# rasmus-kirk/halo

Measured on AMD Instinct MI355X. Metric: MSM points/sec (Pippenger, Pallas, 2^20 points, resident SRS), higher is better.
Workload: dtype u32 limbs (255-bit Montgomery field, integer)

## Files before the change

halo_amd/csrc/curve.hpp:

```cpp
#pragma once
#include "fields.hpp"

HALO_ARITH_BEGIN

struct PallasCurve {
    using Base = FqCfg;
    using Scalar = FpCfg;
    using K = PallasCurveCfg;
};
struct VestaCurve {
    using Base = FpCfg;
    using Scalar = FqCfg;
    using K = VestaCurveCfg;
};

template <class F>
struct Affine {
    Fe<F> x, y;
};

template <class F>
struct XYZZ {
    Fe<F> X, Y, ZZ, ZZZ;
};
// ... 44 lines not shown
    const Fe<F> V = fe_sqr(U);
    const Fe<F> W = fe_mul(U, V);
    const Fe<F> S = fe_mul(p.X, V);
    const Fe<F> X2 = fe_sqr(p.X);
    const Fe<F> M = fe_norm(fe_add_nc(X2, fe_add_nc(X2, X2)));
    XYZZ<F> r;
    r.X = fe_reduce_8p(fe_sub_k<4>(fe_sqr(M), fe_add_nc(S, S)));
    r.Y = fe_sub(fe_mul(M, fe_sub_k<2>(S, r.X)), fe_mul(W, p.Y));
    r.ZZ = fe_mul(V, p.ZZ);
    r.ZZZ = fe_mul(W, p.ZZZ);
    return r;
}

template <class F>
HALO_DEV XYZZ<F> xyzz_mdbl(const Affine<F>& a) {
    const Fe<F> U = fe_norm(fe_add_nc(a.y, a.y));
    const Fe<F> V = fe_sqr(U);
    const Fe<F> W = fe_mul(U, V);
    const Fe<F> S = fe_mul(a.x, V);
    const Fe<F> X2 = fe_sqr(a.x);
    const Fe<F> M = fe_norm(fe_add_nc(X2, fe_add_nc(X2, X2)));
    XYZZ<F> r;
    r.X = fe_reduce_8p(fe_sub_k<4>(fe_sqr(M), fe_add_nc(S, S)));
    r.Y = fe_sub(fe_mul(M, fe_sub_k<2>(S, r.X)), fe_mul(W, a.y));
    r.ZZ = V;
    r.ZZZ = W;
    return r;
}

template <class F>
HALO_DEV XYZZ<F> xyzz_madd(const XYZZ<F>& p, const Affine<F>& q) {
    if (aff_is_id(q)) return p;
    if (xyzz_is_id(p)) return xyzz_from_aff(q);
    const Fe<F> U2 = fe_mul(q.x, p.ZZ);
    const Fe<F> S2 = fe_mul(q.y, p.ZZZ);
    const Fe<F> P = fe_sub_k<2>(U2, p.X);
    const Fe<F> R = fe_sub_k<2>(S2, p.Y);
    const Fe<F> PP = fe_sqr(P);
    const Fe<F> ZZ3 = fe_mul(p.ZZ, PP);
    if (fe_is_zero(ZZ3)) {
        if (fe_is_zero_4p(R)) return xyzz_mdbl(q);
        return xyzz_id<F>();
    }
    const Fe<F> PPP = fe_mul(P, PP);
    const Fe<F> Q = fe_mul(p.X, PP);
    XYZZ<F> r;
    r.X = fe_reduce_8p(fe_sub_k<6>(fe_sqr(R), fe_add_nc(PPP, fe_add_nc(Q, Q))));
    r.Y = fe_sub(fe_mul(R, fe_sub_k<2>(Q, r.X)), fe_mul(p.Y, PPP));
    r.ZZ = ZZ3;
    r.ZZZ = fe_mul(p.ZZZ, PPP);
    return r;
}

template <class F>
HALO_DEV XYZZ<F> xyzz_madd_acc(const XYZZ<F>& p, const Affine<F>& q, uint32_t negmask) {
    if (aff_is_id(q)) return p;
    if (xyzz_is_id(p)) {
        XYZZ<F> r = xyzz_from_aff(q);
        if (negmask) r.Y = fe_neg(q.y);
        return r;
    }
    const Fe<F> U2 = fe_mul(q.x, p.ZZ);
    const Fe<F> S2 = fe_mul(q.y, p.ZZZ);
    const Fe<F> P = fe_sub_k<8>(U2, p.X);
    const Fe<F> R = fe_sub_k_sgn<4>(S2, p.Y, negmask);
    const Fe<F> PP = fe_sqr(P);
    const Fe<F> R2 = fe_sqr(R);
    const Fe<F> ZZ3 = fe_mul(p.ZZ, PP);
    const Fe<F> PPP = fe_mul(P, PP);
    const Fe<F> Q = fe_mul(p.X, PP);
    XYZZ<F> r;
    r.X = fe_sub_k<6>(R2, fe_add_nc(PPP, fe_add_nc(Q, Q)));
    const Fe<F> T = fe_sub_k<8>(Q, r.X);
    r.Y = fe_mul2(R, T, PPP, fe_sub_k<2>(fe_zero<F>(), p.Y));
    r.ZZ = ZZ3;
    r.ZZZ = fe_mul(p.ZZZ, PPP);
    if (fe_is_zero(ZZ3)) {
        if (fe_is_zero(fe_reduce_8p(R))) {
            Affine<F> qs = q;
            if (negmask) qs.y = fe_neg(q.y);
            return xyzz_mdbl(qs);
        }
        return xyzz_id<F>();
    }
    return r;
}

template <class F>
HALO_DEV XYZZ<F> xyzz_madd_run(const XYZZ<F>& p, uint32_t& sneg, bool& fresh, const Affine<F>& q, uint32_t negmask,
                               bool check_q) {
    if (check_q && aff_is_id(q)) return p;
    if (fresh) {
        fresh = false;
        sneg = negmask;
        asm volatile("" : "+v"(sneg));
        XYZZ<F> r;
        r.X = q.x;
        r.Y = q.y;
        r.ZZ = fe_one<F>();
        r.ZZZ = fe_one<F>();
        return r;
    }
    const Fe<F> U2 = fe_mul(q.x, p.ZZ);
    const Fe<F> S2 = fe_mul(q.y, p.ZZZ);
    const Fe<F> P = fe_sub_k<4>(U2, p.X);
    const Fe<F> R = fe_sub_k_sgn<4>(S2, p.Y, negmask ^ sneg);
    const Fe<F> PP = fe_sqr(P);
    const Fe<F> R2 = fe_sqr(R);
    const Fe<F> ZZ3 = fe_mul(p.ZZ, PP);
    const Fe<F> PPP = fe_mul(P, PP);
    const Fe<F> V = fe_mul(U2, PP);
    const Fe<F> Q = fe_sub_nc(V, PPP);
    XYZZ<F> r;
    r.X = fe_sub_nc(fe_sub_nc(R2, Q), V);
    const Fe<F> T = fe_sub_k<6>(r.X, Q);
    r.Y = fe_mul2(R, T, p.Y, PPP);
    r.ZZ = ZZ3;
    r.ZZZ = fe_mul(p.ZZZ, PPP);
    if (P.v[0] < 10u && fe_is_zero(ZZ3)) {
        const bool dbl = fe_is_zero(fe_reduce_8p(R));
        sneg = 0;
        if (dbl) {
            Affine<F> qs = q;
            if (negmask) qs.y = fe_neg(q.y);
            return xyzz_mdbl(qs);
        }
        fresh = true;
        return xyzz_id<F>();
    }
    sneg = ~sneg;
    return r;
}

template <class F>
HALO_DEV XYZZ<F> xyzz_madd_run_aff(const XYZZ<F>& p, uint32_t& sneg, bool& fresh, const Affine<F>& q, uint32_t negmask,
                                   bool check_q) {
    if (check_q && aff_is_id(q)) return p;
    if (fresh) {
        fresh = false;
        sneg = negmask;
        asm volatile("" : "+v"(sneg));
        XYZZ<F> r;
        r.X = q.x;
        r.Y = q.y;
        r.ZZ = fe_one<F>();
        r.ZZZ = fe_one<F>();
        return r;
    }
    const Fe<F> P = fe_sub_k<2>(q.x, p.X);
    const Fe<F> R = fe_sub_k_sgn<4>(q.y, p.Y, negmask ^ sneg);
    const Fe<F> PP = fe_sqr(P);
    const Fe<F> R2 = fe_sqr(R);
    const Fe<F> PPP = fe_mul(P, PP);
    const Fe<F> V = fe_mul(q.x, PP);
    const Fe<F> Q = fe_sub_nc(V, PPP);
    XYZZ<F> r;
    r.X = fe_sub_nc(fe_sub_nc(R2, Q), V);
    const Fe<F> T = fe_sub_k<6>(r.X, Q);
    r.Y = fe_mul2(R, T, p.Y, PPP);
    r.ZZ = PP;
    r.ZZZ = PPP;
    if (P.v[0] < 4u && fe_is_zero(PP)) {
        const bool dbl = fe_is_zero(fe_reduce_8p(R));
        sneg = 0;
        if (dbl) {
            Affine<F> qs = q;
            if (negmask) qs.y = fe_neg(q.y);
            return xyzz_mdbl(qs);
        }
        fresh = true;
        return xyzz_id<F>();
    }
    sneg = ~sneg;
    return r;
}

template <class F>
HALO_DEV XYZZ<F> xyzz_run_out(const XYZZ<F>& p, uint32_t sneg) {
    XYZZ<F> r = p;
    r.X = fe_sub_k<4>(p.X, fe_zero<F>());
    int32_t c = 0;
#pragma unroll
    for (int i = 0; i < NLIMB; i++) {
        const int32_t x = (int32_t)((p.Y.v[i] ^ sneg) - sneg) + (int32_t)(F::P2[i] & sneg) + c;
        r.Y.v[i] = (i == NLIMB - 1) ? (uint32_t)x : ((uint32_t)x & LIMB_MASK);
        c = x >> LIMB_BITS;
    }
    return r;
}

template <class F>
HALO_DEV XYZZ<F> xyzz_settle(const XYZZ<F>& p) {
    XYZZ<F> r = p;
    r.X = fe_reduce_8p(p.X);
    return r;
}

template <class F>
HALO_DEV XYZZ<F> xyzz_add(const XYZZ<F>& p, const XYZZ<F>& q) {
    if (xyzz_is_id(q)) return p;
    if (xyzz_is_id(p)) return q;
    const Fe<F> U1 = fe_mul(p.X, q.ZZ);
    const Fe<F> U2 = fe_mul(q.X, p.ZZ);
    const Fe<F> S1 = fe_mul(p.Y, q.ZZZ);
    const Fe<F> S2 = fe_mul(q.Y, p.ZZZ);
    const Fe<F> P = fe_sub_k<2>(U2, U1);
    const Fe<F> R = fe_sub_k<2>(S2, S1);
    const Fe<F> PP = fe_sqr(P);
    const Fe<F> ZZ3 = fe_mul(fe_mul(p.ZZ, q.ZZ), PP);
    if (fe_is_zero(ZZ3)) {
        if (fe_is_zero_4p(R)) return xyzz_dbl(p);
        return xyzz_id<F>();
    }
    const Fe<F> PPP = fe_mul(P, PP);
    const Fe<F> Q = fe_mul(U1, PP);
    XYZZ<F> r;
    r.X = fe_reduce_8p(fe_sub_k<6>(fe_sqr(R), fe_add_nc(PPP, fe_add_nc(Q, Q))));
    r.Y = fe_sub(fe_mul(R, fe_sub_k<2>(Q, r.X)), fe_mul(S1, PPP));
    r.ZZ = ZZ3;
    r.ZZZ = fe_mul(fe_mul(p.ZZZ, q.ZZZ), PPP);
    return r;
}

template <class F>
HALO_DEV XYZZ<F> xyzz_add_acc(const XYZZ<F>& p, const XYZZ<F>& q) {
    if (xyzz_is_id(q)) return p;
    if (xyzz_is_id(p)) return q;
    const Fe<F> U1 = fe_mul(p.X, q.ZZ);
    const Fe<F> U2 = fe_mul(q.X, p.ZZ);
    const Fe<F> S1 = fe_mul(p.Y, q.ZZZ);
    const Fe<F> S2 = fe_mul(q.Y, p.ZZZ);
    const Fe<F> P = fe_sub_k<2>(U2, U1);
    const Fe<F> R = fe_sub_k<2>(S2, S1);
    const Fe<F> PP = fe_sqr(P);
    const Fe<F> R2 = fe_sqr(R);
    const Fe<F> ZZ3 = fe_mul(fe_mul(p.ZZ, q.ZZ), PP);
    const Fe<F> PPP = fe_mul(P, PP);
    const Fe<F> Q = fe_mul(U1, PP);
    XYZZ<F> r;
    r.X = fe_sub_k<6>(R2, fe_add_nc(PPP, fe_add_nc(Q, Q)));
    const Fe<F> T = fe_sub_k<8>(Q, r.X);
    r.Y = fe_mul2(R, T, PPP, fe_sub_k<2>(fe_zero<F>(), S1));
    r.ZZ = ZZ3;
    r.ZZZ = fe_mul(fe_mul(p.ZZZ, q.ZZZ), PPP);
    if (P.v[0] < 4u && fe_is_zero(ZZ3)) {
        if (fe_is_zero_4p(R)) return xyzz_dbl(xyzz_settle(p));
        return xyzz_id<F>();
    }
    return r;
}

template <class F>
HALO_DEV XYZZ<F> xyzz_neg(const XYZZ<F>& p) {
    XYZZ<F> r = p;
    r.Y = fe_neg(p.Y);
    return r;
}

template <class F>
HALO_DEV Affine<F> xyzz_to_aff(const XYZZ<F>& p) {
    Affine<F> r;
    if (xyzz_is_id(p)) {
        r.x = fe_zero<F>();
        r.y = fe_zero<F>();
        return r;
    }
    const Fe<F> t = fe_inv(fe_mul(p.ZZ, p.ZZZ));
    r.x = fe_mul(p.X, fe_mul(t, p.ZZZ));
    r.y = fe_mul(p.Y, fe_mul(t, p.ZZ));
    return r;
}

template <class F>
HALO_DEV Affine<F> aff_load(const uint4* p) {
    Affine<F> a;
    a.x = fe_load<F>(p);
    a.y = fe_load<F>(p + 2);
    return a;
}
template <class F>
HALO_DEV void aff_store(uint4* p, const Affine<F>& a) {
    fe_store(p, a.x);
    fe_store(p + 2, a.y);
}
template <class F>
HALO_DEV XYZZ<F> xyzz_load(const uint4* p) {
    XYZZ<F> a;
    a.X = fe_load<F>(p);
    a.Y = fe_load<F>(p + 2);
    a.ZZ = fe_load<F>(p + 4);
    a.ZZZ = fe_load<F>(p + 6);
    return a;
}
template <class F>
HALO_DEV void xyzz_store(uint4* p, const XYZZ<F>& a) {
    fe_store(p, a.X);
    fe_store(p + 2, a.Y);
    fe_store(p + 4, a.ZZ);
    fe_store(p + 6, a.ZZZ);
}

constexpr int PARTIAL_U4 = 9;
template <class F>
HALO_DEV void partial_store(uint4* p, const XYZZ<F>& a) {
    const Fe<F>* c[4] = {&a.X, &a.Y, &a.ZZ, &a.ZZZ};
    uint32_t w[4 * NLIMB];
#pragma unroll
    for (int k = 0; k < 4; k++)
#pragma unroll
        for (int i = 0; i < NLIMB; i++) w[k * NLIMB + i] = c[k]->v[i];
#pragma unroll
    for (int q = 0; q < PARTIAL_U4; q++) p[q] = make_uint4(w[4 * q], w[4 * q + 1], w[4 * q + 2], w[4 * q + 3]);
}
template <class F>
HALO_DEV XYZZ<F> partial_load(const uint4* p) {
    uint32_t w[4 * NLIMB];
#pragma unroll
    for (int q = 0; q < PARTIAL_U4; q++) {
        const uint4 v = p[q];
        w[4 * q] = v.x;
        w[4 * q + 1] = v.y;
        w[4 * q + 2] = v.z;
        w[4 * q + 3] = v.w;
    }
    XYZZ<F> a;
    Fe<F>* c[4] = {&a.X, &a.Y, &a.ZZ, &a.ZZZ};
#pragma unroll
    for (int k = 0; k < 4; k++)
#pragma unroll
        for (int i = 0; i < NLIMB; i++) c[k]->v[i] = w[k * NLIMB + i];
    a.X = fe_reduce_8p(a.X);
    return a;
}

template <class F>
HALO_DEV Affine<F> aff_from_wrapped(const uint4* p) {
    Affine<F> a;
    a.x = fe_from_ark<F>(p);
    a.y = fe_from_ark<F>(p + 2);
    return a;
}
template <class F>
HALO_DEV void aff_to_wrapped(uint4* p, const Affine<F>& a) {
    fe_to_ark(p, a.x);
    fe_to_ark(p + 2, a.y);
}

template <class F>
struct Jac {
    Fe<F> X, Y, Z;
};

template <class F>
HALO_DEV Jac<F> jac_from_xyzz(const XYZZ<F>& p) {
    Jac<F> r;
    if (xyzz_is_id(p)) {
        r.X = fe_one<F>();
        r.Y = fe_one<F>();
        r.Z = fe_zero<F>();
        return r;
    }
    r.X = fe_mul(p.X, fe_sqr(p.ZZ));
    r.Y = fe_mul(p.Y, fe_sqr(p.ZZZ));
    r.Z = p.ZZZ;
    return r;
}

template <class F>
HALO_DEV XYZZ<F> jac_to_xyzz(const Jac<F>& j) {
    XYZZ<F> r;
    r.X = j.X;
    r.Y = j.Y;
    r.ZZ = fe_sqr(j.Z);
    r.ZZZ = fe_mul(r.ZZ, j.Z);
    return r;
}

template <class F>
HALO_DEV Jac<F> jac_dbl(const Jac<F>& p) {
    const Fe<F> A = fe_sqr(p.X);
    const Fe<F> B = fe_sqr(p.Y);
    const Fe<F> C = fe_sqr(B);
    const Fe<F> D = fe_dbl(fe_sub(fe_sub(fe_sqr(fe_add(p.X, B)), A), C));
    const Fe<F> E = fe_add(A, fe_dbl(A));
    const Fe<F> Fv = fe_sqr(E);
    Jac<F> r;
    r.X = fe_sub(Fv, fe_dbl(D));
    const Fe<F> C8 = fe_dbl(fe_dbl(fe_dbl(C)));
    r.Y = fe_sub(fe_mul(E, fe_sub(D, r.X)), C8);
    r.Z = fe_dbl(fe_mul(p.Y, p.Z));
    return r;
}

template <class F>
HALO_DEV XYZZ<F> xyzz_scalar_mul(const Affine<F>& P, const uint32_t (&k)[8]) {
    XYZZ<F> acc = xyzz_id<F>();
    for (int i = 255; i >= 0; i--) {
        acc = xyzz_dbl(acc);
        if ((k[i >> 5] >> (i & 31)) & 1u) acc = xyzz_madd(acc, P);
    }
    return acc;
}

HALO_ARITH_END
```

halo_amd/csrc/digits.hpp:

```cpp
#pragma once
#include "digits_core.hpp"
#include "fields.hpp"

namespace halo {

template <class S, int WMAX = 0, int C = 0, class Fn>
HALO_DEV void scalar_signed_digits(const uint4* scalar, int c, int W, Fn&& f) {
    uint32_t w8[8];
    fe_ark_to_canonical_words<S>(scalar, w8);
    uint32_t t8[8];
    int64_t br = 0, lt = 0;
#pragma unroll
    for (int q = 0; q < 8; q++) {
        const int64_t d = (int64_t)(uint32_t)(S::MODULUS64[q >> 1] >> (32 * (q & 1))) - (int64_t)w8[q] + br;
        t8[q] = (uint32_t)d;
        br = d >> 32;
        lt = ((int64_t)t8[q] - (int64_t)w8[q] + lt) >> 32;
    }
    const bool neg = lt != 0;
#pragma unroll
    for (int q = 0; q < 8; q++) w8[q] = neg ? t8[q] : w8[q];
    signed_digit_entries<C, WMAX>(w8, neg ? 0x80000000u : 0u, c, W, f);
}

}
```

halo_amd/csrc/digits_core.hpp:

```cpp
#pragma once
#include <cstdint>

#if defined(__HIPCC__)
#define HALO_DIGITS_FN __host__ __device__ inline __attribute__((always_inline))
#else
#define HALO_DIGITS_FN inline
#endif
#if defined(__clang__)
#define HALO_DIGITS_UNROLL _Pragma("unroll")
#else
#define HALO_DIGITS_UNROLL
#endif

namespace halo {

constexpr uint32_t DIGIT_NONE = 0xffffffffu;

HALO_DIGITS_FN uint32_t digits_funnel(uint32_t hi, uint32_t lo, uint32_t s) {
    return (uint32_t)((((uint64_t)hi << 32) | lo) >> s);
}

HALO_DIGITS_FN uint32_t digits_entry(uint32_t raw, uint32_t& carry, uint32_t half, uint32_t full, uint32_t flip) {
    const uint32_t v = raw + carry;
    carry = (uint32_t)(v > half);
    const uint32_t m = 0u - carry;
    const uint32_t mag = (v ^ m) + ((full + 1u) & m);
    return (mag - 1u) | ((carry << 31) ^ flip);
}

template <int C>
constexpr int digits_windows() { return C > 0 ? (255 + C - 1) / C : 0; }

template <int C, int WMAX = 0, class Fn>
HALO_DIGITS_FN void signed_digit_entries(const uint32_t (&w8)[8], uint32_t flip, int c, int W, Fn&& f) {
    static_assert(C >= 0 && C < 32, "window width");
    uint32_t carry = 0;
    if constexpr (C > 0) {
        constexpr uint32_t full = 1u << C, half = full >> 1;
        static_assert(WMAX == 0 || WMAX >= digits_windows<C>(), "W <= WMAX");
        HALO_DIGITS_UNROLL
        for (int w = 0; w < digits_windows<C>(); w++) {
            const int bit = w * C, q = bit >> 5, s = bit & 31;
            const uint32_t hi = (q + 1 < 8 && s + C > 32) ? w8[q + 1] : 0u;
            const uint32_t raw = digits_funnel(hi, w8[q], (uint32_t)s) & (full - 1u);
            f(w, digits_entry(raw, carry, half, full, flip));
        }
    } else {
        const uint32_t full = 1u << c, half = full >> 1;
        uint32_t x[8];
        HALO_DIGITS_UNROLL
        for (int q = 0; q < 8; q++) x[q] = w8[q];
        auto window = [&](int w) {
            const uint32_t raw = x[0] & (full - 1u);
            HALO_DIGITS_UNROLL
            for (int q = 0; q < 7; q++) x[q] = digits_funnel(x[q + 1], x[q], (uint32_t)c);
            x[7] >>= c;
            f(w, digits_entry(raw, carry, half, full, flip));
        };
        if constexpr (WMAX > 0) {
            HALO_DIGITS_UNROLL
            for (int w = 0; w < WMAX; w++)
                if (w < W) window(w);
        } else {
            for (int w = 0; w < W; w++) window(w);
        }
    }
}

}
```

halo_amd/csrc/field_asm.hpp:

```cpp
#pragma once
#include <stdint.h>

namespace halo {

__device__ __forceinline__ void fe_mul_asm(const uint32_t (&a)[9], const uint32_t (&b)[9], const uint32_t (&np)[5], uint32_t (&r)[9]) {
    uint64_t cc;
    asm(
        "v_mad_u64_u32 v[0:1], %9, %10, %19, 0\n"
        "v_and_b32 %0, 0x1fffffff, v0\n"
        "v_ashrrev_i64 v[0:1], 29, v[0:1]\n"
        "v_mad_u64_u32 v[0:1], %9, %10, %20, v[0:1]\n"
        "v_mad_u64_u32 v[0:1], %9, %11, %19, v[0:1]\n"
        "v_mad_i64_i32 v[0:1], %9, %0, %28, v[0:1]\n"
        "v_and_b32 %1, 0x1fffffff, v0\n"
        "v_ashrrev_i64 v[0:1], 29, v[0:1]\n"
        "v_mad_u64_u32 v[0:1], %9, %10, %21, v[0:1]\n"
        "v_mad_u64_u32 v[0:1], %9, %11, %20, v[0:1]\n"
        "v_mad_u64_u32 v[0:1], %9, %12, %19, v[0:1]\n"
        "v_mad_i64_i32 v[0:1], %9, %1, %28, v[0:1]\n"
        "v_mad_i64_i32 v[0:1], %9, %0, %29, v[0:1]\n"
        "v_and_b32 %2, 0x1fffffff, v0\n"
        "v_ashrrev_i64 v[0:1], 29, v[0:1]\n"
        "v_mad_u64_u32 v[0:1], %9, %10, %22, v[0:1]\n"
        "v_mad_u64_u32 v[0:1], %9, %11, %21, v[0:1]\n"
        "v_mad_u64_u32 v[0:1], %9, %12, %20, v[0:1]\n"
        "v_mad_u64_u32 v[0:1], %9, %13, %19, v[0:1]\n"
        "v_mad_i64_i32 v[0:1], %9, %2, %28, v[0:1]\n"
        "v_mad_i64_i32 v[0:1], %9, %1, %29, v[0:1]\n"
        "v_mad_i64_i32 v[0:1], %9, %0, %30, v[0:1]\n"
        "v_and_b32 %3, 0x1fffffff, v0\n"
        "v_ashrrev_i64 v[0:1], 29, v[0:1]\n"
        "v_mad_u64_u32 v[0:1], %9, %10, %23, v[0:1]\n"
        "v_mad_u64_u32 v[0:1], %9, %11, %22, v[0:1]\n"
        "v_mad_u64_u32 v[0:1], %9, %12, %21, v[0:1]\n"
        "v_mad_u64_u32 v[0:1], %9, %13, %20, v[0:1]\n"
        "v_mad_u64_u32 v[0:1], %9, %14, %19, v[0:1]\n"
        "v_mad_i64_i32 v[0:1], %9, %3, %28, v[0:1]\n"
        "v_mad_i64_i32 v[0:1], %9, %2, %29, v[0:1]\n"
        "v_mad_i64_i32 v[0:1], %9, %1, %30, v[0:1]\n"
        "v_mad_i64_i32 v[0:1], %9, %0, %31, v[0:1]\n"
        "v_and_b32 %4, 0x1fffffff, v0\n"
        "v_ashrrev_i64 v[0:1], 29, v[0:1]\n"
        "v_mad_u64_u32 v[0:1], %9, %10, %24, v[0:1]\n"
        "v_mad_u64_u32 v[0:1], %9, %11, %23, v[0:1]\n"
        "v_mad_u64_u32 v[0:1], %9, %12, %22, v[0:1]\n"
        "v_mad_u64_u32 v[0:1], %9, %13, %21, v[0:1]\n"
        "v_mad_u64_u32 v[0:1], %9, %14, %20, v[0:1]\n"
        "v_mad_u64_u32 v[0:1], %9, %15, %19, v[0:1]\n"
        "v_mad_i64_i32 v[0:1], %9, %4, %28, v[0:1]\n"
        "v_mad_i64_i32 v[0:1], %9, %3, %29, v[0:1]\n"
        "v_mad_i64_i32 v[0:1], %9, %2, %30, v[0:1]\n"
        "v_mad_i64_i32 v[0:1], %9, %1, %31, v[0:1]\n"
        "v_and_b32 %5, 0x1fffffff, v0\n"
        "v_ashrrev_i64 v[0:1], 29, v[0:1]\n"
        "v_mad_u64_u32 v[0:1], %9, %10, %25, v[0:1]\n"
        "v_mad_u64_u32 v[0:1], %9, %11, %24, v[0:1]\n"
        "v_mad_u64_u32 v[0:1], %9, %12, %23, v[0:1]\n"
        "v_mad_u64_u32 v[0:1], %9, %13, %22, v[0:1]\n"
        "v_mad_u64_u32 v[0:1], %9, %14, %21, v[0:1]\n"
        "v_mad_u64_u32 v[0:1], %9, %15, %20, v[0:1]\n"
        "v_mad_u64_u32 v[0:1], %9, %16, %19, v[0:1]\n"
        "v_mad_i64_i32 v[0:1], %9, %5, %28, v[0:1]\n"
        "v_mad_i64_i32 v[0:1], %9, %4, %29, v[0:1]\n"
        "v_mad_i64_i32 v[0:1], %9, %3, %30, v[0:1]\n"
        "v_mad_i64_i32 v[0:1], %9, %2, %31, v[0:1]\n"
        "v_and_b32 %6, 0x1fffffff, v0\n"
        "v_ashrrev_i64 v[0:1], 29, v[0:1]\n"
        "v_mad_u64_u32 v[0:1], %9, %10, %26, v[0:1]\n"
        "v_mad_u64_u32 v[0:1], %9, %11, %25, v[0:1]\n"
        "v_mad_u64_u32 v[0:1], %9, %12, %24, v[0:1]\n"
        "v_mad_u64_u32 v[0:1], %9, %13, %23, v[0:1]\n"
        "v_mad_u64_u32 v[0:1], %9, %14, %22, v[0:1]\n"
        "v_mad_u64_u32 v[0:1], %9, %15, %21, v[0:1]\n"
        "v_mad_u64_u32 v[0:1], %9, %16, %20, v[0:1]\n"
        "v_mad_u64_u32 v[0:1], %9, %17, %19, v[0:1]\n"
        "v_mad_i64_i32 v[0:1], %9, %6, %28, v[0:1]\n"
        "v_mad_i64_i32 v[0:1], %9, %5, %29, v[0:1]\n"
        "v_mad_i64_i32 v[0:1], %9, %4, %30, v[0:1]\n"
        "v_mad_i64_i32 v[0:1], %9, %3, %31, v[0:1]\n"
        "v_and_b32 %7, 0x1fffffff, v0\n"
        "v_ashrrev_i64 v[0:1], 29, v[0:1]\n"
        "v_mad_u64_u32 v[0:1], %9, %10, %27, v[0:1]\n"
        "v_mad_u64_u32 v[0:1], %9, %11, %26, v[0:1]\n"
        "v_mad_u64_u32 v[0:1], %9, %12, %25, v[0:1]\n"
        "v_mad_u64_u32 v[0:1], %9, %13, %24, v[0:1]\n"
        "v_mad_u64_u32 v[0:1], %9, %14, %23, v[0:1]\n"
        "v_mad_u64_u32 v[0:1], %9, %15, %22, v[0:1]\n"
        "v_mad_u64_u32 v[0:1], %9, %16, %21, v[0:1]\n"
        "v_mad_u64_u32 v[0:1], %9, %17, %20, v[0:1]\n"
        "v_mad_u64_u32 v[0:1], %9, %18, %19, v[0:1]\n"
        "v_mad_i64_i32 v[0:1], %9, %7, %28, v[0:1]\n"
        "v_mad_i64_i32 v[0:1], %9, %6, %29, v[0:1]\n"
        "v_mad_i64_i32 v[0:1], %9, %5, %30, v[0:1]\n"
        "v_mad_i64_i32 v[0:1], %9, %4, %31, v[0:1]\n"
        "v_mad_i64_i32 v[0:1], %9, %0, %32, v[0:1]\n"
        "v_or_b32 %8, 0xe0000000, v0\n"
        "v_ashrrev_i64 v[0:1], 29, v[0:1]\n"
        "v_lshl_add_u64 v[0:1], v[0:1], 0, 1\n"
        "v_mad_u64_u32 v[0:1], %9, %11, %27, v[0:1]\n"
        "v_mad_u64_u32 v[0:1], %9, %12, %26, v[0:1]\n"
        "v_mad_u64_u32 v[0:1], %9, %13, %25, v[0:1]\n"
        "v_mad_u64_u32 v[0:1], %9, %14, %24, v[0:1]\n"
        "v_mad_u64_u32 v[0:1], %9, %15, %23, v[0:1]\n"
        "v_mad_u64_u32 v[0:1], %9, %16, %22, v[0:1]\n"
        "v_mad_u64_u32 v[0:1], %9, %17, %21, v[0:1]\n"
        "v_mad_u64_u32 v[0:1], %9, %18, %20, v[0:1]\n"
        "v_mad_i64_i32 v[0:1], %9, %8, %28, v[0:1]\n"
        "v_mad_i64_i32 v[0:1], %9, %7, %29, v[0:1]\n"
        "v_mad_i64_i32 v[0:1], %9, %6, %30, v[0:1]\n"
        "v_mad_i64_i32 v[0:1], %9, %5, %31, v[0:1]\n"
        "v_mad_i64_i32 v[0:1], %9, %1, %32, v[0:1]\n"
        "v_and_b32 %0, 0x1fffffff, v0\n"
        "v_ashrrev_i64 v[0:1], 29, v[0:1]\n"
        "v_mad_u64_u32 v[0:1], %9, %12, %27, v[0:1]\n"
        "v_mad_u64_u32 v[0:1], %9, %13, %26, v[0:1]\n"
        "v_mad_u64_u32 v[0:1], %9, %14, %25, v[0:1]\n"
        "v_mad_u64_u32 v[0:1], %9, %15, %24, v[0:1]\n"
        "v_mad_u64_u32 v[0:1], %9, %16, %23, v[0:1]\n"
        "v_mad_u64_u32 v[0:1], %9, %17, %22, v[0:1]\n"
        "v_mad_u64_u32 v[0:1], %9, %18, %21, v[0:1]\n"
        "v_mad_i64_i32 v[0:1], %9, %8, %29, v[0:1]\n"
        "v_mad_i64_i32 v[0:1], %9, %7, %30, v[0:1]\n"
        "v_mad_i64_i32 v[0:1], %9, %6, %31, v[0:1]\n"
        "v_mad_i64_i32 v[0:1], %9, %2, %32, v[0:1]\n"
        "v_and_b32 %1, 0x1fffffff, v0\n"
        "v_ashrrev_i64 v[0:1], 29, v[0:1]\n"
        "v_mad_u64_u32 v[0:1], %9, %13, %27, v[0:1]\n"
        "v_mad_u64_u32 v[0:1], %9, %14, %26, v[0:1]\n"
        "v_mad_u64_u32 v[0:1], %9, %15, %25, v[0:1]\n"
        "v_mad_u64_u32 v[0:1], %9, %16, %24, v[0:1]\n"
        "v_mad_u64_u32 v[0:1], %9, %17, %23, v[0:1]\n"
        "v_mad_u64_u32 v[0:1], %9, %18, %22, v[0:1]\n"
        "v_mad_i64_i32 v[0:1], %9, %8, %30, v[0:1]\n"
        "v_mad_i64_i32 v[0:1], %9, %7, %31, v[0:1]\n"
        "v_mad_i64_i32 v[0:1], %9, %3, %32, v[0:1]\n"
        "v_and_b32 %2, 0x1fffffff, v0\n"
        "v_ashrrev_i64 v[0:1], 29, v[0:1]\n"
        "v_mad_u64_u32 v[0:1], %9, %14, %27, v[0:1]\n"
        "v_mad_u64_u32 v[0:1], %9, %15, %26, v[0:1]\n"
        "v_mad_u64_u32 v[0:1], %9, %16, %25, v[0:1]\n"
        "v_mad_u64_u32 v[0:1], %9, %17, %24, v[0:1]\n"
        "v_mad_u64_u32 v[0:1], %9, %18, %23, v[0:1]\n"
        "v_mad_i64_i32 v[0:1], %9, %8, %31, v[0:1]\n"
        "v_mad_i64_i32 v[0:1], %9, %4, %32, v[0:1]\n"
        "v_and_b32 %3, 0x1fffffff, v0\n"
        "v_ashrrev_i64 v[0:1], 29, v[0:1]\n"
        "v_mad_u64_u32 v[0:1], %9, %15, %27, v[0:1]\n"
        "v_mad_u64_u32 v[0:1], %9, %16, %26, v[0:1]\n"
        "v_mad_u64_u32 v[0:1], %9, %17, %25, v[0:1]\n"
        "v_mad_u64_u32 v[0:1], %9, %18, %24, v[0:1]\n"
        "v_mad_i64_i32 v[0:1], %9, %5, %32, v[0:1]\n"
        "v_and_b32 %4, 0x1fffffff, v0\n"
        "v_ashrrev_i64 v[0:1], 29, v[0:1]\n"
        "v_mad_u64_u32 v[0:1], %9, %16, %27, v[0:1]\n"
        "v_mad_u64_u32 v[0:1], %9, %17, %26, v[0:1]\n"
        "v_mad_u64_u32 v[0:1], %9, %18, %25, v[0:1]\n"
        "v_mad_i64_i32 v[0:1], %9, %6, %32, v[0:1]\n"
        "v_and_b32 %5, 0x1fffffff, v0\n"
        "v_ashrrev_i64 v[0:1], 29, v[0:1]\n"
        "v_mad_u64_u32 v[0:1], %9, %17, %27, v[0:1]\n"
        "v_mad_u64_u32 v[0:1], %9, %18, %26, v[0:1]\n"
        "v_mad_i64_i32 v[0:1], %9, %7, %32, v[0:1]\n"
        "v_and_b32 %6, 0x1fffffff, v0\n"
        "v_ashrrev_i64 v[0:1], 29, v[0:1]\n"
        "v_mad_u64_u32 v[0:1], %9, %18, %27, v[0:1]\n"
        "v_mad_i64_i32 v[0:1], %9, %8, %32, v[0:1]\n"
        "v_and_b32 %7, 0x1fffffff, v0\n"
        "v_alignbit_b32 %8, v1, v0, 29\n"
        : "=&v"(r[0]), "=&v"(r[1]), "=&v"(r[2]), "=&v"(r[3]), "=&v"(r[4]), "=&v"(r[5]), "=&v"(r[6]), "=&v"(r[7]), "=&v"(r[8]), "=&s"(cc)
        : "v"(a[0]), "v"(a[1]), "v"(a[2]), "v"(a[3]), "v"(a[4]), "v"(a[5]), "v"(a[6]), "v"(a[7]), "v"(a[8]), "v"(b[0]), "v"(b[1]), "v"(b[2]), "v"(b[3]), "v"(b[4]), "v"(b[5]), "v"(b[6]), "v"(b[7]), "v"(b[8]), "s"(np[0]), "s"(np[1]), "s"(np[2]), "s"(np[3]), "s"(np[4])
        : "v0", "v1");
}

__device__ __forceinline__ void fe_sqr_asm(const uint32_t (&a)[9], const uint32_t (&a2)[9], const uint32_t (&np)[5], uint32_t (&r)[9]) {
    uint64_t cc;
    asm(
        "v_mad_u64_u32 v[0:1], %9, %10, %10, 0\n"
        "v_and_b32 %0, 0x1fffffff, v0\n"
        "v_ashrrev_i64 v[0:1], 29, v[0:1]\n"
        "v_mad_u64_u32 v[0:1], %9, %19, %11, v[0:1]\n"
        "v_mad_i64_i32 v[0:1], %9, %0, %28, v[0:1]\n"
        "v_and_b32 %1, 0x1fffffff, v0\n"
        "v_ashrrev_i64 v[0:1], 29, v[0:1]\n"
        "v_mad_u64_u32 v[0:1], %9, %19, %12, v[0:1]\n"
        "v_mad_u64_u32 v[0:1], %9, %11, %11, v[0:1]\n"
        "v_mad_i64_i32 v[0:1], %9, %1, %28, v[0:1]\n"
        "v_mad_i64_i32 v[0:1], %9, %0, %29, v[0:1]\n"
        "v_and_b32 %2, 0x1fffffff, v0\n"
        "v_ashrrev_i64 v[0:1], 29, v[0:1]\n"
        "v_mad_u64_u32 v[0:1], %9, %19, %13, v[0:1]\n"
        "v_mad_u64_u32 v[0:1], %9, %20, %12, v[0:1]\n"
        "v_mad_i64_i32 v[0:1], %9, %2, %28, v[0:1]\n"
        "v_mad_i64_i32 v[0:1], %9, %1, %29, v[0:1]\n"
        "v_mad_i64_i32 v[0:1], %9, %0, %30, v[0:1]\n"
        "v_and_b32 %3, 0x1fffffff, v0\n"
        "v_ashrrev_i64 v[0:1], 29, v[0:1]\n"
        "v_mad_u64_u32 v[0:1], %9, %19, %14, v[0:1]\n"
        "v_mad_u64_u32 v[0:1], %9, %20, %13, v[0:1]\n"
        "v_mad_u64_u32 v[0:1], %9, %12, %12, v[0:1]\n"
        "v_mad_i64_i32 v[0:1], %9, %3, %28, v[0:1]\n"
        "v_mad_i64_i32 v[0:1], %9, %2, %29, v[0:1]\n"
        "v_mad_i64_i32 v[0:1], %9, %1, %30, v[0:1]\n"
        "v_mad_i64_i32 v[0:1], %9, %0, %31, v[0:1]\n"
        "v_and_b32 %4, 0x1fffffff, v0\n"
        "v_ashrrev_i64 v[0:1], 29, v[0:1]\n"
        "v_mad_u64_u32 v[0:1], %9, %19, %15, v[0:1]\n"
        "v_mad_u64_u32 v[0:1], %9, %20, %14, v[0:1]\n"
        "v_mad_u64_u32 v[0:1], %9, %21, %13, v[0:1]\n"
        "v_mad_i64_i32 v[0:1], %9, %4, %28, v[0:1]\n"
        "v_mad_i64_i32 v[0:1], %9, %3, %29, v[0:1]\n"
        "v_mad_i64_i32 v[0:1], %9, %2, %30, v[0:1]\n"
        "v_mad_i64_i32 v[0:1], %9, %1, %31, v[0:1]\n"
        "v_and_b32 %5, 0x1fffffff, v0\n"
        "v_ashrrev_i64 v[0:1], 29, v[0:1]\n"
        "v_mad_u64_u32 v[0:1], %9, %19, %16, v[0:1]\n"
        "v_mad_u64_u32 v[0:1], %9, %20, %15, v[0:1]\n"
        "v_mad_u64_u32 v[0:1], %9, %21, %14, v[0:1]\n"
        "v_mad_u64_u32 v[0:1], %9, %13, %13, v[0:1]\n"
        "v_mad_i64_i32 v[0:1], %9, %5, %28, v[0:1]\n"
        "v_mad_i64_i32 v[0:1], %9, %4, %29, v[0:1]\n"
        "v_mad_i64_i32 v[0:1], %9, %3, %30, v[0:1]\n"
        "v_mad_i64_i32 v[0:1], %9, %2, %31, v[0:1]\n"
        "v_and_b32 %6, 0x1fffffff, v0\n"
        "v_ashrrev_i64 v[0:1], 29, v[0:1]\n"
        "v_mad_u64_u32 v[0:1], %9, %19, %17, v[0:1]\n"
        "v_mad_u64_u32 v[0:1], %9, %20, %16, v[0:1]\n"
        "v_mad_u64_u32 v[0:1], %9, %21, %15, v[0:1]\n"
        "v_mad_u64_u32 v[0:1], %9, %22, %14, v[0:1]\n"
        "v_mad_i64_i32 v[0:1], %9, %6, %28, v[0:1]\n"
        "v_mad_i64_i32 v[0:1], %9, %5, %29, v[0:1]\n"
        "v_mad_i64_i32 v[0:1], %9, %4, %30, v[0:1]\n"
        "v_mad_i64_i32 v[0:1], %9, %3, %31, v[0:1]\n"
        "v_and_b32 %7, 0x1fffffff, v0\n"
        "v_ashrrev_i64 v[0:1], 29, v[0:1]\n"
        "v_mad_u64_u32 v[0:1], %9, %19, %18, v[0:1]\n"
        "v_mad_u64_u32 v[0:1], %9, %20, %17, v[0:1]\n"
        "v_mad_u64_u32 v[0:1], %9, %21, %16, v[0:1]\n"
        "v_mad_u64_u32 v[0:1], %9, %22, %15, v[0:1]\n"
        "v_mad_u64_u32 v[0:1], %9, %14, %14, v[0:1]\n"
        "v_mad_i64_i32 v[0:1], %9, %7, %28, v[0:1]\n"
        "v_mad_i64_i32 v[0:1], %9, %6, %29, v[0:1]\n"
        "v_mad_i64_i32 v[0:1], %9, %5, %30, v[0:1]\n"
        "v_mad_i64_i32 v[0:1], %9, %4, %31, v[0:1]\n"
        "v_mad_i64_i32 v[0:1], %9, %0, %32, v[0:1]\n"
        "v_or_b32 %8, 0xe0000000, v0\n"
        "v_ashrrev_i64 v[0:1], 29, v[0:1]\n"
        "v_lshl_add_u64 v[0:1], v[0:1], 0, 1\n"
        "v_mad_u64_u32 v[0:1], %9, %20, %18, v[0:1]\n"
        "v_mad_u64_u32 v[0:1], %9, %21, %17, v[0:1]\n"
        "v_mad_u64_u32 v[0:1], %9, %22, %16, v[0:1]\n"
        "v_mad_u64_u32 v[0:1], %9, %23, %15, v[0:1]\n"
        "v_mad_i64_i32 v[0:1], %9, %8, %28, v[0:1]\n"
        "v_mad_i64_i32 v[0:1], %9, %7, %29, v[0:1]\n"
        "v_mad_i64_i32 v[0:1], %9, %6, %30, v[0:1]\n"
        "v_mad_i64_i32 v[0:1], %9, %5, %31, v[0:1]\n"
        "v_mad_i64_i32 v[0:1], %9, %1, %32, v[0:1]\n"
        "v_and_b32 %0, 0x1fffffff, v0\n"
        "v_ashrrev_i64 v[0:1], 29, v[0:1]\n"
        "v_mad_u64_u32 v[0:1], %9, %21, %18, v[0:1]\n"
        "v_mad_u64_u32 v[0:1], %9, %22, %17, v[0:1]\n"
        "v_mad_u64_u32 v[0:1], %9, %23, %16, v[0:1]\n"
        "v_mad_u64_u32 v[0:1], %9, %15, %15, v[0:1]\n"
        "v_mad_i64_i32 v[0:1], %9, %8, %29, v[0:1]\n"
        "v_mad_i64_i32 v[0:1], %9, %7, %30, v[0:1]\n"
        "v_mad_i64_i32 v[0:1], %9, %6, %31, v[0:1]\n"
        "v_mad_i64_i32 v[0:1], %9, %2, %32, v[0:1]\n"
        "v_and_b32 %1, 0x1fffffff, v0\n"
        "v_ashrrev_i64 v[0:1], 29, v[0:1]\n"
        "v_mad_u64_u32 v[0:1], %9, %22, %18, v[0:1]\n"
        "v_mad_u64_u32 v[0:1], %9, %23, %17, v[0:1]\n"
        "v_mad_u64_u32 v[0:1], %9, %24, %16, v[0:1]\n"
        "v_mad_i64_i32 v[0:1], %9, %8, %30, v[0:1]\n"
        "v_mad_i64_i32 v[0:1], %9, %7, %31, v[0:1]\n"
        "v_mad_i64_i32 v[0:1], %9, %3, %32, v[0:1]\n"
        "v_and_b32 %2, 0x1fffffff, v0\n"
        "v_ashrrev_i64 v[0:1], 29, v[0:1]\n"
        "v_mad_u64_u32 v[0:1], %9, %23, %18, v[0:1]\n"
        "v_mad_u64_u32 v[0:1], %9, %24, %17, v[0:1]\n"
        "v_mad_u64_u32 v[0:1], %9, %16, %16, v[0:1]\n"
        "v_mad_i64_i32 v[0:1], %9, %8, %31, v[0:1]\n"
        "v_mad_i64_i32 v[0:1], %9, %4, %32, v[0:1]\n"
        "v_and_b32 %3, 0x1fffffff, v0\n"
        "v_ashrrev_i64 v[0:1], 29, v[0:1]\n"
        "v_mad_u64_u32 v[0:1], %9, %24, %18, v[0:1]\n"
        "v_mad_u64_u32 v[0:1], %9, %25, %17, v[0:1]\n"
        "v_mad_i64_i32 v[0:1], %9, %5, %32, v[0:1]\n"
        "v_and_b32 %4, 0x1fffffff, v0\n"
        "v_ashrrev_i64 v[0:1], 29, v[0:1]\n"
        "v_mad_u64_u32 v[0:1], %9, %25, %18, v[0:1]\n"
        "v_mad_u64_u32 v[0:1], %9, %17, %17, v[0:1]\n"
        "v_mad_i64_i32 v[0:1], %9, %6, %32, v[0:1]\n"
        "v_and_b32 %5, 0x1fffffff, v0\n"
        "v_ashrrev_i64 v[0:1], 29, v[0:1]\n"
        "v_mad_u64_u32 v[0:1], %9, %26, %18, v[0:1]\n"
        "v_mad_i64_i32 v[0:1], %9, %7, %32, v[0:1]\n"
        "v_and_b32 %6, 0x1fffffff, v0\n"
        "v_ashrrev_i64 v[0:1], 29, v[0:1]\n"
        "v_mad_u64_u32 v[0:1], %9, %18, %18, v[0:1]\n"
        "v_mad_i64_i32 v[0:1], %9, %8, %32, v[0:1]\n"
        "v_and_b32 %7, 0x1fffffff, v0\n"
        "v_alignbit_b32 %8, v1, v0, 29\n"
        : "=&v"(r[0]), "=&v"(r[1]), "=&v"(r[2]), "=&v"(r[3]), "=&v"(r[4]), "=&v"(r[5]), "=&v"(r[6]), "=&v"(r[7]), "=&v"(r[8]), "=&s"(cc)
        : "v"(a[0]), "v"(a[1]), "v"(a[2]), "v"(a[3]), "v"(a[4]), "v"(a[5]), "v"(a[6]), "v"(a[7]), "v"(a[8]), "v"(a2[0]), "v"(a2[1]), "v"(a2[2]), "v"(a2[3]), "v"(a2[4]), "v"(a2[5]), "v"(a2[6]), "v"(a2[7]), "v"(a2[8]), "s"(np[0]), "s"(np[1]), "s"(np[2]), "s"(np[3]), "s"(np[4])
        : "v0", "v1");
}

__device__ __forceinline__ void fe_mul2_asm(const uint32_t (&a)[9], const uint32_t (&b)[9], const uint32_t (&c)[9], const uint32_t (&d)[9], const uint32_t (&np)[5], uint32_t (&r)[9]) {
    uint64_t cc;
    asm(
        "v_mad_u64_u32 v[0:1], %9, %10, %19, 0\n"
        "v_mad_u64_u32 v[2:3], %9, %28, %37, 0\n"
        "v_lshl_add_u64 v[0:1], v[2:3], 0, v[0:1]\n"
        "v_and_b32 %0, 0x1fffffff, v0\n"
        "v_ashrrev_i64 v[0:1], 29, v[0:1]\n"
        "v_mad_u64_u32 v[0:1], %9, %10, %20, v[0:1]\n"
        "v_mad_u64_u32 v[0:1], %9, %11, %19, v[0:1]\n"
        "v_mad_u64_u32 v[2:3], %9, %28, %38, 0\n"
        "v_mad_u64_u32 v[2:3], %9, %29, %37, v[2:3]\n"
        "v_lshl_add_u64 v[0:1], v[2:3], 0, v[0:1]\n"
        "v_mad_i64_i32 v[0:1], %9, %0, %46, v[0:1]\n"
        "v_and_b32 %1, 0x1fffffff, v0\n"
        "v_ashrrev_i64 v[0:1], 29, v[0:1]\n"
        "v_mad_u64_u32 v[0:1], %9, %10, %21, v[0:1]\n"
        "v_mad_u64_u32 v[0:1], %9, %11, %20, v[0:1]\n"
        "v_mad_u64_u32 v[0:1], %9, %12, %19, v[0:1]\n"
        "v_mad_u64_u32 v[2:3], %9, %28, %39, 0\n"
        "v_mad_u64_u32 v[2:3], %9, %29, %38, v[2:3]\n"
        "v_mad_u64_u32 v[2:3], %9, %30, %37, v[2:3]\n"
        "v_lshl_add_u64 v[0:1], v[2:3], 0, v[0:1]\n"
        "v_mad_i64_i32 v[0:1], %9, %1, %46, v[0:1]\n"
        "v_mad_i64_i32 v[0:1], %9, %0, %47, v[0:1]\n"
        "v_and_b32 %2, 0x1fffffff, v0\n"
        "v_ashrrev_i64 v[0:1], 29, v[0:1]\n"
        "v_mad_u64_u32 v[0:1], %9, %10, %22, v[0:1]\n"
        "v_mad_u64_u32 v[0:1], %9, %11, %21, v[0:1]\n"
        "v_mad_u64_u32 v[0:1], %9, %12, %20, v[0:1]\n"
        "v_mad_u64_u32 v[0:1], %9, %13, %19, v[0:1]\n"
        "v_mad_u64_u32 v[2:3], %9, %28, %40, 0\n"
        "v_mad_u64_u32 v[2:3], %9, %29, %39, v[2:3]\n"
        "v_mad_u64_u32 v[2:3], %9, %30, %38, v[2:3]\n"
        "v_mad_u64_u32 v[2:3], %9, %31, %37, v[2:3]\n"
        "v_lshl_add_u64 v[0:1], v[2:3], 0, v[0:1]\n"
        "v_mad_i64_i32 v[0:1], %9, %2, %46, v[0:1]\n"
        "v_mad_i64_i32 v[0:1], %9, %1, %47, v[0:1]\n"
        "v_mad_i64_i32 v[0:1], %9, %0, %48, v[0:1]\n"
        "v_and_b32 %3, 0x1fffffff, v0\n"
        "v_ashrrev_i64 v[0:1], 29, v[0:1]\n"
        "v_mad_u64_u32 v[0:1], %9, %10, %23, v[0:1]\n"
        "v_mad_u64_u32 v[0:1], %9, %11, %22, v[0:1]\n"
        "v_mad_u64_u32 v[0:1], %9, %12, %21, v[0:1]\n"
        "v_mad_u64_u32 v[0:1], %9, %13, %20, v[0:1]\n"
        "v_mad_u64_u32 v[0:1], %9, %14, %19, v[0:1]\n"
        "v_mad_u64_u32 v[2:3], %9, %28, %41, 0\n"
        "v_mad_u64_u32 v[2:3], %9, %29, %40, v[2:3]\n"
        "v_mad_u64_u32 v[2:3], %9, %30, %39, v[2:3]\n"
        "v_mad_u64_u32 v[2:3], %9, %31, %38, v[2:3]\n"
        "v_mad_u64_u32 v[2:3], %9, %32, %37, v[2:3]\n"
        "v_lshl_add_u64 v[0:1], v[2:3], 0, v[0:1]\n"
        "v_mad_i64_i32 v[0:1], %9, %3, %46, v[0:1]\n"
        "v_mad_i64_i32 v[0:1], %9, %2, %47, v[0:1]\n"
        "v_mad_i64_i32 v[0:1], %9, %1, %48, v[0:1]\n"
        "v_mad_i64_i32 v[0:1], %9, %0, %49, v[0:1]\n"
        "v_and_b32 %4, 0x1fffffff, v0\n"
        "v_ashrrev_i64 v[0:1], 29, v[0:1]\n"
        "v_mad_u64_u32 v[0:1], %9, %10, %24, v[0:1]\n"
        "v_mad_u64_u32 v[0:1], %9, %11, %23, v[0:1]\n"
        "v_mad_u64_u32 v[0:1], %9, %12, %22, v[0:1]\n"
        "v_mad_u64_u32 v[0:1], %9, %13, %21, v[0:1]\n"
        "v_mad_u64_u32 v[0:1], %9, %14, %20, v[0:1]\n"
        "v_mad_u64_u32 v[0:1], %9, %15, %19, v[0:1]\n"
        "v_mad_u64_u32 v[2:3], %9, %28, %42, 0\n"
        "v_mad_u64_u32 v[2:3], %9, %29, %41, v[2:3]\n"
        "v_mad_u64_u32 v[2:3], %9, %30, %40, v[2:3]\n"
        "v_mad_u64_u32 v[2:3], %9, %31, %39, v[2:3]\n"
        "v_mad_u64_u32 v[2:3], %9, %32, %38, v[2:3]\n"
        "v_mad_u64_u32 v[2:3], %9, %33, %37, v[2:3]\n"
        "v_lshl_add_u64 v[0:1], v[2:3], 0, v[0:1]\n"
        "v_mad_i64_i32 v[0:1], %9, %4, %46, v[0:1]\n"
        "v_mad_i64_i32 v[0:1], %9, %3, %47, v[0:1]\n"
        "v_mad_i64_i32 v[0:1], %9, %2, %48, v[0:1]\n"
        "v_mad_i64_i32 v[0:1], %9, %1, %49, v[0:1]\n"
        "v_and_b32 %5, 0x1fffffff, v0\n"
        "v_ashrrev_i64 v[0:1], 29, v[0:1]\n"
        "v_mad_u64_u32 v[0:1], %9, %10, %25, v[0:1]\n"
        "v_mad_u64_u32 v[0:1], %9, %11, %24, v[0:1]\n"
        "v_mad_u64_u32 v[0:1], %9, %12, %23, v[0:1]\n"
        "v_mad_u64_u32 v[0:1], %9, %13, %22, v[0:1]\n"
        "v_mad_u64_u32 v[0:1], %9, %14, %21, v[0:1]\n"
        "v_mad_u64_u32 v[0:1], %9, %15, %20, v[0:1]\n"
        "v_mad_u64_u32 v[0:1], %9, %16, %19, v[0:1]\n"
        "v_mad_u64_u32 v[2:3], %9, %28, %43, 0\n"
        "v_mad_u64_u32 v[2:3], %9, %29, %42, v[2:3]\n"
        "v_mad_u64_u32 v[2:3], %9, %30, %41, v[2:3]\n"
        "v_mad_u64_u32 v[2:3], %9, %31, %40, v[2:3]\n"
        "v_mad_u64_u32 v[2:3], %9, %32, %39, v[2:3]\n"
        "v_mad_u64_u32 v[2:3], %9, %33, %38, v[2:3]\n"
        "v_mad_u64_u32 v[2:3], %9, %34, %37, v[2:3]\n"
        "v_lshl_add_u64 v[0:1], v[2:3], 0, v[0:1]\n"
        "v_mad_i64_i32 v[0:1], %9, %5, %46, v[0:1]\n"
        "v_mad_i64_i32 v[0:1], %9, %4, %47, v[0:1]\n"
        "v_mad_i64_i32 v[0:1], %9, %3, %48, v[0:1]\n"
        "v_mad_i64_i32 v[0:1], %9, %2, %49, v[0:1]\n"
        "v_and_b32 %6, 0x1fffffff, v0\n"
        "v_ashrrev_i64 v[0:1], 29, v[0:1]\n"
        "v_mad_u64_u32 v[0:1], %9, %10, %26, v[0:1]\n"
        "v_mad_u64_u32 v[0:1], %9, %11, %25, v[0:1]\n"
        "v_mad_u64_u32 v[0:1], %9, %12, %24, v[0:1]\n"
        "v_mad_u64_u32 v[0:1], %9, %13, %23, v[0:1]\n"
        "v_mad_u64_u32 v[0:1], %9, %14, %22, v[0:1]\n"
        "v_mad_u64_u32 v[0:1], %9, %15, %21, v[0:1]\n"
        "v_mad_u64_u32 v[0:1], %9, %16, %20, v[0:1]\n"
        "v_mad_u64_u32 v[0:1], %9, %17, %19, v[0:1]\n"
        "v_mad_u64_u32 v[2:3], %9, %28, %44, 0\n"
        "v_mad_u64_u32 v[2:3], %9, %29, %43, v[2:3]\n"
        "v_mad_u64_u32 v[2:3], %9, %30, %42, v[2:3]\n"
        "v_mad_u64_u32 v[2:3], %9, %31, %41, v[2:3]\n"
        "v_mad_u64_u32 v[2:3], %9, %32, %40, v[2:3]\n"
        "v_mad_u64_u32 v[2:3], %9, %33, %39, v[2:3]\n"
        "v_mad_u64_u32 v[2:3], %9, %34, %38, v[2:3]\n"
        "v_mad_u64_u32 v[2:3], %9, %35, %37, v[2:3]\n"
        "v_lshl_add_u64 v[0:1], v[2:3], 0, v[0:1]\n"
        "v_mad_i64_i32 v[0:1], %9, %6, %46, v[0:1]\n"
        "v_mad_i64_i32 v[0:1], %9, %5, %47, v[0:1]\n"
        "v_mad_i64_i32 v[0:1], %9, %4, %48, v[0:1]\n"
        "v_mad_i64_i32 v[0:1], %9, %3, %49, v[0:1]\n"
        "v_and_b32 %7, 0x1fffffff, v0\n"
        "v_ashrrev_i64 v[0:1], 29, v[0:1]\n"
        "v_mad_u64_u32 v[0:1], %9, %10, %27, v[0:1]\n"
        "v_mad_u64_u32 v[0:1], %9, %11, %26, v[0:1]\n"
        "v_mad_u64_u32 v[0:1], %9, %12, %25, v[0:1]\n"
        "v_mad_u64_u32 v[0:1], %9, %13, %24, v[0:1]\n"
        "v_mad_u64_u32 v[0:1], %9, %14, %23, v[0:1]\n"
        "v_mad_u64_u32 v[0:1], %9, %15, %22, v[0:1]\n"
        "v_mad_u64_u32 v[0:1], %9, %16, %21, v[0:1]\n"
        "v_mad_u64_u32 v[0:1], %9, %17, %20, v[0:1]\n"
        "v_mad_u64_u32 v[0:1], %9, %18, %19, v[0:1]\n"
        "v_mad_u64_u32 v[2:3], %9, %28, %45, 0\n"
        "v_mad_u64_u32 v[2:3], %9, %29, %44, v[2:3]\n"
        "v_mad_u64_u32 v[2:3], %9, %30, %43, v[2:3]\n"
        "v_mad_u64_u32 v[2:3], %9, %31, %42, v[2:3]\n"
        "v_mad_u64_u32 v[2:3], %9, %32, %41, v[2:3]\n"
        "v_mad_u64_u32 v[2:3], %9, %33, %40, v[2:3]\n"
        "v_mad_u64_u32 v[2:3], %9, %34, %39, v[2:3]\n"
        "v_mad_u64_u32 v[2:3], %9, %35, %38, v[2:3]\n"
        "v_mad_u64_u32 v[2:3], %9, %36, %37, v[2:3]\n"
        "v_lshl_add_u64 v[0:1], v[2:3], 0, v[0:1]\n"
        "v_mad_i64_i32 v[0:1], %9, %7, %46, v[0:1]\n"
        "v_mad_i64_i32 v[0:1], %9, %6, %47, v[0:1]\n"
        "v_mad_i64_i32 v[0:1], %9, %5, %48, v[0:1]\n"
        "v_mad_i64_i32 v[0:1], %9, %4, %49, v[0:1]\n"
        "v_mad_i64_i32 v[0:1], %9, %0, %50, v[0:1]\n"
        "v_or_b32 %8, 0xe0000000, v0\n"
        "v_ashrrev_i64 v[0:1], 29, v[0:1]\n"
        "v_lshl_add_u64 v[0:1], v[0:1], 0, 1\n"
        "v_mad_u64_u32 v[0:1], %9, %11, %27, v[0:1]\n"
        "v_mad_u64_u32 v[0:1], %9, %12, %26, v[0:1]\n"
        "v_mad_u64_u32 v[0:1], %9, %13, %25, v[0:1]\n"
        "v_mad_u64_u32 v[0:1], %9, %14, %24, v[0:1]\n"
        "v_mad_u64_u32 v[0:1], %9, %15, %23, v[0:1]\n"
        "v_mad_u64_u32 v[0:1], %9, %16, %22, v[0:1]\n"
        "v_mad_u64_u32 v[0:1], %9, %17, %21, v[0:1]\n"
        "v_mad_u64_u32 v[0:1], %9, %18, %20, v[0:1]\n"
        "v_mad_u64_u32 v[2:3], %9, %29, %45, 0\n"
        "v_mad_u64_u32 v[2:3], %9, %30, %44, v[2:3]\n"
        "v_mad_u64_u32 v[2:3], %9, %31, %43, v[2:3]\n"
        "v_mad_u64_u32 v[2:3], %9, %32, %42, v[2:3]\n"
        "v_mad_u64_u32 v[2:3], %9, %33, %41, v[2:3]\n"
        "v_mad_u64_u32 v[2:3], %9, %34, %40, v[2:3]\n"
        "v_mad_u64_u32 v[2:3], %9, %35, %39, v[2:3]\n"
        "v_mad_u64_u32 v[2:3], %9, %36, %38, v[2:3]\n"
        "v_lshl_add_u64 v[0:1], v[2:3], 0, v[0:1]\n"
        "v_mad_i64_i32 v[0:1], %9, %8, %46, v[0:1]\n"
        "v_mad_i64_i32 v[0:1], %9, %7, %47, v[0:1]\n"
        "v_mad_i64_i32 v[0:1], %9, %6, %48, v[0:1]\n"
        "v_mad_i64_i32 v[0:1], %9, %5, %49, v[0:1]\n"
        "v_mad_i64_i32 v[0:1], %9, %1, %50, v[0:1]\n"
        "v_and_b32 %0, 0x1fffffff, v0\n"
        "v_ashrrev_i64 v[0:1], 29, v[0:1]\n"
        "v_mad_u64_u32 v[0:1], %9, %12, %27, v[0:1]\n"
        "v_mad_u64_u32 v[0:1], %9, %13, %26, v[0:1]\n"
        "v_mad_u64_u32 v[0:1], %9, %14, %25, v[0:1]\n"
        "v_mad_u64_u32 v[0:1], %9, %15, %24, v[0:1]\n"
        "v_mad_u64_u32 v[0:1], %9, %16, %23, v[0:1]\n"
        "v_mad_u64_u32 v[0:1], %9, %17, %22, v[0:1]\n"
        "v_mad_u64_u32 v[0:1], %9, %18, %21, v[0:1]\n"
        "v_mad_u64_u32 v[2:3], %9, %30, %45, 0\n"
        "v_mad_u64_u32 v[2:3], %9, %31, %44, v[2:3]\n"
        "v_mad_u64_u32 v[2:3], %9, %32, %43, v[2:3]\n"
        "v_mad_u64_u32 v[2:3], %9, %33, %42, v[2:3]\n"
        "v_mad_u64_u32 v[2:3], %9, %34, %41, v[2:3]\n"
        "v_mad_u64_u32 v[2:3], %9, %35, %40, v[2:3]\n"
        "v_mad_u64_u32 v[2:3], %9, %36, %39, v[2:3]\n"
        "v_lshl_add_u64 v[0:1], v[2:3], 0, v[0:1]\n"
        "v_mad_i64_i32 v[0:1], %9, %8, %47, v[0:1]\n"
        "v_mad_i64_i32 v[0:1], %9, %7, %48, v[0:1]\n"
        "v_mad_i64_i32 v[0:1], %9, %6, %49, v[0:1]\n"
        "v_mad_i64_i32 v[0:1], %9, %2, %50, v[0:1]\n"
        "v_and_b32 %1, 0x1fffffff, v0\n"
        "v_ashrrev_i64 v[0:1], 29, v[0:1]\n"
        "v_mad_u64_u32 v[0:1], %9, %13, %27, v[0:1]\n"
        "v_mad_u64_u32 v[0:1], %9, %14, %26, v[0:1]\n"
        "v_mad_u64_u32 v[0:1], %9, %15, %25, v[0:1]\n"
        "v_mad_u64_u32 v[0:1], %9, %16, %24, v[0:1]\n"
        "v_mad_u64_u32 v[0:1], %9, %17, %23, v[0:1]\n"
        "v_mad_u64_u32 v[0:1], %9, %18, %22, v[0:1]\n"
        "v_mad_u64_u32 v[2:3], %9, %31, %45, 0\n"
        "v_mad_u64_u32 v[2:3], %9, %32, %44, v[2:3]\n"
        "v_mad_u64_u32 v[2:3], %9, %33, %43, v[2:3]\n"
        "v_mad_u64_u32 v[2:3], %9, %34, %42, v[2:3]\n"
        "v_mad_u64_u32 v[2:3], %9, %35, %41, v[2:3]\n"
        "v_mad_u64_u32 v[2:3], %9, %36, %40, v[2:3]\n"
        "v_lshl_add_u64 v[0:1], v[2:3], 0, v[0:1]\n"
        "v_mad_i64_i32 v[0:1], %9, %8, %48, v[0:1]\n"
        "v_mad_i64_i32 v[0:1], %9, %7, %49, v[0:1]\n"
        "v_mad_i64_i32 v[0:1], %9, %3, %50, v[0:1]\n"
        "v_and_b32 %2, 0x1fffffff, v0\n"
        "v_ashrrev_i64 v[0:1], 29, v[0:1]\n"
        "v_mad_u64_u32 v[0:1], %9, %14, %27, v[0:1]\n"
        "v_mad_u64_u32 v[0:1], %9, %15, %26, v[0:1]\n"
        "v_mad_u64_u32 v[0:1], %9, %16, %25, v[0:1]\n"
        "v_mad_u64_u32 v[0:1], %9, %17, %24, v[0:1]\n"
        "v_mad_u64_u32 v[0:1], %9, %18, %23, v[0:1]\n"
        "v_mad_u64_u32 v[2:3], %9, %32, %45, 0\n"
        "v_mad_u64_u32 v[2:3], %9, %33, %44, v[2:3]\n"
        "v_mad_u64_u32 v[2:3], %9, %34, %43, v[2:3]\n"
        "v_mad_u64_u32 v[2:3], %9, %35, %42, v[2:3]\n"
        "v_mad_u64_u32 v[2:3], %9, %36, %41, v[2:3]\n"
        "v_lshl_add_u64 v[0:1], v[2:3], 0, v[0:1]\n"
        "v_mad_i64_i32 v[0:1], %9, %8, %49, v[0:1]\n"
        "v_mad_i64_i32 v[0:1], %9, %4, %50, v[0:1]\n"
        "v_and_b32 %3, 0x1fffffff, v0\n"
        "v_ashrrev_i64 v[0:1], 29, v[0:1]\n"
        "v_mad_u64_u32 v[0:1], %9, %15, %27, v[0:1]\n"
        "v_mad_u64_u32 v[0:1], %9, %16, %26, v[0:1]\n"
        "v_mad_u64_u32 v[0:1], %9, %17, %25, v[0:1]\n"
        "v_mad_u64_u32 v[0:1], %9, %18, %24, v[0:1]\n"
        "v_mad_u64_u32 v[2:3], %9, %33, %45, 0\n"
        "v_mad_u64_u32 v[2:3], %9, %34, %44, v[2:3]\n"
        "v_mad_u64_u32 v[2:3], %9, %35, %43, v[2:3]\n"
        "v_mad_u64_u32 v[2:3], %9, %36, %42, v[2:3]\n"
        "v_lshl_add_u64 v[0:1], v[2:3], 0, v[0:1]\n"
        "v_mad_i64_i32 v[0:1], %9, %5, %50, v[0:1]\n"
        "v_and_b32 %4, 0x1fffffff, v0\n"
        "v_ashrrev_i64 v[0:1], 29, v[0:1]\n"
        "v_mad_u64_u32 v[0:1], %9, %16, %27, v[0:1]\n"
        "v_mad_u64_u32 v[0:1], %9, %17, %26, v[0:1]\n"
        "v_mad_u64_u32 v[0:1], %9, %18, %25, v[0:1]\n"
        "v_mad_u64_u32 v[2:3], %9, %34, %45, 0\n"
        "v_mad_u64_u32 v[2:3], %9, %35, %44, v[2:3]\n"
        "v_mad_u64_u32 v[2:3], %9, %36, %43, v[2:3]\n"
        "v_lshl_add_u64 v[0:1], v[2:3], 0, v[0:1]\n"
        "v_mad_i64_i32 v[0:1], %9, %6, %50, v[0:1]\n"
        "v_and_b32 %5, 0x1fffffff, v0\n"
        "v_ashrrev_i64 v[0:1], 29, v[0:1]\n"
        "v_mad_u64_u32 v[0:1], %9, %17, %27, v[0:1]\n"
        "v_mad_u64_u32 v[0:1], %9, %18, %26, v[0:1]\n"
        "v_mad_u64_u32 v[2:3], %9, %35, %45, 0\n"
        "v_mad_u64_u32 v[2:3], %9, %36, %44, v[2:3]\n"
        "v_lshl_add_u64 v[0:1], v[2:3], 0, v[0:1]\n"
        "v_mad_i64_i32 v[0:1], %9, %7, %50, v[0:1]\n"
        "v_and_b32 %6, 0x1fffffff, v0\n"
        "v_ashrrev_i64 v[0:1], 29, v[0:1]\n"
        "v_mad_u64_u32 v[0:1], %9, %18, %27, v[0:1]\n"
        "v_mad_u64_u32 v[2:3], %9, %36, %45, 0\n"
        "v_lshl_add_u64 v[0:1], v[2:3], 0, v[0:1]\n"
        "v_mad_i64_i32 v[0:1], %9, %8, %50, v[0:1]\n"
        "v_and_b32 %7, 0x1fffffff, v0\n"
        "v_alignbit_b32 %8, v1, v0, 29\n"
        : "=&v"(r[0]), "=&v"(r[1]), "=&v"(r[2]), "=&v"(r[3]), "=&v"(r[4]), "=&v"(r[5]), "=&v"(r[6]), "=&v"(r[7]), "=&v"(r[8]), "=&s"(cc)
        : "v"(a[0]), "v"(a[1]), "v"(a[2]), "v"(a[3]), "v"(a[4]), "v"(a[5]), "v"(a[6]), "v"(a[7]), "v"(a[8]), "v"(b[0]), "v"(b[1]), "v"(b[2]), "v"(b[3]), "v"(b[4]), "v"(b[5]), "v"(b[6]), "v"(b[7]), "v"(b[8]), "v"(c[0]), "v"(c[1]), "v"(c[2]), "v"(c[3]), "v"(c[4]), "v"(c[5]), "v"(c[6]), "v"(c[7]), "v"(c[8]), "v"(d[0]), "v"(d[1]), "v"(d[2]), "v"(d[3]), "v"(d[4]), "v"(d[5]), "v"(d[6]), "v"(d[7]), "v"(d[8]), "s"(np[0]), "s"(np[1]), "s"(np[2]), "s"(np[3]), "s"(np[4])
        : "v0", "v1", "v2", "v3");
}

__device__ __forceinline__ void fe_muls_asm(const uint32_t (&a)[9], const uint32_t (&b)[9], const uint32_t (&np)[5], uint32_t (&r)[9]) {
    uint64_t cc;
    asm(
        "v_mad_i64_i32 v[0:1], %9, %10, %19, 0\n"
        "v_and_b32 %0, 0x1fffffff, v0\n"
        "v_ashrrev_i64 v[0:1], 29, v[0:1]\n"
        "v_mad_i64_i32 v[0:1], %9, %10, %20, v[0:1]\n"
        "v_mad_i64_i32 v[0:1], %9, %11, %19, v[0:1]\n"
        "v_mad_i64_i32 v[0:1], %9, %0, %28, v[0:1]\n"
        "v_and_b32 %1, 0x1fffffff, v0\n"
        "v_ashrrev_i64 v[0:1], 29, v[0:1]\n"
        "v_mad_i64_i32 v[0:1], %9, %10, %21, v[0:1]\n"
        "v_mad_i64_i32 v[0:1], %9, %11, %20, v[0:1]\n"
        "v_mad_i64_i32 v[0:1], %9, %12, %19, v[0:1]\n"
        "v_mad_i64_i32 v[0:1], %9, %1, %28, v[0:1]\n"
        "v_mad_i64_i32 v[0:1], %9, %0, %29, v[0:1]\n"
        "v_and_b32 %2, 0x1fffffff, v0\n"
        "v_ashrrev_i64 v[0:1], 29, v[0:1]\n"
        "v_mad_i64_i32 v[0:1], %9, %10, %22, v[0:1]\n"
        "v_mad_i64_i32 v[0:1], %9, %11, %21, v[0:1]\n"
        "v_mad_i64_i32 v[0:1], %9, %12, %20, v[0:1]\n"
        "v_mad_i64_i32 v[0:1], %9, %13, %19, v[0:1]\n"
        "v_mad_i64_i32 v[0:1], %9, %2, %28, v[0:1]\n"
        "v_mad_i64_i32 v[0:1], %9, %1, %29, v[0:1]\n"
        "v_mad_i64_i32 v[0:1], %9, %0, %30, v[0:1]\n"
        "v_and_b32 %3, 0x1fffffff, v0\n"
        "v_ashrrev_i64 v[0:1], 29, v[0:1]\n"
        "v_mad_i64_i32 v[0:1], %9, %10, %23, v[0:1]\n"
        "v_mad_i64_i32 v[0:1], %9, %11, %22, v[0:1]\n"
        "v_mad_i64_i32 v[0:1], %9, %12, %21, v[0:1]\n"
        "v_mad_i64_i32 v[0:1], %9, %13, %20, v[0:1]\n"
        "v_mad_i64_i32 v[0:1], %9, %14, %19, v[0:1]\n"
        "v_mad_i64_i32 v[0:1], %9, %3, %28, v[0:1]\n"
        "v_mad_i64_i32 v[0:1], %9, %2, %29, v[0:1]\n"
        "v_mad_i64_i32 v[0:1], %9, %1, %30, v[0:1]\n"
        "v_mad_i64_i32 v[0:1], %9, %0, %31, v[0:1]\n"
        "v_and_b32 %4, 0x1fffffff, v0\n"
        "v_ashrrev_i64 v[0:1], 29, v[0:1]\n"
        "v_mad_i64_i32 v[0:1], %9, %10, %24, v[0:1]\n"
        "v_mad_i64_i32 v[0:1], %9, %11, %23, v[0:1]\n"
        "v_mad_i64_i32 v[0:1], %9, %12, %22, v[0:1]\n"
        "v_mad_i64_i32 v[0:1], %9, %13, %21, v[0:1]\n"
        "v_mad_i64_i32 v[0:1], %9, %14, %20, v[0:1]\n"
        "v_mad_i64_i32 v[0:1], %9, %15, %19, v[0:1]\n"
        "v_mad_i64_i32 v[0:1], %9, %4, %28, v[0:1]\n"
        "v_mad_i64_i32 v[0:1], %9, %3, %29, v[0:1]\n"
        "v_mad_i64_i32 v[0:1], %9, %2, %30, v[0:1]\n"
        "v_mad_i64_i32 v[0:1], %9, %1, %31, v[0:1]\n"
        "v_and_b32 %5, 0x1fffffff, v0\n"
        "v_ashrrev_i64 v[0:1], 29, v[0:1]\n"
        "v_mad_i64_i32 v[0:1], %9, %10, %25, v[0:1]\n"
        "v_mad_i64_i32 v[0:1], %9, %11, %24, v[0:1]\n"
        "v_mad_i64_i32 v[0:1], %9, %12, %23, v[0:1]\n"
        "v_mad_i64_i32 v[0:1], %9, %13, %22, v[0:1]\n"
        "v_mad_i64_i32 v[0:1], %9, %14, %21, v[0:1]\n"
        "v_mad_i64_i32 v[0:1], %9, %15, %20, v[0:1]\n"
        "v_mad_i64_i32 v[0:1], %9, %16, %19, v[0:1]\n"
        "v_mad_i64_i32 v[0:1], %9, %5, %28, v[0:1]\n"
        "v_mad_i64_i32 v[0:1], %9, %4, %29, v[0:1]\n"
        "v_mad_i64_i32 v[0:1], %9, %3, %30, v[0:1]\n"
        "v_mad_i64_i32 v[0:1], %9, %2, %31, v[0:1]\n"
        "v_and_b32 %6, 0x1fffffff, v0\n"
        "v_ashrrev_i64 v[0:1], 29, v[0:1]\n"
        "v_mad_i64_i32 v[0:1], %9, %10, %26, v[0:1]\n"
        "v_mad_i64_i32 v[0:1], %9, %11, %25, v[0:1]\n"
        "v_mad_i64_i32 v[0:1], %9, %12, %24, v[0:1]\n"
        "v_mad_i64_i32 v[0:1], %9, %13, %23, v[0:1]\n"
        "v_mad_i64_i32 v[0:1], %9, %14, %22, v[0:1]\n"
        "v_mad_i64_i32 v[0:1], %9, %15, %21, v[0:1]\n"
        "v_mad_i64_i32 v[0:1], %9, %16, %20, v[0:1]\n"
        "v_mad_i64_i32 v[0:1], %9, %17, %19, v[0:1]\n"
        "v_mad_i64_i32 v[0:1], %9, %6, %28, v[0:1]\n"
        "v_mad_i64_i32 v[0:1], %9, %5, %29, v[0:1]\n"
        "v_mad_i64_i32 v[0:1], %9, %4, %30, v[0:1]\n"
        "v_mad_i64_i32 v[0:1], %9, %3, %31, v[0:1]\n"
        "v_and_b32 %7, 0x1fffffff, v0\n"
        "v_ashrrev_i64 v[0:1], 29, v[0:1]\n"
        "v_mad_i64_i32 v[0:1], %9, %10, %27, v[0:1]\n"
        "v_mad_i64_i32 v[0:1], %9, %11, %26, v[0:1]\n"
        "v_mad_i64_i32 v[0:1], %9, %12, %25, v[0:1]\n"
        "v_mad_i64_i32 v[0:1], %9, %13, %24, v[0:1]\n"
        "v_mad_i64_i32 v[0:1], %9, %14, %23, v[0:1]\n"
        "v_mad_i64_i32 v[0:1], %9, %15, %22, v[0:1]\n"
        "v_mad_i64_i32 v[0:1], %9, %16, %21, v[0:1]\n"
        "v_mad_i64_i32 v[0:1], %9, %17, %20, v[0:1]\n"
        "v_mad_i64_i32 v[0:1], %9, %18, %19, v[0:1]\n"
        "v_mad_i64_i32 v[0:1], %9, %7, %28, v[0:1]\n"
        "v_mad_i64_i32 v[0:1], %9, %6, %29, v[0:1]\n"
        "v_mad_i64_i32 v[0:1], %9, %5, %30, v[0:1]\n"
        "v_mad_i64_i32 v[0:1], %9, %4, %31, v[0:1]\n"
        "v_mad_i64_i32 v[0:1], %9, %0, %32, v[0:1]\n"
        "v_or_b32 %8, 0xe0000000, v0\n"
        "v_ashrrev_i64 v[0:1], 29, v[0:1]\n"
        "v_lshl_add_u64 v[0:1], v[0:1], 0, 1\n"
        "v_mad_i64_i32 v[0:1], %9, %11, %27, v[0:1]\n"
        "v_mad_i64_i32 v[0:1], %9, %12, %26, v[0:1]\n"
        "v_mad_i64_i32 v[0:1], %9, %13, %25, v[0:1]\n"
        "v_mad_i64_i32 v[0:1], %9, %14, %24, v[0:1]\n"
        "v_mad_i64_i32 v[0:1], %9, %15, %23, v[0:1]\n"
        "v_mad_i64_i32 v[0:1], %9, %16, %22, v[0:1]\n"
        "v_mad_i64_i32 v[0:1], %9, %17, %21, v[0:1]\n"
        "v_mad_i64_i32 v[0:1], %9, %18, %20, v[0:1]\n"
        "v_mad_i64_i32 v[0:1], %9, %8, %28, v[0:1]\n"
        "v_mad_i64_i32 v[0:1], %9, %7, %29, v[0:1]\n"
        "v_mad_i64_i32 v[0:1], %9, %6, %30, v[0:1]\n"
        "v_mad_i64_i32 v[0:1], %9, %5, %31, v[0:1]\n"
        "v_mad_i64_i32 v[0:1], %9, %1, %32, v[0:1]\n"
        "v_and_b32 %0, 0x1fffffff, v0\n"
        "v_ashrrev_i64 v[0:1], 29, v[0:1]\n"
        "v_mad_i64_i32 v[0:1], %9, %12, %27, v[0:1]\n"
        "v_mad_i64_i32 v[0:1], %9, %13, %26, v[0:1]\n"
        "v_mad_i64_i32 v[0:1], %9, %14, %25, v[0:1]\n"
        "v_mad_i64_i32 v[0:1], %9, %15, %24, v[0:1]\n"
        "v_mad_i64_i32 v[0:1], %9, %16, %23, v[0:1]\n"
        "v_mad_i64_i32 v[0:1], %9, %17, %22, v[0:1]\n"
        "v_mad_i64_i32 v[0:1], %9, %18, %21, v[0:1]\n"
        "v_mad_i64_i32 v[0:1], %9, %8, %29, v[0:1]\n"
        "v_mad_i64_i32 v[0:1], %9, %7, %30, v[0:1]\n"
        "v_mad_i64_i32 v[0:1], %9, %6, %31, v[0:1]\n"
        "v_mad_i64_i32 v[0:1], %9, %2, %32, v[0:1]\n"
        "v_and_b32 %1, 0x1fffffff, v0\n"
        "v_ashrrev_i64 v[0:1], 29, v[0:1]\n"
        "v_mad_i64_i32 v[0:1], %9, %13, %27, v[0:1]\n"
        "v_mad_i64_i32 v[0:1], %9, %14, %26, v[0:1]\n"
        "v_mad_i64_i32 v[0:1], %9, %15, %25, v[0:1]\n"
        "v_mad_i64_i32 v[0:1], %9, %16, %24, v[0:1]\n"
        "v_mad_i64_i32 v[0:1], %9, %17, %23, v[0:1]\n"
        "v_mad_i64_i32 v[0:1], %9, %18, %22, v[0:1]\n"
        "v_mad_i64_i32 v[0:1], %9, %8, %30, v[0:1]\n"
        "v_mad_i64_i32 v[0:1], %9, %7, %31, v[0:1]\n"
        "v_mad_i64_i32 v[0:1], %9, %3, %32, v[0:1]\n"
        "v_and_b32 %2, 0x1fffffff, v0\n"
        "v_ashrrev_i64 v[0:1], 29, v[0:1]\n"
        "v_mad_i64_i32 v[0:1], %9, %14, %27, v[0:1]\n"
        "v_mad_i64_i32 v[0:1], %9, %15, %26, v[0:1]\n"
        "v_mad_i64_i32 v[0:1], %9, %16, %25, v[0:1]\n"
        "v_mad_i64_i32 v[0:1], %9, %17, %24, v[0:1]\n"
        "v_mad_i64_i32 v[0:1], %9, %18, %23, v[0:1]\n"
        "v_mad_i64_i32 v[0:1], %9, %8, %31, v[0:1]\n"
        "v_mad_i64_i32 v[0:1], %9, %4, %32, v[0:1]\n"
        "v_and_b32 %3, 0x1fffffff, v0\n"
        "v_ashrrev_i64 v[0:1], 29, v[0:1]\n"
        "v_mad_i64_i32 v[0:1], %9, %15, %27, v[0:1]\n"
        "v_mad_i64_i32 v[0:1], %9, %16, %26, v[0:1]\n"
        "v_mad_i64_i32 v[0:1], %9, %17, %25, v[0:1]\n"
        "v_mad_i64_i32 v[0:1], %9, %18, %24, v[0:1]\n"
        "v_mad_i64_i32 v[0:1], %9, %5, %32, v[0:1]\n"
        "v_and_b32 %4, 0x1fffffff, v0\n"
        "v_ashrrev_i64 v[0:1], 29, v[0:1]\n"
        "v_mad_i64_i32 v[0:1], %9, %16, %27, v[0:1]\n"
        "v_mad_i64_i32 v[0:1], %9, %17, %26, v[0:1]\n"
        "v_mad_i64_i32 v[0:1], %9, %18, %25, v[0:1]\n"
        "v_mad_i64_i32 v[0:1], %9, %6, %32, v[0:1]\n"
        "v_and_b32 %5, 0x1fffffff, v0\n"
        "v_ashrrev_i64 v[0:1], 29, v[0:1]\n"
        "v_mad_i64_i32 v[0:1], %9, %17, %27, v[0:1]\n"
        "v_mad_i64_i32 v[0:1], %9, %18, %26, v[0:1]\n"
        "v_mad_i64_i32 v[0:1], %9, %7, %32, v[0:1]\n"
        "v_and_b32 %6, 0x1fffffff, v0\n"
        "v_ashrrev_i64 v[0:1], 29, v[0:1]\n"
        "v_mad_i64_i32 v[0:1], %9, %18, %27, v[0:1]\n"
        "v_mad_i64_i32 v[0:1], %9, %8, %32, v[0:1]\n"
        "v_and_b32 %7, 0x1fffffff, v0\n"
        "v_alignbit_b32 %8, v1, v0, 29\n"
        : "=&v"(r[0]), "=&v"(r[1]), "=&v"(r[2]), "=&v"(r[3]), "=&v"(r[4]), "=&v"(r[5]), "=&v"(r[6]), "=&v"(r[7]), "=&v"(r[8]), "=&s"(cc)
        : "v"(a[0]), "v"(a[1]), "v"(a[2]), "v"(a[3]), "v"(a[4]), "v"(a[5]), "v"(a[6]), "v"(a[7]), "v"(a[8]), "v"(b[0]), "v"(b[1]), "v"(b[2]), "v"(b[3]), "v"(b[4]), "v"(b[5]), "v"(b[6]), "v"(b[7]), "v"(b[8]), "s"(np[0]), "s"(np[1]), "s"(np[2]), "s"(np[3]), "s"(np[4])
        : "v0", "v1");
}

}
```

halo_amd/csrc/gen_field_asm.py:

```python
import sys

N = 9
RED_J = (1, 2, 3, 4, 8)


def column_products(k, kind):
    out = []
    for i in range(N):
        j = k - i
        if j < 0 or j >= N:
            continue
        if kind in ("mul", "muls"):
            out.append((f"a{i}", f"b{j}"))
        elif kind == "sqr":
            if i < j:
                out.append((f"a2{i}", f"a{j}"))
            elif i == j:
                out.append((f"a{i}", f"a{i}"))
    return out


def body(kind):
    ins = []
    first = True
    for k in range(2 * N - 1):
        if kind == "mul2":
            prods = [(f"a{i}", f"b{k - i}") for i in range(N) if 0 <= k - i < N]
            prods2 = [(f"c{i}", f"d{k - i}") for i in range(N) if 0 <= k - i < N]
        else:
            prods = column_products(k, kind)
            prods2 = []
        mad = "v_mad_i64_i32" if kind == "muls" else "v_mad_u64_u32"
        for x, y in prods:
            ins.append(f"{mad} v[0:1], {{cc}}, {{{x}}}, {{{y}}}, {'0' if first else 'v[0:1]'}")
            first = False
        if prods2:
            for t, (x, y) in enumerate(prods2):
                ins.append(f"v_mad_u64_u32 v[2:3], {{cc}}, {{{x}}}, {{{y}}}, {'0' if t == 0 else 'v[2:3]'}")
            ins.append("v_lshl_add_u64 v[0:1], v[2:3], 0, v[0:1]")
        for j in RED_J:
            i = k - j
            if 0 <= i < N:
                ins.append(f"v_mad_i64_i32 v[0:1], {{cc}}, {{r{i}}}, {{np{j}}}, v[0:1]")
        if k < N - 1:
            ins.append(f"v_and_b32 {{r{k}}}, 0x1fffffff, v0")
            ins.append("v_ashrrev_i64 v[0:1], 29, v[0:1]")
        elif k == N - 1:
            ins.append(f"v_or_b32 {{r{k}}}, 0xe0000000, v0")
            ins.append("v_ashrrev_i64 v[0:1], 29, v[0:1]")
            ins.append("v_lshl_add_u64 v[0:1], v[0:1], 0, 1")
        elif k < 2 * N - 2:
            ins.append(f"v_and_b32 {{r{k - N}}}, 0x1fffffff, v0")
            ins.append("v_ashrrev_i64 v[0:1], 29, v[0:1]")
        else:
            ins.append(f"v_and_b32 {{r{k - N}}}, 0x1fffffff, v0")
            ins.append(f"v_alignbit_b32 {{r{N - 1}}}, v1, v0, 29")
    return ins


def emit(name, kind):
    ins_names = {"mul": ["a", "b"], "muls": ["a", "b"], "sqr": ["a", "a2"], "mul2": ["a", "b", "c", "d"]}[kind]
    ops = [f"r{i}" for i in range(N)] + ["cc"]
    ops += [f"{v}{i}" for v in ins_names for i in range(N)]
    ops += [f"np{j}" for j in RED_J]
    idx = {o: t for t, o in enumerate(ops)}
    lines = [ln.format(**{o: f"%{t}" for o, t in idx.items()}) for ln in body(kind)]
    params = ", ".join(f"const uint32_t (&{v})[9]" for v in ins_names)
    outs = ", ".join(f'"=&v"(r[{i}])' for i in range(N)) + ', "=&s"(cc)'
    ins = ", ".join(f'"v"({v}[{i}])' for v in ins_names for i in range(N))
    ins += ", " + ", ".join(f'"s"(np[{t}])' for t in range(len(RED_J)))
    clob = '"v0", "v1"' + (', "v2", "v3"' if kind == "mul2" else "")
    asm = "\n".join(f'        "{ln}\\n"' for ln in lines)
    return [f"__device__ __forceinline__ void {name}({params}, const uint32_t (&np)[5], uint32_t (&r)[9]) {{",
            "    uint64_t cc;",
            "    asm(",
            asm,
            f"        : {outs}",
            f"        : {ins}",
            f"        : {clob});",
            "}", ""]


def main():
    out = ["// Generated by halo_amd/csrc/gen_field_asm.py -- do not edit (see its docstring).",
           "// np = {-p_1, -p_2, -p_3, -p_4, -p_8} (int32); inputs as fields.hpp's fe_mul / fe_sqr / fe_mul2.",
           "#pragma once", "#include <stdint.h>", "", "namespace halo {", ""]
    out += emit("fe_mul_asm", "mul")
    out += emit("fe_sqr_asm", "sqr")
    out += emit("fe_mul2_asm", "mul2")
    out += emit("fe_muls_asm", "muls")
    out += ["}  // namespace halo", ""]
    sys.stdout.write("\n".join(out))


if __name__ == "__main__":
    main()
```

halo_amd/csrc/msm.hip:

```cpp
#include <algorithm>
#include <type_traits>
#include <vector>
#include <cstdlib>

#include "digits.hpp"
#include "dispatch.hpp"
#include "glv.hpp"
#include "msm.hpp"
#include "points.hpp"
#include "runtime.hpp"
#include "sort.hpp"
#include "tree.hpp"

namespace halo {

static_assert(MSM_PARTIAL_U4 == PARTIAL_U4, "msm_plan.hpp lays the partials out in curve.hpp's PARTIAL_U4 words");

template <class S>
__global__ void k_digits(const uint4* scalars, size_t n, int c, int W, uint32_t* digits, size_t ld, int w_lo,
                         int w_hi) {
    const size_t i = (size_t)blockIdx.x * blockDim.x + threadIdx.x;
    if (i >= n) return;
    scalar_signed_digits<S>(scalars + 2 * i, c, W, [&](int w, uint32_t out) {
        if (w >= w_lo && w < w_hi) digits[(size_t)(w - w_lo) * ld + i] = out;
    });
}

struct DigitSrcs {
    const uint4* s[8];
};
template <class S>
__global__ void k_digits_multi(DigitSrcs src, size_t n, int c, int W, uint32_t* digits, size_t SN) {
    const size_t i = (size_t)blockIdx.x * blockDim.x + threadIdx.x;
    if (i >= n) return;
    uint32_t* d = digits + (size_t)blockIdx.y * SN;
    scalar_signed_digits<S>(src.s[blockIdx.y] + 2 * i, c, W, [&](int w, uint32_t out) { d[(size_t)w * n + i] = out; });
}

template <class Cv>
__global__ void k_digits_glv(const uint4* scalars, size_t n, int c, int W, uint32_t* digits) {
    using S = typename Cv::Scalar;
    const size_t i = (size_t)blockIdx.x * blockDim.x + threadIdx.x;
    if (i >= n) return;
    uint32_t w8[8];
    fe_ark_to_canonical_words<S>(scalars + 2 * i, w8);
    bool neg[2];
    uint32_t mag[2][5];
    glv::decompose<typename Cv::K>(w8, neg[0], mag[0], neg[1], mag[1]);
    const uint32_t half = 1u << (c - 1);
    const uint32_t full = 1u << c;
    for (int h = 0; h < 2; h++) {
        const uint32_t nflip = neg[h] ? 0x80000000u : 0u;
        uint32_t carry = 0;
        for (int w = 0; w < W; w++) {
            const int bit = w * c;
            uint32_t raw = 0;
            if (bit < 160) {
                const int q = bit >> 5, sh = bit & 31;
                const uint64_t lo = mag[h][q];
                const uint64_t hi = (q + 1 < 5) ? mag[h][q + 1] : 0;
                raw = (uint32_t)(((hi << 32) | lo) >> sh) & (full - 1);
            }
            const uint32_t v = raw + carry;
            uint32_t out;
            if (v > half) {
                carry = 1;
                const uint32_t m = full - v;
                out = (m == 0) ? DIGIT_NONE : (((m - 1) | 0x80000000u) ^ nflip);
            } else {
                carry = 0;
                out = (v == 0) ? DIGIT_NONE : ((v - 1) | nflip);
            }
            digits[(size_t)w * 2 * n + (size_t)h * n + i] = out;
        }
    }
}

constexpr int ACC_MIN_BLOCKS = 4;
template <class Cv>
__device__ __forceinline__ void acc_chunk(size_t t, uint32_t cnt, const uint32_t* keys, const uint32_t* vals, uint32_t K,
                                          const uint4* bases, uint32_t n_per_window, uint32_t npw_lg, size_t stride,
                                          uint32_t blk_lg, uint32_t glv_n, uint4* first, uint4* last,
                                          uint4* bucket_sums, uint32_t* bstart, uint32_t NB, uint32_t key_lg,
                                          uint32_t poly_off, bool check_q) {
    using F = typename Cv::Base;
    const size_t beg = t * K;
    if (beg >= cnt) {
        if (t == 0)
            for (uint32_t b = 0; b <= NB; b++) bstart[b] = 0;
        return;
    }
    const uint32_t end = (uint32_t)min((size_t)cnt, beg + K);
    uint32_t cur = keys[beg];
    {
        const uint32_t prev = beg ? keys[beg - 1] : 0xffffffffu;
        if (prev != cur)
            for (uint32_t b = prev + 1; b <= cur; b++) bstart[b] = (uint32_t)beg;
    }
    bool first_done = false;
    XYZZ<F> acc = xyzz_id<F>();
    bool fresh = true;
    uint32_t sneg = 0;
    auto step = [&](uint32_t e, auto pos) {
        constexpr int POS = decltype(pos)::value;
        const uint32_t k = POS == 0 ? cur : keys[e];
        if (POS != 0 && k != cur) {
            for (uint32_t b = cur + 1; b <= k; b++) bstart[b] = e;
            if (!first_done) {
                partial_store(first + PARTIAL_U4 * t, xyzz_run_out(acc, sneg));
                first_done = true;
            } else {
                xyzz_store(bucket_sums + 8 * (size_t)cur, xyzz_settle(xyzz_run_out(acc, sneg)));
            }
            acc = xyzz_id<F>();
            fresh = true;
            sneg = 0;
            cur = k;
        }
        const uint32_t v = vals[e];
        size_t idx = v & 0x7fffffffu;
        if (stride) {
            const uint32_t w = npw_lg < 32 ? (uint32_t)idx >> npw_lg : (uint32_t)idx / n_per_window;
            uint32_t i = (uint32_t)idx - w * n_per_window;
            if (blk_lg < 32) i += (i >> blk_lg) << blk_lg;
            idx = (size_t)w * stride + i + (size_t)((k >> key_lg) & 1u) * poly_off;
        }
        const bool phi = glv_n && idx >= glv_n;
        if (phi) idx -= glv_n;
        Affine<F> p = aff_load<F>(bases + 4 * idx);
        if (phi) p.x = fe_mul(p.x, fe_from_const<F>(Cv::K::BETA));
        const uint32_t negmask = (v & 0x80000000u) ? ~0u : 0u;
        if constexpr (POS == 0) {
            if (!(check_q && aff_is_id(p))) {
                fresh = false;
                sneg = negmask;
                acc.X = p.x;
                acc.Y = p.y;
                acc.ZZ = fe_one<F>();
                acc.ZZZ = fe_one<F>();
            }
        } else if constexpr (POS == 1) {
            acc = xyzz_madd_run_aff(acc, sneg, fresh, p, negmask, check_q);
        } else {
            acc = xyzz_madd_run(acc, sneg, fresh, p, negmask, check_q);
        }
    };
    uint32_t e = (uint32_t)beg;
    step(e++, std::integral_constant<int, 0>{});
    if (e < end) step(e++, std::integral_constant<int, 1>{});
    for (; e < end; e++) step(e, std::integral_constant<int, 2>{});
    partial_store((first_done ? last : first) + PARTIAL_U4 * t, xyzz_run_out(acc, sneg));
    if (end == cnt)
        for (uint32_t b = cur + 1; b <= NB; b++) bstart[b] = cnt;
}

template <class Cv>
__global__ __launch_bounds__(256, ACC_MIN_BLOCKS) void k_acc(const uint32_t* keys, const uint32_t* vals, const uint32_t* count,
                                             uint32_t K, const uint4* bases, uint32_t n_per_window, uint32_t npw_lg,
                                             size_t stride, uint32_t blk_lg, uint32_t glv_n, uint4* first, uint4* last,
                                             uint4* bucket_sums, uint32_t* bstart, uint32_t NB, uint32_t key_lg = 31,
                                             uint32_t poly_off = 0, uint32_t check_q = 1) {
    acc_chunk<Cv>((size_t)blockIdx.x * blockDim.x + threadIdx.x, *count, keys, vals, K, bases, n_per_window, npw_lg,
                  stride, blk_lg, glv_n, first, last, bucket_sums, bstart, NB, key_lg, poly_off, check_q != 0);
}

template <class Cv>
__device__ __forceinline__ void hide_term_block(const uint4* hide_table, const uint4* hide_scalar, int glv,
                                                uint4* hide_out) {
    using F = typename Cv::Base;
    using S = typename Cv::Scalar;
    __shared__ uint4 red[128 * 8];
    __shared__ uint32_t kw[8];
    __shared__ uint32_t neg[2];
    const int i = threadIdx.x;
    if (i == 0) {
        uint32_t w8[8];
        fe_ark_to_canonical_words<S>(hide_scalar, w8);
        if (glv) {
            bool n1, n2;
            uint32_t k1[5], k2[5];
            glv::decompose<typename Cv::K>(w8, n1, k1, n2, k2);
            for (int q = 0; q < 4; q++) {
                kw[q] = k1[q];
                kw[4 + q] = k2[q];
            }
            neg[0] = n1;
            neg[1] = n2;
        } else {
            for (int q = 0; q < 8; q++) kw[q] = w8[q];
        }
    }
    __syncthreads();
    XYZZ<F> v = xyzz_id<F>();
    if ((kw[i >> 5] >> (i & 31)) & 1u) {
        Affine<F> p = aff_load<F>(hide_table + 4 * (glv ? (i & 127) : i));
        if (glv) {
            if (i >= 128) p.x = fe_mul(p.x, fe_from_const<F>(Cv::K::BETA));
            if (neg[i >> 7]) p.y = fe_neg(p.y);
        }
        v = xyzz_from_aff(p);
    }
    v = block_group_sum<F>(v, 256, red);
    if (i == 0) xyzz_store(hide_out, v);
}

template <class Cv>
__global__ __launch_bounds__(256) void k_hide_term(const uint4* hide_table ,
                                                   const uint4* hide_scalar , int glv, uint4* hide_out) {
    hide_term_block<Cv>(hide_table, hide_scalar, glv, hide_out);
}

struct HideScalars {
    const uint4* sc[8];
};
template <class Cv>
__global__ __launch_bounds__(256) void k_hide_terms(const uint4* hide_table, HideScalars hs, int glv, uint4* hide_out) {
    hide_term_block<Cv>(hide_table, hs.sc[blockIdx.x], glv, hide_out + 8 * blockIdx.x);
}

constexpr int MSM_SETS = 4;
struct MsmScratch {
    DevBuf digits, bstart, partials, bucket_sums, seg_acc, seg_sum, bits, window_sums, scan_tmp, conv;
    const uint32_t* skeys = nullptr;
    const uint32_t* scount = nullptr;
    SortScratch sort;
    hipEvent_t acc_done = nullptr, tail_done = nullptr, start = nullptr, front_done = nullptr;
    bool tail_pending = false;
    hipStream_t owner = nullptr;
};
struct MsmPipe {
    MsmScratch set[MSM_SETS];
    hipStream_t slot_owner[2] = {nullptr, nullptr};
    int slot_next[2] = {0, 0};
    uint64_t slot_used[2] = {0, 0}, clock = 0;
    hipStream_t tail[MSM_SETS] = {};
};
static MsmPipe g_msm_pipe[64];

static bool set_busy(const MsmScratch& m) {
    return m.tail_pending && hipEventQuery(m.tail_done) == hipErrorNotReady;
}

static int msm_pick_set(MsmPipe& P, hipStream_t s, bool advance) {
    int slot = (P.slot_owner[0] == s) ? 0 : (P.slot_owner[1] == s) ? 1 : -1;
    if (slot < 0) slot = (P.slot_used[0] <= P.slot_used[1]) ? 0 : 1;
    int set = 2 * slot + P.slot_next[slot];
    if (set_busy(P.set[set])) {
        const int o = slot ^ 1;
        const int oset = 2 * o + P.slot_next[o];
        if (!set_busy(P.set[2 * o]) && !set_busy(P.set[2 * o + 1])) {
            slot = o;
            set = oset;
        }
    }
    if (advance) {
        P.slot_owner[slot] = s;
        P.slot_next[slot] ^= 1;
        P.slot_used[slot] = ++P.clock;
    }
    return set;
}

static int pipe_init(MsmPipe& P) {
    if (P.tail[0]) return HALO_OK;
    for (auto& t : P.tail) HALO_HIP(hipStreamCreateWithFlags(&t, hipStreamNonBlocking));
    for (auto& m : P.set) {
        HALO_HIP(hipEventCreateWithFlags(&m.acc_done, hipEventDisableTiming));
        HALO_HIP(hipEventCreateWithFlags(&m.tail_done, hipEventDisableTiming));
        HALO_HIP(hipEventCreateWithFlags(&m.start, hipEventDisableTiming));
        HALO_HIP(hipEventCreateWithFlags(&m.front_done, hipEventDisableTiming));
    }
    return HALO_OK;
}

void msm_shutdown() {
    for (auto& P : g_msm_pipe) {
        if (!P.tail[0]) continue;
        for (auto& t : P.tail) {
            (void)hipStreamSynchronize(t);
            (void)hipStreamDestroy(t);
            t = nullptr;
        }

        for (auto& m : P.set) {
            for (hipEvent_t* e : {&m.acc_done, &m.tail_done, &m.start, &m.front_done}) {
                if (*e) (void)hipEventDestroy(*e);
                *e = nullptr;
            }
            m.tail_pending = false;
            m.owner = nullptr;
        }
        P.slot_owner[0] = P.slot_owner[1] = nullptr;
    }
}

template <class Cv>
constexpr int curve_id() {
    return std::is_same<Cv, PallasCurve>::value ? HALO_PALLAS : HALO_VESTA;
}

template <class Scratch>
constexpr bool has_grid = std::is_same<Scratch, MsmScratch>::value;

template <class Scratch>
static int plan_reserve(Scratch& S, const MsmPlan& p, size_t hide_slots) {
    if constexpr (has_grid<Scratch>) {
        HALO_CHECK(S.digits.reserve(p.digits_bytes));
        HALO_CHECK(S.seg_acc.reserve(p.rows_bytes));
        HALO_CHECK(S.seg_sum.reserve(p.cols_bytes));
        HALO_CHECK(S.bits.reserve(p.terms_bytes));
    }
    HALO_CHECK(S.bstart.reserve(p.bstart_bytes));
    HALO_CHECK(S.partials.reserve(p.partials_bytes));
    HALO_CHECK(S.bucket_sums.reserve(p.bucket_sums_bytes));
    HALO_CHECK(S.window_sums.reserve(p.window_sums_bytes(hide_slots)));
    return HALO_OK;
}
static uint4* plan_hide_slot(const MsmScratch& M, const MsmPlan& p) { return M.window_sums.as<uint4>() + 8 * (size_t)p.SW; }

struct AccArgs {
    const uint32_t *keys, *vals, *count;
    const uint4* bases;
    uint32_t n_per_window = 1;
    uint32_t npw_lg = 0;
    size_t stride = 0;
    uint32_t blk_lg = 32;
    uint32_t glv_n = 0;
    uint32_t key_lg = 31;
    uint32_t poly_off = 0;
    uint32_t check_q = 1;
    bool profiled = true;
};
template <class Cv, class Scratch>
static int acc_launch(const MsmPlan& p, Scratch& S, const AccArgs& a, hipStream_t s) {
    ProfScope prof(a.profiled ? "msm_acc" : nullptr, s);
    uint4* parts = S.partials.template as<uint4>();
    HALO_LAUNCH(prof, k_acc<Cv>, dim3(grid_for(p.nchunks, 256)), dim3(256), 0, s, a.keys, a.vals, a.count, p.K, a.bases,
                a.n_per_window, a.npw_lg, a.stride, a.blk_lg, a.glv_n, parts + p.off_first, parts + p.off_last,
                S.bucket_sums.template as<uint4>(), S.bstart.template as<uint32_t>(), (uint32_t)p.NB, a.key_lg, a.poly_off,
                a.check_q);
    HALO_HIP(hipGetLastError());
    return HALO_OK;
}

template <class Scratch>
static MsmTailArgs plan_tail_args(const DeviceState* st, const MsmPlan& p, Scratch& S, size_t n, const uint32_t* skeys,
                                  const uint32_t* scount) {
    MsmTailArgs ta;
    uint4* parts = S.partials.template as<uint4>();
    ta.p = p;
    ta.num_cu = (uint32_t)st->num_cu;
    ta.n = n;
    ta.skeys = skeys;
    ta.scount = scount;
    ta.first = parts + p.off_first;
    ta.last = parts + p.off_last;
    ta.g1 = parts + p.off_g1;
    ta.g2 = parts + p.off_g2;
    ta.bstart = S.bstart.template as<uint32_t>();
    ta.bucket_sums = S.bucket_sums.template as<uint4>();
    ta.rows = ta.cols = ta.terms = nullptr;
    if constexpr (has_grid<Scratch>) {
        ta.rows = S.seg_acc.template as<uint4>();
        ta.cols = S.seg_sum.template as<uint4>();
        ta.terms = S.bits.template as<uint4>();
    }
    ta.window_sums = S.window_sums.template as<uint4>();
    return ta;
}

struct MsmWindowRange {
    int w_lo = 0, w_hi = 0, base_w0 = 0;
};

template <class Cv>
static int msm_device_t(DeviceState* st, const uint4* bases_int, bool shifted, size_t shift_stride,
                        const uint4* scalars_ark, size_t n, int c_req, const uint4* hide_table, const uint4* hide_scalar,
                        uint4* d_out_wrapped, hipStream_t s, const MsmOpts& o, MsmWindowRange wr = {}) {
    MsmPipe& PP = g_msm_pipe[st->device & 63];
    HALO_CHECK(pipe_init(PP));
    const int set = o.preset >= 0 ? o.preset : msm_pick_set(PP, s, true);
    MsmScratch& M = PP.set[set];
    if (M.tail_pending && o.preset < 0) HALO_HIP(hipStreamWaitEvent(s, M.tail_done, 0));
    const hipStream_t ts = PP.tail[set];
    const size_t nn = std::max<size_t>(n, 1);
    const bool glv = !shifted;
    const size_t NP = glv ? 2 * nn : nn;
    const int c = c_req ? c_req : msm_window_bits(NP);
    const int W_all = glv ? (129 + c - 1) / c : msm_windows(c);
    int w_lo = wr.w_lo, w_hi = wr.w_hi;
    if (w_hi <= 0 || glv) {
        w_lo = 0;
        w_hi = W_all;
    }
    if (w_lo < 0 || w_hi > W_all || w_lo >= w_hi)
        return set_error(HALO_EINVAL, "window range [%d, %d) outside [0, %d)", w_lo, w_hi, W_all);
    const int W = w_hi - w_lo;
    if (shifted && w_lo != wr.base_w0) bases_int += 4 * (size_t)(w_lo - wr.base_w0) * shift_stride;
    const uint32_t B = 1u << (c - 1);
    const int SW = shifted ? 1 : W;
    const MsmPlan pl = msm_plan((size_t)W * NP, (size_t)SW * B, SW, B, c, st->num_cu, W, shifted ? (size_t)W * nn : NP);
    HALO_CHECK(plan_reserve(M, pl, 1));

    uint4* hide_slot = nullptr;
    if (hide_table && hide_scalar) {
        hide_slot = plan_hide_slot(M, pl);
        HALO_HIP(hipEventRecord(M.start, s));
        HALO_HIP(hipStreamWaitEvent(ts, M.start, 0));
        if (o.hide_ready) HALO_HIP(hipStreamWaitEvent(ts, o.hide_ready, 0));
        hipLaunchKernelGGL(k_hide_term<Cv>, dim3(1), dim3(256), 0, ts, hide_table, hide_scalar, (int)o.hide_glv,
                           hide_slot);
        HALO_HIP(hipGetLastError());
    }

    if (n > 0) {
        const bool fuse = shifted && w_lo == 0 && w_hi == W_all && msm_fuse_first_pass(1, n, W_all, B, pl.key_bits);
        if (glv)
            hipLaunchKernelGGL(k_digits_glv<Cv>, dim3(grid_for(n, 256)), dim3(256), 0, s, scalars_ark, n, c, W,
                               M.digits.as<uint32_t>());
        else if (!fuse)
            hipLaunchKernelGGL(k_digits<typename Cv::Scalar>, dim3(grid_for(n, 256)), dim3(256), 0, s, scalars_ark,
                               n, c, W_all, M.digits.as<uint32_t>(), n, w_lo, w_hi);
        HALO_HIP(hipGetLastError());
        uint32_t *skeys = nullptr, *svals = nullptr;
        const uint32_t* scount = nullptr;
        RsFused fz{scalars_ark, n, c, W_all, curve_id<Cv>() == HALO_PALLAS ? HALO_FP : HALO_FQ};
        HALO_CHECK(msm_radix_sort(M.digits.as<const uint32_t>(), pl.E, pl.SN, B, pl.key_bits, M.sort, &skeys, &svals,
                                  &scount, nullptr, pl.NB, s, fuse ? &fz : nullptr));
        const SrsState& srs_c = st->srs[curve_id<Cv>()];
        const bool srs_bases = shifted && srs_c.shifted_c != 0 && srs_c.shifted.ptr &&
                               (const char*)bases_int >= srs_c.shifted.as<const char>() &&
                               (const char*)bases_int < srs_c.shifted.as<const char>() + srs_c.shifted.bytes;
        AccArgs a{skeys, svals, scount, bases_int};
        a.n_per_window = (uint32_t)nn;
        a.npw_lg = is_pow2(nn) ? ilog2(nn) : 0xffu;
        a.stride = (shifted && (shift_stride != nn || o.blk_lg < 32)) ? shift_stride : (size_t)0;
        a.blk_lg = o.blk_lg;
        a.glv_n = glv ? (uint32_t)nn : 0u;
        a.check_q = (srs_bases && !srs_c.shifted_has_id) ? 0u : 1u;
        HALO_CHECK(acc_launch<Cv>(pl, M, a, s));
        M.skeys = skeys;
        M.scount = scount;
    } else {
        HALO_HIP(hipMemsetAsync(M.window_sums.ptr, 0, (size_t)SW * 128, s));
    }
    HALO_HIP(hipEventRecord(M.acc_done, s));
    HALO_HIP(hipStreamWaitEvent(ts, M.acc_done, 0));
    MsmTailArgs ta = plan_tail_args(st, pl, M, n, M.skeys, M.scount);
    const bool fuse = SW == 1 && n > 0;
    if (fuse) {
        ta.final_mode = o.out_xyzz ? 2 : 1;
        ta.final_hide = (const uint4*)hide_slot;
        ta.final_out = (uint4*)d_out_wrapped;
    }
// ... 682 lines not shown
```

halo_amd/csrc/msm_tail.hip:

```cpp
#include <algorithm>
#include <cstdlib>

#include "dispatch.hpp"
#include "msm.hpp"
#include "runtime.hpp"
#include "sort.hpp"
#include "tree.hpp"


namespace halo {

template <class Cv>
__global__ __launch_bounds__(MSM_GROUP) void k_group_sums(const uint32_t* keys, const uint32_t* count, uint32_t K,
                                                          uint32_t span, const uint4* src, uint4* out) {
    using F = typename Cv::Base;
    static_assert(MSM_GROUP == 64, "one wave per group");
    const uint32_t g = blockIdx.x, i = threadIdx.x;
    const uint32_t cnt = *count;
    const size_t e0 = (size_t)g * MSM_GROUP * span * K, e1 = e0 + (size_t)MSM_GROUP * span * K;
    if (e1 > cnt || keys[e0] != keys[e1 - 1]) return;
    const XYZZ<F> v = wave_group_sum<F>(partial_load<F>(src + PARTIAL_U4 * ((size_t)g * MSM_GROUP + i)), 64);
    if (i == 0) partial_store(out + PARTIAL_U4 * (size_t)g, v);
}

template <class Cv, int LN>
__global__ __launch_bounds__(256) void k_merge(const uint32_t* bstart, const uint32_t* count, uint32_t K, size_t nb,
                                               const uint4* first, const uint4* last, const uint4* g1, const uint4* g2,
                                               uint4* bucket_sums) {
    using F = typename Cv::Base;
    const size_t gid = (size_t)blockIdx.x * blockDim.x + threadIdx.x;
    const size_t b = gid / LN;
    const uint32_t j = (uint32_t)(gid % LN);
    bool active = false, starts = false;
    uint32_t t0 = 0, t1 = 0;
    if (b < nb) {
        const uint32_t s = bstart[b], e = bstart[b + 1];
        if (s == e) {
            if (j == 0) xyzz_store(bucket_sums + 8 * b, xyzz_id<F>());
        } else {
            const uint32_t cnt = *count;
            t0 = s / K;
            t1 = (e - 1) / K;
            starts = s == t0 * K;
            active = !(t0 == t1 && !starts && e < min(cnt, (t0 + 1) * K));
        }
    }
    XYZZ<F> acc = xyzz_id<F>();
    if (active) {
        const uint32_t total = t1 - t0, per = (total + LN - 1) / LN;
        uint32_t t = t0 + 1 + j * per;
        const uint32_t tb = min(t1, t0 + (j + 1) * per);
        constexpr uint32_t G2 = MSM_GROUP * MSM_GROUP;
        auto next_src = [&]() -> const uint4* {
            const uint4* src;
            if (t % G2 == 0 && t + G2 <= tb) {
                src = g2 + PARTIAL_U4 * (size_t)(t / G2);
                t += G2;
            } else if (t % MSM_GROUP == 0 && t + MSM_GROUP <= tb) {
                src = g1 + PARTIAL_U4 * (size_t)(t / MSM_GROUP);
                t += MSM_GROUP;
            } else {
                src = first + PARTIAL_U4 * (size_t)t;
                t++;
            }
            return src;
        };
        if (j == 0) acc = partial_load<F>((starts ? first : last) + PARTIAL_U4 * (size_t)t0);
        else if (t <= tb) acc = partial_load<F>(next_src());
        if (t <= tb) {
            XYZZ<F> nxt = partial_load<F>(next_src());
            for (;;) {
                const XYZZ<F> cur = nxt;
                const bool more = t <= tb;
                if (more) nxt = partial_load<F>(next_src());
                acc = xyzz_add_acc(acc, cur);
                if (!more) break;
            }
        }
    }
    for (int m = 1; m < LN; m <<= 1) acc = xyzz_add_acc(acc, xyzz_shfl_xor(acc, m));
    if (active && j == 0) xyzz_store(bucket_sums + 8 * b, xyzz_settle(acc));
}

struct RowcolShape {
    uint32_t gr, rpb, nrb, gc, cpb, ncb;
};
__host__ __device__ __forceinline__ RowcolShape rowcol_shape(uint32_t L, uint32_t H, uint32_t epl) {
    RowcolShape r;
    r.gr = L / epl;
    r.rpb = 256 / r.gr;
    r.nrb = (H + r.rpb - 1) / r.rpb;
    r.gc = H / epl < 256 ? H / epl : 256;
    r.cpb = 256 / r.gc;
    r.ncb = (L + r.cpb - 1) / r.cpb;
    return r;
}
template <class Cv>
__global__ __launch_bounds__(256) void k_rowcol(const uint4* bucket_sums, uint32_t L, uint32_t H, uint32_t epl, uint4* rows,
                                                uint4* cols) {
    using F = typename Cv::Base;
    __shared__ uint4 red[128 * 8];
    const uint32_t w = blockIdx.y, tid = threadIdx.x;
    const uint4* bs = bucket_sums + 8 * (size_t)w * L * H;
    const RowcolShape sh = rowcol_shape(L, H, epl);
    XYZZ<F> v = xyzz_id<F>();
    if (blockIdx.x < sh.nrb) {
        const uint32_t h = blockIdx.x * sh.rpb + tid / sh.gr, l0 = tid % sh.gr;
        if (h < H)
            for (uint32_t l = l0; l < L; l += sh.gr) v = xyzz_add_acc(v, xyzz_load<F>(bs + 8 * ((size_t)h * L + l)));
        v = block_group_sum<F>(xyzz_settle(v), sh.gr, red);
        if (l0 == 0 && h < H) xyzz_store(rows + 8 * ((size_t)w * H + h), v);
    } else {
        const uint32_t l = (blockIdx.x - sh.nrb) * sh.cpb + tid / sh.gc, h0 = tid % sh.gc;
        if (l < L)
            for (uint32_t h = h0; h < H; h += sh.gc) v = xyzz_add_acc(v, xyzz_load<F>(bs + 8 * ((size_t)h * L + l)));
        v = block_group_sum<F>(xyzz_settle(v), sh.gc, red);
        if (h0 == 0 && l < L) xyzz_store(cols + 8 * ((size_t)w * L + l), v);
    }
}

template <class Cv>
__global__ __launch_bounds__(256) void k_bitterms(const uint4* rows, const uint4* cols, uint32_t H, uint32_t L,
                                                  uint32_t logH, uint4* out) {
    using F = typename Cv::Base;
    __shared__ uint4 red[128 * 8];
    const uint32_t k = blockIdx.x, w = blockIdx.y, tid = threadIdx.x;
    const uint32_t NT = gridDim.x;
    const bool is_col = k > logH;
    const uint32_t cnt = is_col ? L : H;
    const uint4* src = is_col ? cols + 8 * (size_t)w * L : rows + 8 * (size_t)w * H;
    const uint32_t bit = is_col ? (k - 1 - logH) : (k - 1);
    XYZZ<F> acc = xyzz_id<F>();
    for (uint32_t j = tid; j < cnt; j += 256) {
        if (k != 0 && !((j >> bit) & 1u)) continue;
        acc = xyzz_add_acc(acc, xyzz_load<F>(src + 8 * j));
    }
    acc = block_group_sum<F>(xyzz_settle(acc), 256, red);
    if (tid == 0) xyzz_store(out + 8 * ((size_t)w * NT + k), acc);
}

template <class F>
__device__ __forceinline__ void pair_emit_host(uint32_t* host, uint32_t* flag, const XYZZ<F>& v, uint32_t seq) {
    const Fe<F>* c[4] = {&v.X, &v.Y, &v.ZZ, &v.ZZZ};
#pragma unroll
    for (int k = 0; k < 4; k++) {
        uint32_t w[8];
        fe_pack(*c[k], w);
#pragma unroll
        for (int i = 0; i < 8; i++) __hip_atomic_store(host + 8 * k + i, w[i], __ATOMIC_RELAXED, __HIP_MEMORY_SCOPE_SYSTEM);
    }
    __hip_atomic_store(flag, seq, __ATOMIC_RELEASE, __HIP_MEMORY_SCOPE_SYSTEM);
}

template <class Cv>
__global__ __launch_bounds__(64) void k_bitcombine(const uint4* terms, uint32_t NT, uint32_t logH, uint32_t logL,
                                                   uint4* window_sums, int fin, const uint4* hide, uint4* out,
                                                   const uint4* pair_hide, MsmOuts8 pair_outs, uint32_t* pair_host,
                                                   uint32_t pair_seq) {
    using F = typename Cv::Base;
    const uint32_t w = blockIdx.x, k = threadIdx.x;
    XYZZ<F> v = xyzz_id<F>();
    const uint32_t D = logH + logL;
    if (D <= 16) {
        const uint32_t j = k >> 2;
        if (j < D) {
            const uint32_t kt = j < logL ? 1 + logH + j : 1 + (j - logL);
            v = xyzz_load<F>(terms + 8 * ((size_t)w * NT + kt));
        }
        for (uint32_t i = 0; i + 1 < D; i++) {
            const XYZZ<F> d2 = xyzz_dbl_quad(v);
            if (i < j) v = d2;
        }
        v = xyzz_shfl(v, (int)((4 * k) & 63u));
        if (k == D) v = xyzz_load<F>(terms + 8 * (size_t)w * NT);
        if (k > D) v = xyzz_id<F>();
        uint32_t G = 1;
        while (G < D + 1) G <<= 1;
        v = wave_group_sum<F>(v, G);
    } else
    {
        if (k < NT) {
            v = xyzz_load<F>(terms + 8 * ((size_t)w * NT + k));
            const uint32_t d = (k == 0) ? 0 : (k <= logH ? (k - 1 + logL) : (k - 1 - logH));
            for (uint32_t i = 0; i < d; i++) v = xyzz_dbl(v);
        }
        uint32_t G = 1;
        while (G < NT) G <<= 1;
        v = wave_group_sum<F>(v, G);
    }
    if (k != 0) return;
    if (pair_hide) {
        const XYZZ<F> r = xyzz_add(v, xyzz_load<F>(pair_hide + 8 * w));
        xyzz_store(pair_outs.o[w], r);
        if (pair_host && w < 2) pair_emit_host(pair_host + 32 * w, pair_host + 64 + w, r, pair_seq);
        return;
    }
    if (fin == 0) {
        xyzz_store(window_sums + 8 * w, v);
        return;
    }
    if (hide) v = xyzz_add(v, xyzz_load<F>(hide));
    if (fin == 2)
        xyzz_store(out, v);
    else
        aff_to_wrapped(out, xyzz_to_aff(v));
}

constexpr uint32_t BATCH_SEGS = 8;
template <class Cv, uint32_t SEGS>
__global__ __launch_bounds__(256) void k_batch_window_sums(const uint4* bucket_sums, uint32_t SW, uint32_t B,
                                                           uint4* window_sums) {
    using F = typename Cv::Base;
    static_assert(SEGS >= 2 && SEGS <= 64 && (SEGS & (SEGS - 1)) == 0, "lanes per window");
    constexpr int KBITS = __builtin_ctz(SEGS);
    const uint32_t tid = threadIdx.x;
    const size_t t = (size_t)blockIdx.x * blockDim.x + tid;
    const uint32_t k = tid % SEGS, G = B / SEGS;
    const size_t w = t / SEGS;
    XYZZ<F> v = xyzz_id<F>();
    if (w < SW) {
        const uint4* bs = bucket_sums + 8 * (w * B + (size_t)k * G);
        XYZZ<F> R = xyzz_id<F>(), S = xyzz_id<F>();
        for (int j = (int)G - 1; j >= 0; j--) {
            R = xyzz_add_acc(R, xyzz_load<F>(bs + 8 * j));
            S = xyzz_add_acc(S, R);
        }
        R = xyzz_settle(R);
        S = xyzz_settle(S);
        if (k) {
            XYZZ<F> X = R;
            for (uint32_t g = G; g > 1; g >>= 1) X = xyzz_dbl(X);
            XYZZ<F> Y = xyzz_id<F>();
            for (int bit = KBITS - 1; bit >= 0; bit--) {
                Y = xyzz_dbl(Y);
                if ((k >> bit) & 1u) Y = xyzz_add(Y, X);
            }
            S = xyzz_add(S, Y);
        }
        v = S;
    }
    v = wave_group_sum<F>(v, SEGS);
    if (k == 0 && w < SW) xyzz_store(window_sums + 8 * w, v);
}

template <class Cv>
__global__ __launch_bounds__(64) void k_final(const uint4* window_sums, int W, int c, const uint4* hide_xyzz,
                                              uint4* out_wrapped, int xyzz_out) {
    using F = typename Cv::Base;
    XYZZ<F> horner = xyzz_id<F>();
    const uint32_t s1 = threadIdx.x & 60u;
    for (int w = W - 1; w >= 0; w--) {
        if (w != W - 1 && !xyzz_is_id(horner))
            for (int k = 0; k < c; k++) horner = xyzz_dbl_quad(horner);
        const XYZZ<F> ws = xyzz_load<F>(window_sums + 8 * w);
        const bool idp = xyzz_is_id(horner), idq = xyzz_is_id(ws);
        if (idp || idq) {
            if (idp) horner = ws;
        } else {
            const XYZZ<F> r = xyzz_add_quad((threadIdx.x & 3u) == 1 ? ws : horner, s1, s1 + 1, false, false);
            horner = xyzz_shfl(r, (int)(s1 + 2));
        }
    }
    if (threadIdx.x != 0) return;
    if (hide_xyzz) horner = xyzz_add(horner, xyzz_load<F>(hide_xyzz));
    if (xyzz_out)
        xyzz_store(out_wrapped, horner);
    else
        aff_to_wrapped(out_wrapped, xyzz_to_aff(horner));
}

template <class Cv>
static int tail_launch_t(const MsmTailArgs& a, hipStream_t ts) {
    if (a.n > 0) {
        if (a.p.ng1)
            hipLaunchKernelGGL(k_group_sums<Cv>, dim3((unsigned)a.p.ng1), dim3(MSM_GROUP), 0, ts, a.skeys, a.scount, a.p.K,
                               1u, (const uint4*)a.first, a.g1);
        if (a.p.ng2)
            hipLaunchKernelGGL(k_group_sums<Cv>, dim3((unsigned)a.p.ng2), dim3(MSM_GROUP), 0, ts, a.skeys, a.scount, a.p.K,
                               MSM_GROUP, (const uint4*)a.g1, a.g2);
        constexpr int lanes = 2;
        hipLaunchKernelGGL((k_merge<Cv, lanes>), dim3(grid_for(a.p.NB * lanes, 256)), dim3(256), 0, ts, (const uint32_t*)a.bstart,
                           a.scount, a.p.K, a.p.NB, (const uint4*)a.first, (const uint4*)a.last,
                           (const uint4*)a.g1, (const uint4*)a.g2, a.bucket_sums);
        if (a.batch_windows) {
            const uint32_t B = a.p.L * a.p.H;
            if (B < 2 * BATCH_SEGS || B > 512 || (B & (B - 1)))
                return set_error(HALO_EINVAL, "batched window sums: %u buckets per window", B);
            const uint32_t segs = std::max(BATCH_SEGS, B / 8);
            auto kws = segs == 8 ? k_batch_window_sums<Cv, 8> : segs == 16 ? k_batch_window_sums<Cv, 16>
                     : segs == 32 ? k_batch_window_sums<Cv, 32> : k_batch_window_sums<Cv, 64>;
            hipLaunchKernelGGL(kws, dim3(grid_for((size_t)a.p.SW * segs, 256)), dim3(256), 0, ts,
                               (const uint4*)a.bucket_sums, (uint32_t)a.p.SW, B, a.window_sums);
            HALO_HIP(hipGetLastError());
            return HALO_OK;
        }
        uint32_t epl = 1;
        while (epl < 4 && 2 * epl <= std::min(a.p.L, a.p.H)) {
            const RowcolShape sh = rowcol_shape(a.p.L, a.p.H, epl);
            if ((size_t)(sh.nrb + sh.ncb) * a.p.SW <= (size_t)a.num_cu) break;
            epl *= 2;
        }
        const RowcolShape sh = rowcol_shape(a.p.L, a.p.H, epl);
        hipLaunchKernelGGL(k_rowcol<Cv>, dim3(sh.nrb + sh.ncb, a.p.SW), dim3(256), 0, ts, (const uint4*)a.bucket_sums,
                           a.p.L, a.p.H, epl, a.rows, a.cols);
        hipLaunchKernelGGL(k_bitterms<Cv>, dim3(a.p.NT, a.p.SW), dim3(256), 0, ts, (const uint4*)a.rows,
                           (const uint4*)a.cols, a.p.H, a.p.L, a.p.logH, a.terms);
        const int fin = a.p.SW == 1 ? a.final_mode : 0;
        hipLaunchKernelGGL(k_bitcombine<Cv>, dim3(a.p.SW), dim3(64), 0, ts, (const uint4*)a.terms, a.p.NT, a.p.logH, a.p.logL,
                           a.window_sums, fin, a.final_hide, a.final_out, a.pair_hide, a.pair_outs, a.pair_host, a.pair_seq);
    }
    HALO_HIP(hipGetLastError());
    return HALO_OK;
}

int msm_final_launch(int curve, const uint4* window_sums, int W, int c, const uint4* hide, uint4* out, int xyzz_out,
                     hipStream_t s) {
    DISPATCH_CURVE(curve, Cv, {
        hipLaunchKernelGGL(k_final<Cv>, dim3(1), dim3(64), 0, s, window_sums, W, c, hide, out, xyzz_out);
    });
    HALO_HIP(hipGetLastError());
    return HALO_OK;
}

int msm_tail_launch(int curve, const MsmTailArgs& a, hipStream_t ts) {
    int rc;
    DISPATCH_CURVE(curve, Cv, { rc = tail_launch_t<Cv>(a, ts); });
    return rc;
}

}
```

halo_amd/csrc/sort.hip:

```cpp
#include <algorithm>
#include <utility>
#include <vector>
#include <type_traits>
#include <cstdlib>

#include "digits.hpp"
#include "dispatch.hpp"
#include "fields.hpp"
#include "runtime.hpp"
#include "sort.hpp"

namespace halo {

constexpr int RS_THREADS = 512;
constexpr int RS_BINS = 256;
constexpr int RS_BINS_MAX = 512;
template <int BITS>
constexpr int rs_rounds() { return BITS == 8 ? 16 : 14; }
constexpr size_t RS_STAGE_BYTES = 2 * 4 * RS_THREADS * 16;
constexpr uint32_t RS_NONE = 0xffffffffu;

struct RsScalars {
    const uint4* s[8] = {};
    uint32_t n = 0, P = 1, B = 0;
};
HALO_DEV const uint4* rs_scalar(const RsScalars& sc, uint32_t g, uint32_t& p, uint32_t& i) {
    p = sc.P == 1 ? 0u : g / sc.n;
    i = g - p * sc.n;
    const uint4* src = sc.s[0];
#pragma unroll
    for (uint32_t q = 1; q < 8; q++)
        if (p == q) src = sc.s[q];
    return src + 2 * (size_t)i;
}

struct RsIn {
    RsScalars sc;
    int c = 0, W = 0;
    const uint32_t* digits;
    const uint32_t* keys;
    const uint32_t* vals;
    const uint32_t* count;
    size_t E;
    size_t npw;
    uint32_t B;
    uint32_t pass;
    uint32_t shift;
};

template <bool PASS0, bool WANT_VAL = true>
HALO_DEV void rs_load(const RsIn& in, size_t e, size_t limit, uint32_t& a, uint32_t& b) {
    const size_t ec = e < limit ? e : (limit ? limit - 1 : 0);
    if constexpr (PASS0) {
        a = in.digits[ec];
        b = 0;
    } else {
        a = in.keys[ec];
        b = WANT_VAL ? in.vals[ec] : 0u;
    }
}
template <bool PASS0>
HALO_DEV bool rs_decode(const RsIn& in, size_t e, size_t limit, uint32_t a, uint32_t b, uint32_t& key, uint32_t& val) {
    if (e >= limit) return false;
    if constexpr (PASS0) {
        if (a == RS_NONE) return false;
        const uint32_t w = (in.npw >= in.E) ? 0u : (uint32_t)e / (uint32_t)in.npw;
        key = w * in.B + (a & 0x7fffffffu);
        val = ((uint32_t)e - w * (uint32_t)in.npw) | (a & 0x80000000u);
    } else {
        key = a;
        val = b;
    }
    return true;
}

HALO_DEV size_t rs_limit(const RsIn& in) { return in.pass == 0 ? in.E : (size_t)*in.count; }

constexpr int RS_CH = 64;
#define RS_RLX_AGENT __ATOMIC_RELAXED, __HIP_MEMORY_SCOPE_AGENT
HALO_DEV void rs_acquire() {
    if (threadIdx.x == 0) __builtin_amdgcn_fence(__ATOMIC_ACQUIRE, "agent");
    asm volatile("s_waitcnt vmcnt(0)" ::: "memory");
    __syncthreads();
}
HALO_DEV bool rs_last_arriver(uint32_t* c, uint32_t total, uint32_t* flag) {
    asm volatile("s_waitcnt vmcnt(0)" ::: "memory");
    __syncthreads();
    if (threadIdx.x == 0) *flag = __hip_atomic_fetch_add(c, 1u, RS_RLX_AGENT) == total - 1;
    __syncthreads();
    return *flag != 0;
}
template <int BINS>
HALO_DEV void rs_publish_and_scan(const uint32_t* h, uint32_t tile, uint32_t ntiles, uint32_t* hist, uint32_t* chunk,
                                  uint32_t* ctr, uint32_t* count) {
    static_assert(BINS <= RS_THREADS, "one thread per digit");
    constexpr int DPL = BINS / 64;
    __shared__ uint32_t flag;
    __shared__ uint32_t s[BINS];
    const uint32_t d = threadIdx.x;
    if (d < BINS) __hip_atomic_store(hist + (size_t)tile * BINS + d, h[d], RS_RLX_AGENT);
    const uint32_t ch = tile / RS_CH, nchunks = (ntiles + RS_CH - 1) / RS_CH;
    const uint32_t t0 = ch * RS_CH, nt = min((uint32_t)RS_CH, ntiles - t0);
    if (!rs_last_arriver(ctr + ch, nt, &flag)) return;
    rs_acquire();
    if (d < BINS) {
        uint32_t v[RS_CH];
#pragma unroll
        for (int i = 0; i < RS_CH; i++) v[i] = (i < (int)nt) ? hist[(size_t)(t0 + i) * BINS + d] : 0u;
        uint32_t run = 0;
#pragma unroll
        for (int i = 0; i < RS_CH; i++) {
            if (i < (int)nt) hist[(size_t)(t0 + i) * BINS + d] = run;
            run += v[i];
        }
        __hip_atomic_store(chunk + (size_t)ch * BINS + d, run, RS_RLX_AGENT);
    }
    if (d == 0) __hip_atomic_store(ctr + ch, 0u, RS_RLX_AGENT);
    if (!rs_last_arriver(ctr + nchunks, nchunks, &flag)) return;
    rs_acquire();
    constexpr uint32_t U = 16;
    if (d < BINS) {
        uint32_t run = 0;
        for (uint32_t c0 = 0; c0 < nchunks; c0 += U) {
            uint32_t v[U];
#pragma unroll
            for (uint32_t i = 0; i < U; i++) v[i] = (c0 + i < nchunks) ? chunk[(size_t)(c0 + i) * BINS + d] : 0u;
#pragma unroll
            for (uint32_t i = 0; i < U; i++) run += v[i];
        }
        s[d] = run;
    }
    __syncthreads();
    if (d < 64) {
        uint32_t c[DPL], sum = 0;
#pragma unroll
        for (int q = 0; q < DPL; q++) {
            c[q] = s[d * DPL + q];
            sum += c[q];
        }
        uint32_t incl = sum;
#pragma unroll
        for (int off = 1; off < 64; off <<= 1) {
            const uint32_t t = __shfl_up(incl, off);
            if ((int)d >= off) incl += t;
        }
        uint32_t ex = incl - sum;
#pragma unroll
        for (int q = 0; q < DPL; q++) {
            s[d * DPL + q] = ex;
            ex += c[q];
        }
        if (d == 63 && count) *count = incl;
    }
    __syncthreads();
    if (d < BINS) {
        uint32_t run = s[d];
        for (uint32_t c0 = 0; c0 < nchunks; c0 += U) {
            uint32_t v[U];
#pragma unroll
            for (uint32_t i = 0; i < U; i++) v[i] = (c0 + i < nchunks) ? chunk[(size_t)(c0 + i) * BINS + d] : 0u;
#pragma unroll
            for (uint32_t i = 0; i < U; i++) {
                if (c0 + i < nchunks) chunk[(size_t)(c0 + i) * BINS + d] = run;
                run += v[i];
            }
        }
    }
    if (d == 0) __hip_atomic_store(ctr + nchunks, 0u, RS_RLX_AGENT);
}

template <int BITS, bool PASS0>
__global__ __launch_bounds__(RS_THREADS) void k_rs_hist(RsIn in, uint32_t ntiles, uint32_t* hist, uint32_t* chunk,
                                                        uint32_t* ctr, uint32_t* count) {
    constexpr int ROUNDS = rs_rounds<BITS>();
    constexpr int BINS = 1 << BITS;
    constexpr int RS_TILE = RS_THREADS * ROUNDS;
    __shared__ uint32_t h[BINS];
    if (threadIdx.x < BINS) h[threadIdx.x] = 0;
    const size_t limit = rs_limit(in);
    const size_t base = (size_t)blockIdx.x * RS_TILE;
    uint32_t A[ROUNDS], Bv[ROUNDS];
#pragma unroll
    for (int r = 0; r < ROUNDS; r++)
        rs_load<PASS0, false>(in, base + (size_t)r * RS_THREADS + threadIdx.x, limit, A[r], Bv[r]);
    __syncthreads();
#pragma unroll
    for (int r = 0; r < ROUNDS; r++) {
        uint32_t k, v;
        if (rs_decode<PASS0>(in, base + (size_t)r * RS_THREADS + threadIdx.x, limit, A[r], Bv[r], k, v))
            atomicAdd(&h[(k >> in.shift) & (BINS - 1u)], 1u);
    }
    __syncthreads();
    rs_publish_and_scan<BINS>(h, blockIdx.x, ntiles, hist, chunk, ctr, count);
}

template <class S, int C>
__global__ __launch_bounds__(RS_THREADS) void k_rs_hist_sc(const RsScalars sc, int c, int W, uint32_t ntiles,
                                                         uint32_t* hist, uint32_t* chunk, uint32_t* ctr,
                                                         uint32_t* count) {
    __shared__ uint32_t h[RS_BINS];
    if (threadIdx.x < RS_BINS) h[threadIdx.x] = 0;
    __syncthreads();
    const uint32_t g = blockIdx.x * RS_THREADS + threadIdx.x;
    if (g < sc.P * sc.n) {
        uint32_t p, i;
        scalar_signed_digits<S, 0, C>(rs_scalar(sc, g, p, i), c, W, [&](int, uint32_t d) {
            if (d != DIGIT_NONE) atomicAdd(&h[d & 255u], 1u);
        });
    }
    __syncthreads();
    rs_publish_and_scan<RS_BINS>(h, blockIdx.x, ntiles, hist, chunk, ctr, count);
}

template <int BITS, class SF = void, bool PASS0 = false, int C = 0>
__global__ __launch_bounds__(RS_THREADS) void k_rs_scatter(RsIn in, const uint32_t* tile_off, const uint32_t* chunk_off,
                                                           uint32_t* keys_out, uint32_t* vals_out) {
    constexpr int ROUNDS = rs_rounds<BITS>();
    constexpr int BINS = 1 << BITS;
    constexpr uint32_t DMASK = BINS - 1;
    constexpr int DPL = BINS / 64;
    constexpr int RS_TILE = RS_THREADS * ROUNDS;
    constexpr int WAVES = RS_THREADS / 64;
    constexpr int PER_WAVE = RS_TILE / WAVES;
    __shared__ uint32_t goff[BINS];
    __shared__ uint32_t lstart[BINS];
    __shared__ uint32_t wpos[WAVES][BINS];
    static_assert(2 * 4 * RS_TILE <= RS_STAGE_BYTES, "staging size");
    extern __shared__ uint32_t rs_stage[];
    uint32_t* skey = rs_stage;
    uint32_t* sval = rs_stage + RS_TILE;
    __shared__ uint32_t total;
    const int tid = threadIdx.x, lane = tid & 63, wave = tid >> 6;
    const size_t limit = rs_limit(in);
    const size_t wbase = (size_t)blockIdx.x * RS_TILE + (size_t)wave * PER_WAVE;
    constexpr int R = PER_WAVE / 64;
    uint32_t K[R], V[R];
    uint32_t validmask = 0;
    if constexpr (!std::is_void<SF>::value) {
#pragma unroll
        for (int r = 0; r < R; r++) {
            K[r] = 0;
            V[r] = 0;
        }
        const uint32_t g = blockIdx.x * RS_THREADS + tid;
        if (g < in.sc.P * in.sc.n) {
            uint32_t p, i;
            const uint4* src = rs_scalar(in.sc, g, p, i);
            const uint32_t koff = p * in.sc.B;
            scalar_signed_digits<SF, R, C>(src, in.c, in.W, [&](int w, uint32_t d) {
                K[w] = koff + (d & 0x7fffffffu);
                V[w] = ((uint32_t)w * in.sc.n + i) | (d & 0x80000000u);
                validmask |= (uint32_t)(d != DIGIT_NONE) << w;
            });
        }
    } else {
        uint32_t A[R], Bv[R];
#pragma unroll
        for (int r = 0; r < R; r++) rs_load<PASS0>(in, wbase + (size_t)r * 64 + lane, limit, A[r], Bv[r]);
#pragma unroll
        for (int r = 0; r < R; r++) {
            K[r] = 0;
            V[r] = 0;
            if (rs_decode<PASS0>(in, wbase + (size_t)r * 64 + lane, limit, A[r], Bv[r], K[r], V[r])) validmask |= 1u << r;
        }
    }
    bool any_order = PASS0 || !std::is_void<SF>::value;
    if constexpr (!PASS0 && std::is_void<SF>::value) {
        const uint32_t first = __builtin_amdgcn_readfirstlane(K[0]);
        uint32_t diff = 0;
#pragma unroll
        for (int r = 0; r < R; r++) diff |= K[r] ^ first;
        diff &= (1u << in.shift) - 1u;
        any_order = __ballot(diff != 0 || validmask != (1u << R) - 1u) == 0;
    }
    if (tid < BINS) {
        goff[tid] = tile_off[(size_t)blockIdx.x * BINS + tid] + chunk_off[(size_t)(blockIdx.x / RS_CH) * BINS + tid];
#pragma unroll
        for (int w = 0; w < WAVES; w++) wpos[w][tid] = 0;
    }
    __syncthreads();
#pragma unroll
    for (int r = 0; r < R; r++)
        if ((validmask >> r) & 1u) atomicAdd(&wpos[wave][(K[r] >> in.shift) & DMASK], 1u);
    __syncthreads();
    if (tid < BINS) {
        uint32_t cnt = 0;
#pragma unroll
        for (int w = 0; w < WAVES; w++) cnt += wpos[w][tid];
        lstart[tid] = cnt;
    }
    __syncthreads();
    if (wave == 0) {
        uint32_t c[DPL];
        uint32_t sum = 0;
#pragma unroll
        for (int q = 0; q < DPL; q++) {
            c[q] = lstart[lane * DPL + q];
            sum += c[q];
        }
        uint32_t incl = sum;
#pragma unroll
        for (int off = 1; off < 64; off <<= 1) {
            const uint32_t t = __shfl_up(incl, off);
            if (lane >= off) incl += t;
        }
        uint32_t ex = incl - sum;
#pragma unroll
        for (int q = 0; q < DPL; q++) {
            lstart[lane * DPL + q] = ex;
            ex += c[q];
        }
        if (lane == 63) total = incl;
    }
    __syncthreads();
    if (tid < BINS) {
        uint32_t p = lstart[tid];
#pragma unroll
        for (int w = 0; w < WAVES; w++) {
            const uint32_t c = wpos[w][tid];
            wpos[w][tid] = p;
            p += c;
        }
    }
    __syncthreads();
    if (any_order) {
#pragma unroll
        for (int r = 0; r < R; r++) {
            if (!((validmask >> r) & 1u)) continue;
            const uint32_t pos = atomicAdd(&wpos[wave][(K[r] >> in.shift) & DMASK], 1u);
            skey[pos] = K[r];
            sval[pos] = V[r];
        }
    } else {
#pragma unroll
    for (int r = 0; r < R; r++) {
        const uint32_t k = K[r], v = V[r];
        const bool valid = (validmask >> r) & 1u;
        const uint32_t dg = (k >> in.shift) & DMASK;
        uint64_t same = __ballot(valid);
#pragma unroll
        for (int b = 0; b < BITS; b++) {
            const uint64_t m = __ballot((dg >> b) & 1u);
            same &= ((dg >> b) & 1u) ? m : ~m;
        }
        const uint64_t below = same & ((1ull << lane) - 1ull);
        if (valid) {
            const uint32_t pos = wpos[wave][dg] + (uint32_t)__popcll(below);
            skey[pos] = k;
            sval[pos] = v;
        }
        __builtin_amdgcn_wave_barrier();
        if (valid && below == 0) wpos[wave][dg] += (uint32_t)__popcll(same);
        __builtin_amdgcn_wave_barrier();
    }
    }
    __syncthreads();
    for (uint32_t i = tid; i < total; i += RS_THREADS) {
        const uint32_t k = skey[i];
        const uint32_t dg = (k >> in.shift) & DMASK;
        const uint32_t g = goff[dg] + (i - lstart[dg]);
        if (g >= in.E) continue;
        keys_out[g] = k;
        vals_out[g] = sval[i];
    }
}

__global__ void k_bucket_starts(const uint32_t* keys, const uint32_t* count, size_t NB, size_t cap, uint32_t* bstart) {
    const size_t e = (size_t)blockIdx.x * blockDim.x + threadIdx.x;
    const size_t n = *count;
    if (e > n || e > cap) return;
    const int64_t prev = (e == 0) ? -1 : (int64_t)keys[e - 1];
    const int64_t cur = (e == n) ? (int64_t)NB : (int64_t)keys[e];
    for (int64_t b = prev + 1; b <= cur; b++) bstart[b] = (uint32_t)e;
}

constexpr int SC_THREADS = 1024;
__device__ inline uint32_t sc_block_excl(uint32_t v, uint32_t* s, uint32_t* total) {
    s[threadIdx.x] = v;
    __syncthreads();
    for (int off = 1; off < SC_THREADS; off <<= 1) {
        const uint32_t t = ((int)threadIdx.x >= off) ? s[threadIdx.x - off] : 0;
        __syncthreads();
        s[threadIdx.x] += t;
        __syncthreads();
    }
    const uint32_t incl = s[threadIdx.x];
    *total = s[SC_THREADS - 1];
    __syncthreads();
    return incl - v;
}

__global__ __launch_bounds__(SC_THREADS) void k_sc_reduce(const uint32_t* in, size_t n, size_t per, uint32_t* sums) {
    __shared__ uint32_t s[SC_THREADS];
    const size_t beg = (size_t)blockIdx.x * per, end = min(n, beg + per);
    uint32_t acc = 0;
    for (size_t i = beg + threadIdx.x; i < end; i += SC_THREADS) acc += in[i];
    s[threadIdx.x] = acc;
    __syncthreads();
    for (int off = SC_THREADS / 2; off > 0; off >>= 1) {
        if ((int)threadIdx.x < off) s[threadIdx.x] += s[threadIdx.x + off];
        __syncthreads();
    }
    if (threadIdx.x == 0) sums[blockIdx.x] = s[0];
}

__global__ __launch_bounds__(SC_THREADS) void k_sc_sums(uint32_t* sums, int nb) {
    __shared__ uint32_t s[SC_THREADS];
    const int per = (nb + SC_THREADS - 1) / SC_THREADS;
    uint32_t loc[8];
    uint32_t acc = 0;
    for (int k = 0; k < per; k++) {
        const int i = threadIdx.x * per + k;
        loc[k] = (i < nb) ? sums[i] : 0;
        acc += loc[k];
    }
    uint32_t tot;
    uint32_t ex = sc_block_excl(acc, s, &tot);
    for (int k = 0; k < per; k++) {
        const int i = threadIdx.x * per + k;
        if (i < nb) sums[i] = ex;
        ex += loc[k];
    }
    if (threadIdx.x == 0) sums[nb] = tot;
}

__global__ __launch_bounds__(SC_THREADS) void k_sc_apply(const uint32_t* in, size_t n, size_t per, const uint32_t* sums,
                                                         uint32_t* out) {
    __shared__ uint32_t s[SC_THREADS];
    const size_t beg = (size_t)blockIdx.x * per, end = min(n, beg + per);
    uint32_t base = sums[blockIdx.x];
    for (size_t tile = beg; tile < end; tile += (size_t)SC_THREADS * 4) {
        uint32_t loc[4];
        uint32_t acc = 0;
        for (int k = 0; k < 4; k++) {
            const size_t i = tile + (size_t)threadIdx.x * 4 + k;
            loc[k] = (i < end) ? in[i] : 0;
            acc += loc[k];
        }
        uint32_t tot;
        uint32_t ex = sc_block_excl(acc, s, &tot) + base;
        for (int k = 0; k < 4; k++) {
            const size_t i = tile + (size_t)threadIdx.x * 4 + k;
            if (i < end) out[i] = ex;
            ex += loc[k];
        }
        base += tot;
    }
    if (blockIdx.x == gridDim.x - 1 && threadIdx.x == 0) out[n] = sums[gridDim.x];
}

int device_exclusive_scan(const uint32_t* in, size_t n, uint32_t* out, DevBuf& tmp, hipStream_t s) {
    const size_t per = (size_t)SC_THREADS * 16;
    size_t nb = std::max<size_t>(1, (n + per - 1) / per);
    if (nb > (size_t)SC_THREADS * 8) return set_error(HALO_EINVAL, "scan too large (%zu)", n);
    HALO_CHECK(tmp.reserve((nb + 1) * 4));
    hipLaunchKernelGGL(k_sc_reduce, dim3((unsigned)nb), dim3(SC_THREADS), 0, s, in, n, per, tmp.as<uint32_t>());
    hipLaunchKernelGGL(k_sc_sums, dim3(1), dim3(SC_THREADS), 0, s, tmp.as<uint32_t>(), (int)nb);
    hipLaunchKernelGGL(k_sc_apply, dim3((unsigned)nb), dim3(SC_THREADS), 0, s, in, n, per, tmp.as<const uint32_t>(),
                       out);
    HALO_HIP(hipGetLastError());
    return HALO_OK;
}

static std::vector<std::pair<uint32_t, uint32_t>> rs_plan(uint32_t key_bits, bool fused) {
    std::vector<std::pair<uint32_t, uint32_t>> P;
    if (key_bits == 17 || (key_bits == 18 && !fused)) {
        const uint32_t b0 = (key_bits == 18) ? 9 : 8;
        P.push_back({0, b0});
        P.push_back({b0, key_bits - b0});
        return P;
    }
    const uint32_t passes = std::max<uint32_t>(1, (key_bits + 7) / 8);
    for (uint32_t p = 0; p < passes; p++) P.push_back({8 * p, 8});
    return P;
}

template <class SF, int C>
static void rs_launch_fused(const RsIn& in, uint32_t nt, uint32_t* hist, uint32_t* offs, SortScratch& S, int cur,
                            hipStream_t s) {
    hipLaunchKernelGGL((k_rs_hist_sc<SF, C>), dim3(nt), dim3(RS_THREADS), 0, s, in.sc, in.c, in.W, nt, hist, offs,
                       S.ctr.as<uint32_t>(), S.count.as<uint32_t>());
    hipLaunchKernelGGL((k_rs_scatter<8, SF, false, C>), dim3(nt), dim3(RS_THREADS), RS_STAGE_BYTES, s, in,
                       (const uint32_t*)hist, (const uint32_t*)offs, S.keys[cur].as<uint32_t>(),
                       S.vals[cur].as<uint32_t>());
}

int msm_radix_sort(const uint32_t* digits, size_t E, size_t npw, uint32_t B, uint32_t key_bits, SortScratch& S,
                   uint32_t** keys_out, uint32_t** vals_out, const uint32_t** count_out, uint32_t* bstart, size_t NB,
                   hipStream_t s, const RsFused* fused) {
    const auto plan = rs_plan(key_bits, fused != nullptr);
    auto tiles_of = [&](uint32_t bits) {
        const size_t tile = (size_t)RS_THREADS * (bits == 8 ? rs_rounds<8>() : rs_rounds<9>());
        return (uint32_t)std::max<size_t>(1, (E + tile - 1) / tile);
    };
    uint32_t ntmax = 1;
    for (auto& q : plan) ntmax = std::max(ntmax, tiles_of(q.second));
    const size_t nsc = fused ? fused->n * (size_t)fused->P : 0;
    if (fused && (fused->P < 1 || fused->P > 8 || fused->W > rs_rounds<8>() || nsc >= (1ull << 31) / 16 ||
                  (fused->P > 1 && (B & 255)) || fused->c < 1 || fused->c > 31 ||
                  fused->W > (255 + fused->c - 1) / fused->c))
        return set_error(HALO_EINVAL, "fused sort pass: %d outputs of %u buckets, %d windows, %zu scalars", fused->P, B,
                         fused->W, nsc);
    const uint32_t ntiles0 = fused ? (uint32_t)std::max<size_t>(1, (nsc + RS_THREADS - 1) / RS_THREADS) : 0u;
    ntmax = std::max(ntmax, ntiles0);
    HALO_CHECK(S.keys[0].reserve(std::max<size_t>(E, 1) * 4));
    HALO_CHECK(S.keys[1].reserve(std::max<size_t>(E, 1) * 4));
    HALO_CHECK(S.vals[0].reserve(std::max<size_t>(E, 1) * 4));
    HALO_CHECK(S.vals[1].reserve(std::max<size_t>(E, 1) * 4));
    HALO_CHECK(S.hist.reserve((size_t)RS_BINS_MAX * ntmax * 4));
    const size_t nchmax = (ntmax + RS_CH - 1) / RS_CH;
    HALO_CHECK(S.offs.reserve(nchmax * RS_BINS_MAX * 4));
    HALO_CHECK(S.count.reserve(16));
    const size_t ctr_had = S.ctr.bytes;
    HALO_CHECK(S.ctr.reserve((nchmax + 1) * 4));
    if (S.ctr.bytes != ctr_had) HALO_HIP(hipMemsetAsync(S.ctr.ptr, 0, S.ctr.bytes, s));
    int cur = 0;
    for (uint32_t p = 0; p < (uint32_t)plan.size(); p++) {
        const uint32_t bits = plan[p].second;
        RsIn in;
        in.digits = digits;
        in.keys = S.keys[cur ^ 1].as<const uint32_t>();
        in.vals = S.vals[cur ^ 1].as<const uint32_t>();
        in.count = S.count.as<const uint32_t>();
        in.E = E;
        in.npw = npw;
        in.B = B;
        in.pass = p;
        in.shift = plan[p].first;
        const bool fp = fused && p == 0;
        const uint32_t nt = fp ? ntiles0 : tiles_of(bits);
        uint32_t* hist = S.hist.as<uint32_t>();
        uint32_t* offs = S.offs.as<uint32_t>();
        if (fp) {
            for (int q = 0; q < 8; q++)
                in.sc.s[q] = (const uint4*)(fused->P == 1 ? (q == 0 ? fused->scalars : nullptr) : fused->srcs[q]);
            in.sc.n = (uint32_t)fused->n;
            in.sc.P = (uint32_t)fused->P;
            in.sc.B = B;
            in.c = fused->c;
            in.W = fused->W;
            DISPATCH_FIELD(fused->field, SF, {
                if (in.c == 17 && in.W == digits_windows<17>())
                    rs_launch_fused<SF, 17>(in, nt, hist, offs, S, cur, s);
                else if (in.c == 16 && in.W == digits_windows<16>())
                    rs_launch_fused<SF, 16>(in, nt, hist, offs, S, cur, s);
                else
                    rs_launch_fused<SF, 0>(in, nt, hist, offs, S, cur, s);
            });
        } else {
            uint32_t* cnt = p == 0 ? S.count.as<uint32_t>() : nullptr;
            if (bits == 9) {
                auto kh = p == 0 ? k_rs_hist<9, true> : k_rs_hist<9, false>;
                auto ks = p == 0 ? k_rs_scatter<9, void, true> : k_rs_scatter<9, void, false>;
                hipLaunchKernelGGL(kh, dim3(nt), dim3(RS_THREADS), 0, s, in, nt, hist, offs, S.ctr.as<uint32_t>(), cnt);
                hipLaunchKernelGGL(ks, dim3(nt), dim3(RS_THREADS), 2 * 4 * RS_THREADS * rs_rounds<9>(), s, in,
                                   (const uint32_t*)hist, (const uint32_t*)offs, S.keys[cur].as<uint32_t>(),
                                   S.vals[cur].as<uint32_t>());
            } else {
                auto kh = p == 0 ? k_rs_hist<8, true> : k_rs_hist<8, false>;
                auto ks = p == 0 ? k_rs_scatter<8, void, true> : k_rs_scatter<8, void, false>;
                hipLaunchKernelGGL(kh, dim3(nt), dim3(RS_THREADS), 0, s, in, nt, hist, offs, S.ctr.as<uint32_t>(), cnt);
                hipLaunchKernelGGL(ks, dim3(nt), dim3(RS_THREADS), RS_STAGE_BYTES, s, in, (const uint32_t*)hist,
                                   (const uint32_t*)offs, S.keys[cur].as<uint32_t>(), S.vals[cur].as<uint32_t>());
            }
        }
        HALO_HIP(hipGetLastError());
        cur ^= 1;
    }
    *keys_out = S.keys[cur ^ 1].as<uint32_t>();
    *vals_out = S.vals[cur ^ 1].as<uint32_t>();
    *count_out = S.count.as<const uint32_t>();
    if (bstart) HALO_CHECK(msm_bucket_starts(*keys_out, S.count.as<const uint32_t>(), NB, E, bstart, s));
    HALO_HIP(hipGetLastError());
    return HALO_OK;
}

int msm_bucket_starts(const uint32_t* keys, const uint32_t* count, size_t NB, size_t E, uint32_t* bstart, hipStream_t s) {
    hipLaunchKernelGGL(k_bucket_starts, dim3((unsigned)((E + 1 + 255) / 256)), dim3(256), 0, s, keys, count, NB, E,
                       bstart);
    HALO_HIP(hipGetLastError());
    return HALO_OK;
}

}
```

halo_amd/csrc/sort.hpp:

```cpp
#pragma once
#include "runtime.hpp"

namespace halo {

struct SortScratch {
    DevBuf keys[2], vals[2], hist, offs, count, scan_tmp, ctr;
};

int device_exclusive_scan(const uint32_t* in, size_t n, uint32_t* out, DevBuf& tmp, hipStream_t s);

struct RsFused {
    const void* scalars;
    size_t n;
    int c, W, field;
    int P = 1;
    const void* srcs[8] = {};
};
int msm_radix_sort(const uint32_t* digits, size_t E, size_t npw, uint32_t B, uint32_t key_bits, SortScratch& S,
                   uint32_t** keys_out, uint32_t** vals_out, const uint32_t** count_out, uint32_t* bstart, size_t NB,
                   hipStream_t s, const RsFused* fused = nullptr);

int msm_bucket_starts(const uint32_t* keys, const uint32_t* count, size_t NB, size_t E, uint32_t* bstart, hipStream_t s);

}
```

Before: 965.4 million.

## Cache folded scalars between sort passes, defer partial run-out, simplify mul2 asm

The fused sort histogram pass now converts each scalar to canonical form and folds it to a signed magnitude once, writing the 8 words to a new scratch buffer. The scatter pass reads that buffer instead of redoing the Montgomery-to-canonical conversion, which costs extra global traffic in exchange for less arithmetic. Partial bucket sums are stored before the XYZZ run-out, with the sign packed into the top bit of ZZ, and the run-out is done on load. The dual-product multiply asm now accumulates the second product chain straight into the main accumulator, dropping the temporary register pair and the add instructions. The tail reduction also changes how per-lane ranges are split.

```diff
diff --git a/halo_amd/csrc/curve.hpp b/halo_amd/csrc/curve.hpp
--- a/halo_amd/csrc/curve.hpp
+++ b/halo_amd/csrc/curve.hpp
@@ -370,13 +370,14 @@
 
 constexpr int PARTIAL_U4 = 9;
 template <class F>
-HALO_DEV void partial_store(uint4* p, const XYZZ<F>& a) {
+HALO_DEV void partial_store(uint4* p, const XYZZ<F>& a, uint32_t sneg = 0) {
     const Fe<F>* c[4] = {&a.X, &a.Y, &a.ZZ, &a.ZZZ};
     uint32_t w[4 * NLIMB];
 #pragma unroll
     for (int k = 0; k < 4; k++)
 #pragma unroll
         for (int i = 0; i < NLIMB; i++) w[k * NLIMB + i] = c[k]->v[i];
+    w[2 * NLIMB] |= sneg & 0x80000000u;
 #pragma unroll
     for (int q = 0; q < PARTIAL_U4; q++) p[q] = make_uint4(w[4 * q], w[4 * q + 1], w[4 * q + 2], w[4 * q + 3]);
 }
@@ -397,6 +398,9 @@
     for (int k = 0; k < 4; k++)
 #pragma unroll
         for (int i = 0; i < NLIMB; i++) c[k]->v[i] = w[k * NLIMB + i];
+    const uint32_t sneg = (uint32_t)((int32_t)a.ZZ.v[0] >> 31);
+    a.ZZ.v[0] &= 0x7fffffffu;
+    a = xyzz_run_out(a, sneg);
     a.X = fe_reduce_8p(a.X);
     return a;
 }
diff --git a/halo_amd/csrc/digits.hpp b/halo_amd/csrc/digits.hpp
--- a/halo_amd/csrc/digits.hpp
+++ b/halo_amd/csrc/digits.hpp
@@ -4,23 +4,29 @@
 
 namespace halo {
 
+template <class S>
+HALO_DEV void scalar_fold(const uint4* scalar, uint32_t (&f8)[8]) {
+    fe_ark_to_canonical_words<S>(scalar, f8);
+    uint32_t p8[8];
+#pragma unroll
+    for (int q = 0; q < 8; q++) p8[q] = (uint32_t)(S::MODULUS64[q >> 1] >> (32 * (q & 1)));
+    digits_fold(f8, p8);
+}
+
+template <int WMAX = 0, int C = 0, class Fn>
+HALO_DEV void folded_signed_digits(const uint32_t (&f8)[8], int c, int W, Fn&& f) {
+    uint32_t w8[8];
+#pragma unroll
+    for (int q = 0; q < 8; q++) w8[q] = f8[q];
+    const uint32_t flip = digits_unfold(w8);
+    signed_digit_entries<C, WMAX>(w8, flip, c, W, f);
+}
+
 template <class S, int WMAX = 0, int C = 0, class Fn>
 HALO_DEV void scalar_signed_digits(const uint4* scalar, int c, int W, Fn&& f) {
-    uint32_t w8[8];
-    fe_ark_to_canonical_words<S>(scalar, w8);
-    uint32_t t8[8];
-    int64_t br = 0, lt = 0;
-#pragma unroll
-    for (int q = 0; q < 8; q++) {
-        const int64_t d = (int64_t)(uint32_t)(S::MODULUS64[q >> 1] >> (32 * (q & 1))) - (int64_t)w8[q] + br;
-        t8[q] = (uint32_t)d;
-        br = d >> 32;
-        lt = ((int64_t)t8[q] - (int64_t)w8[q] + lt) >> 32;
-    }
-    const bool neg = lt != 0;
-#pragma unroll
-    for (int q = 0; q < 8; q++) w8[q] = neg ? t8[q] : w8[q];
-    signed_digit_entries<C, WMAX>(w8, neg ? 0x80000000u : 0u, c, W, f);
+    uint32_t f8[8];
+    scalar_fold<S>(scalar, f8);
+    folded_signed_digits<WMAX, C>(f8, c, W, f);
 }
 
 }
diff --git a/halo_amd/csrc/digits_core.hpp b/halo_amd/csrc/digits_core.hpp
--- a/halo_amd/csrc/digits_core.hpp
+++ b/halo_amd/csrc/digits_core.hpp
@@ -26,6 +26,27 @@
     const uint32_t m = 0u - carry;
     const uint32_t mag = (v ^ m) + ((full + 1u) & m);
     return (mag - 1u) | ((carry << 31) ^ flip);
+}
+
+HALO_DIGITS_FN void digits_fold(uint32_t (&w8)[8], const uint32_t (&p8)[8]) {
+    uint32_t t8[8];
+    int64_t br = 0, lt = 0;
+    HALO_DIGITS_UNROLL
+    for (int q = 0; q < 8; q++) {
+        const int64_t d = (int64_t)p8[q] - (int64_t)w8[q] + br;
+        t8[q] = (uint32_t)d;
+        br = d >> 32;
+        lt = ((int64_t)t8[q] - (int64_t)w8[q] + lt) >> 32;
+    }
+    const bool neg = lt != 0;
+    HALO_DIGITS_UNROLL
+    for (int q = 0; q < 8; q++) w8[q] = neg ? t8[q] : w8[q];
+    w8[7] |= neg ? 0x80000000u : 0u;
+}
+HALO_DIGITS_FN uint32_t digits_unfold(uint32_t (&w8)[8]) {
+    const uint32_t flip = w8[7] & 0x80000000u;
+    w8[7] &= 0x7fffffffu;
+    return flip;
 }
 
 template <int C>
diff --git a/halo_amd/csrc/field_asm.hpp b/halo_amd/csrc/field_asm.hpp
--- a/halo_amd/csrc/field_asm.hpp
+++ b/halo_amd/csrc/field_asm.hpp
@@ -309,25 +309,22 @@
     uint64_t cc;
     asm(
         "v_mad_u64_u32 v[0:1], %9, %10, %19, 0\n"
-        "v_mad_u64_u32 v[2:3], %9, %28, %37, 0\n"
-        "v_lshl_add_u64 v[0:1], v[2:3], 0, v[0:1]\n"
+        "v_mad_u64_u32 v[0:1], %9, %28, %37, v[0:1]\n"
         "v_and_b32 %0, 0x1fffffff, v0\n"
         "v_ashrrev_i64 v[0:1], 29, v[0:1]\n"
         "v_mad_u64_u32 v[0:1], %9, %10, %20, v[0:1]\n"
         "v_mad_u64_u32 v[0:1], %9, %11, %19, v[0:1]\n"
-        "v_mad_u64_u32 v[2:3], %9, %28, %38, 0\n"
-        "v_mad_u64_u32 v[2:3], %9, %29, %37, v[2:3]\n"
-        "v_lshl_add_u64 v[0:1], v[2:3], 0, v[0:1]\n"
+        "v_mad_u64_u32 v[0:1], %9, %28, %38, v[0:1]\n"
+        "v_mad_u64_u32 v[0:1], %9, %29, %37, v[0:1]\n"
         "v_mad_i64_i32 v[0:1], %9, %0, %46, v[0:1]\n"
         "v_and_b32 %1, 0x1fffffff, v0\n"
         "v_ashrrev_i64 v[0:1], 29, v[0:1]\n"
         "v_mad_u64_u32 v[0:1], %9, %10, %21, v[0:1]\n"
         "v_mad_u64_u32 v[0:1], %9, %11, %20, v[0:1]\n"
         "v_mad_u64_u32 v[0:1], %9, %12, %19, v[0:1]\n"
-        "v_mad_u64_u32 v[2:3], %9, %28, %39, 0\n"
-        "v_mad_u64_u32 v[2:3], %9, %29, %38, v[2:3]\n"
-        "v_mad_u64_u32 v[2:3], %9, %30, %37, v[2:3]\n"
-        "v_lshl_add_u64 v[0:1], v[2:3], 0, v[0:1]\n"
+        "v_mad_u64_u32 v[0:1], %9, %28, %39, v[0:1]\n"
+        "v_mad_u64_u32 v[0:1], %9, %29, %38, v[0:1]\n"
+        "v_mad_u64_u32 v[0:1], %9, %30, %37, v[0:1]\n"
         "v_mad_i64_i32 v[0:1], %9, %1, %46, v[0:1]\n"
         "v_mad_i64_i32 v[0:1], %9, %0, %47, v[0:1]\n"
         "v_and_b32 %2, 0x1fffffff, v0\n"
@@ -336,11 +333,10 @@
         "v_mad_u64_u32 v[0:1], %9, %11, %21, v[0:1]\n"
         "v_mad_u64_u32 v[0:1], %9, %12, %20, v[0:1]\n"
         "v_mad_u64_u32 v[0:1], %9, %13, %19, v[0:1]\n"
-        "v_mad_u64_u32 v[2:3], %9, %28, %40, 0\n"
-        "v_mad_u64_u32 v[2:3], %9, %29, %39, v[2:3]\n"
-        "v_mad_u64_u32 v[2:3], %9, %30, %38, v[2:3]\n"
-        "v_mad_u64_u32 v[2:3], %9, %31, %37, v[2:3]\n"
-        "v_lshl_add_u64 v[0:1], v[2:3], 0, v[0:1]\n"
+        "v_mad_u64_u32 v[0:1], %9, %28, %40, v[0:1]\n"
+        "v_mad_u64_u32 v[0:1], %9, %29, %39, v[0:1]\n"
+        "v_mad_u64_u32 v[0:1], %9, %30, %38, v[0:1]\n"
+        "v_mad_u64_u32 v[0:1], %9, %31, %37, v[0:1]\n"
         "v_mad_i64_i32 v[0:1], %9, %2, %46, v[0:1]\n"
         "v_mad_i64_i32 v[0:1], %9, %1, %47, v[0:1]\n"
         "v_mad_i64_i32 v[0:1], %9, %0, %48, v[0:1]\n"
@@ -351,12 +347,11 @@
         "v_mad_u64_u32 v[0:1], %9, %12, %21, v[0:1]\n"
         "v_mad_u64_u32 v[0:1], %9, %13, %20, v[0:1]\n"
         "v_mad_u64_u32 v[0:1], %9, %14, %19, v[0:1]\n"
-        "v_mad_u64_u32 v[2:3], %9, %28, %41, 0\n"
-        "v_mad_u64_u32 v[2:3], %9, %29, %40, v[2:3]\n"
-        "v_mad_u64_u32 v[2:3], %9, %30, %39, v[2:3]\n"
-        "v_mad_u64_u32 v[2:3], %9, %31, %38, v[2:3]\n"
-        "v_mad_u64_u32 v[2:3], %9, %32, %37, v[2:3]\n"
-        "v_lshl_add_u64 v[0:1], v[2:3], 0, v[0:1]\n"
+        "v_mad_u64_u32 v[0:1], %9, %28, %41, v[0:1]\n"
+        "v_mad_u64_u32 v[0:1], %9, %29, %40, v[0:1]\n"
+        "v_mad_u64_u32 v[0:1], %9, %30, %39, v[0:1]\n"
+        "v_mad_u64_u32 v[0:1], %9, %31, %38, v[0:1]\n"
+        "v_mad_u64_u32 v[0:1], %9, %32, %37, v[0:1]\n"
         "v_mad_i64_i32 v[0:1], %9, %3, %46, v[0:1]\n"
         "v_mad_i64_i32 v[0:1], %9, %2, %47, v[0:1]\n"
         "v_mad_i64_i32 v[0:1], %9, %1, %48, v[0:1]\n"
@@ -369,13 +364,12 @@
         "v_mad_u64_u32 v[0:1], %9, %13, %21, v[0:1]\n"
         "v_mad_u64_u32 v[0:1], %9, %14, %20, v[0:1]\n"
         "v_mad_u64_u32 v[0:1], %9, %15, %19, v[0:1]\n"
-        "v_mad_u64_u32 v[2:3], %9, %28, %42, 0\n"
-        "v_mad_u64_u32 v[2:3], %9, %29, %41, v[2:3]\n"
-        "v_mad_u64_u32 v[2:3], %9, %30, %40, v[2:3]\n"
-        "v_mad_u64_u32 v[2:3], %9, %31, %39, v[2:3]\n"
-        "v_mad_u64_u32 v[2:3], %9, %32, %38, v[2:3]\n"
-        "v_mad_u64_u32 v[2:3], %9, %33, %37, v[2:3]\n"
-        "v_lshl_add_u64 v[0:1], v[2:3], 0, v[0:1]\n"
+        "v_mad_u64_u32 v[0:1], %9, %28, %42, v[0:1]\n"
+        "v_mad_u64_u32 v[0:1], %9, %29, %41, v[0:1]\n"
+        "v_mad_u64_u32 v[0:1], %9, %30, %40, v[0:1]\n"
+        "v_mad_u64_u32 v[0:1], %9, %31, %39, v[0:1]\n"
+        "v_mad_u64_u32 v[0:1], %9, %32, %38, v[0:1]\n"
+        "v_mad_u64_u32 v[0:1], %9, %33, %37, v[0:1]\n"
         "v_mad_i64_i32 v[0:1], %9, %4, %46, v[0:1]\n"
         "v_mad_i64_i32 v[0:1], %9, %3, %47, v[0:1]\n"
         "v_mad_i64_i32 v[0:1], %9, %2, %48, v[0:1]\n"
@@ -389,14 +383,13 @@
         "v_mad_u64_u32 v[0:1], %9, %14, %21, v[0:1]\n"
         "v_mad_u64_u32 v[0:1], %9, %15, %20, v[0:1]\n"
         "v_mad_u64_u32 v[0:1], %9, %16, %19, v[0:1]\n"
-        "v_mad_u64_u32 v[2:3], %9, %28, %43, 0\n"
-        "v_mad_u64_u32 v[2:3], %9, %29, %42, v[2:3]\n"
-        "v_mad_u64_u32 v[2:3], %9, %30, %41, v[2:3]\n"
-        "v_mad_u64_u32 v[2:3], %9, %31, %40, v[2:3]\n"
-        "v_mad_u64_u32 v[2:3], %9, %32, %39, v[2:3]\n"
-        "v_mad_u64_u32 v[2:3], %9, %33, %38, v[2:3]\n"
-        "v_mad_u64_u32 v[2:3], %9, %34, %37, v[2:3]\n"
-        "v_lshl_add_u64 v[0:1], v[2:3], 0, v[0:1]\n"
+        "v_mad_u64_u32 v[0:1], %9, %28, %43, v[0:1]\n"
+        "v_mad_u64_u32 v[0:1], %9, %29, %42, v[0:1]\n"
+        "v_mad_u64_u32 v[0:1], %9, %30, %41, v[0:1]\n"
+        "v_mad_u64_u32 v[0:1], %9, %31, %40, v[0:1]\n"
+        "v_mad_u64_u32 v[0:1], %9, %32, %39, v[0:1]\n"
+        "v_mad_u64_u32 v[0:1], %9, %33, %38, v[0:1]\n"
+        "v_mad_u64_u32 v[0:1], %9, %34, %37, v[0:1]\n"
         "v_mad_i64_i32 v[0:1], %9, %5, %46, v[0:1]\n"
         "v_mad_i64_i32 v[0:1], %9, %4, %47, v[0:1]\n"
         "v_mad_i64_i32 v[0:1], %9, %3, %48, v[0:1]\n"
@@ -411,15 +404,14 @@
         "v_mad_u64_u32 v[0:1], %9, %15, %21, v[0:1]\n"
         "v_mad_u64_u32 v[0:1], %9, %16, %20, v[0:1]\n"
         "v_mad_u64_u32 v[0:1], %9, %17, %19, v[0:1]\n"
-        "v_mad_u64_u32 v[2:3], %9, %28, %44, 0\n"
-        "v_mad_u64_u32 v[2:3], %9, %29, %43, v[2:3]\n"
-        "v_mad_u64_u32 v[2:3], %9, %30, %42, v[2:3]\n"
-        "v_mad_u64_u32 v[2:3], %9, %31, %41, v[2:3]\n"
-        "v_mad_u64_u32 v[2:3], %9, %32, %40, v[2:3]\n"
-        "v_mad_u64_u32 v[2:3], %9, %33, %39, v[2:3]\n"
-        "v_mad_u64_u32 v[2:3], %9, %34, %38, v[2:3]\n"
-        "v_mad_u64_u32 v[2:3], %9, %35, %37, v[2:3]\n"
-        "v_lshl_add_u64 v[0:1], v[2:3], 0, v[0:1]\n"
+        "v_mad_u64_u32 v[0:1], %9, %28, %44, v[0:1]\n"
+        "v_mad_u64_u32 v[0:1], %9, %29, %43, v[0:1]\n"
+        "v_mad_u64_u32 v[0:1], %9, %30, %42, v[0:1]\n"
+        "v_mad_u64_u32 v[0:1], %9, %31, %41, v[0:1]\n"
+        "v_mad_u64_u32 v[0:1], %9, %32, %40, v[0:1]\n"
+        "v_mad_u64_u32 v[0:1], %9, %33, %39, v[0:1]\n"
+        "v_mad_u64_u32 v[0:1], %9, %34, %38, v[0:1]\n"
+        "v_mad_u64_u32 v[0:1], %9, %35, %37, v[0:1]\n"
         "v_mad_i64_i32 v[0:1], %9, %6, %46, v[0:1]\n"
         "v_mad_i64_i32 v[0:1], %9, %5, %47, v[0:1]\n"
         "v_mad_i64_i32 v[0:1], %9, %4, %48, v[0:1]\n"
@@ -435,16 +427,15 @@
         "v_mad_u64_u32 v[0:1], %9, %16, %21, v[0:1]\n"
         "v_mad_u64_u32 v[0:1], %9, %17, %20, v[0:1]\n"
         "v_mad_u64_u32 v[0:1], %9, %18, %19, v[0:1]\n"
-        "v_mad_u64_u32 v[2:3], %9, %28, %45, 0\n"
-        "v_mad_u64_u32 v[2:3], %9, %29, %44, v[2:3]\n"
-        "v_mad_u64_u32 v[2:3], %9, %30, %43, v[2:3]\n"
-        "v_mad_u64_u32 v[2:3], %9, %31, %42, v[2:3]\n"
-        "v_mad_u64_u32 v[2:3], %9, %32, %41, v[2:3]\n"
-        "v_mad_u64_u32 v[2:3], %9, %33, %40, v[2:3]\n"
-        "v_mad_u64_u32 v[2:3], %9, %34, %39, v[2:3]\n"
-        "v_mad_u64_u32 v[2:3], %9, %35, %38, v[2:3]\n"
-        "v_mad_u64_u32 v[2:3], %9, %36, %37, v[2:3]\n"
-        "v_lshl_add_u64 v[0:1], v[2:3], 0, v[0:1]\n"
+        "v_mad_u64_u32 v[0:1], %9, %28, %45, v[0:1]\n"
+        "v_mad_u64_u32 v[0:1], %9, %29, %44, v[0:1]\n"
+        "v_mad_u64_u32 v[0:1], %9, %30, %43, v[0:1]\n"
+        "v_mad_u64_u32 v[0:1], %9, %31, %42, v[0:1]\n"
+        "v_mad_u64_u32 v[0:1], %9, %32, %41, v[0:1]\n"
+        "v_mad_u64_u32 v[0:1], %9, %33, %40, v[0:1]\n"
+        "v_mad_u64_u32 v[0:1], %9, %34, %39, v[0:1]\n"
+        "v_mad_u64_u32 v[0:1], %9, %35, %38, v[0:1]\n"
+        "v_mad_u64_u32 v[0:1], %9, %36, %37, v[0:1]\n"
         "v_mad_i64_i32 v[0:1], %9, %7, %46, v[0:1]\n"
         "v_mad_i64_i32 v[0:1], %9, %6, %47, v[0:1]\n"
         "v_mad_i64_i32 v[0:1], %9, %5, %48, v[0:1]\n"
@@ -461,15 +452,14 @@
         "v_mad_u64_u32 v[0:1], %9, %16, %22, v[0:1]\n"
         "v_mad_u64_u32 v[0:1], %9, %17, %21, v[0:1]\n"
         "v_mad_u64_u32 v[0:1], %9, %18, %20, v[0:1]\n"
-        "v_mad_u64_u32 v[2:3], %9, %29, %45, 0\n"
-        "v_mad_u64_u32 v[2:3], %9, %30, %44, v[2:3]\n"
-        "v_mad_u64_u32 v[2:3], %9, %31, %43, v[2:3]\n"
-        "v_mad_u64_u32 v[2:3], %9, %32, %42, v[2:3]\n"
-        "v_mad_u64_u32 v[2:3], %9, %33, %41, v[2:3]\n"
-        "v_mad_u64_u32 v[2:3], %9, %34, %40, v[2:3]\n"
-        "v_mad_u64_u32 v[2:3], %9, %35, %39, v[2:3]\n"
-        "v_mad_u64_u32 v[2:3], %9, %36, %38, v[2:3]\n"
-        "v_lshl_add_u64 v[0:1], v[2:3], 0, v[0:1]\n"
+        "v_mad_u64_u32 v[0:1], %9, %29, %45, v[0:1]\n"
+        "v_mad_u64_u32 v[0:1], %9, %30, %44, v[0:1]\n"
+        "v_mad_u64_u32 v[0:1], %9, %31, %43, v[0:1]\n"
+        "v_mad_u64_u32 v[0:1], %9, %32, %42, v[0:1]\n"
+        "v_mad_u64_u32 v[0:1], %9, %33, %41, v[0:1]\n"
+        "v_mad_u64_u32 v[0:1], %9, %34, %40, v[0:1]\n"
+        "v_mad_u64_u32 v[0:1], %9, %35, %39, v[0:1]\n"
+        "v_mad_u64_u32 v[0:1], %9, %36, %38, v[0:1]\n"
         "v_mad_i64_i32 v[0:1], %9, %8, %46, v[0:1]\n"
         "v_mad_i64_i32 v[0:1], %9, %7, %47, v[0:1]\n"
         "v_mad_i64_i32 v[0:1], %9, %6, %48, v[0:1]\n"
@@ -484,14 +474,13 @@
         "v_mad_u64_u32 v[0:1], %9, %16, %23, v[0:1]\n"
         "v_mad_u64_u32 v[0:1], %9, %17, %22, v[0:1]\n"
         "v_mad_u64_u32 v[0:1], %9, %18, %21, v[0:1]\n"
-        "v_mad_u64_u32 v[2:3], %9, %30, %45, 0\n"
-        "v_mad_u64_u32 v[2:3], %9, %31, %44, v[2:3]\n"
-        "v_mad_u64_u32 v[2:3], %9, %32, %43, v[2:3]\n"
-        "v_mad_u64_u32 v[2:3], %9, %33, %42, v[2:3]\n"
-        "v_mad_u64_u32 v[2:3], %9, %34, %41, v[2:3]\n"
-        "v_mad_u64_u32 v[2:3], %9, %35, %40, v[2:3]\n"
-        "v_mad_u64_u32 v[2:3], %9, %36, %39, v[2:3]\n"
-        "v_lshl_add_u64 v[0:1], v[2:3], 0, v[0:1]\n"
+        "v_mad_u64_u32 v[0:1], %9, %30, %45, v[0:1]\n"
+        "v_mad_u64_u32 v[0:1], %9, %31, %44, v[0:1]\n"
+        "v_mad_u64_u32 v[0:1], %9, %32, %43, v[0:1]\n"
+        "v_mad_u64_u32 v[0:1], %9, %33, %42, v[0:1]\n"
+        "v_mad_u64_u32 v[0:1], %9, %34, %41, v[0:1]\n"
+        "v_mad_u64_u32 v[0:1], %9, %35, %40, v[0:1]\n"
+        "v_mad_u64_u32 v[0:1], %9, %36, %39, v[0:1]\n"
         "v_mad_i64_i32 v[0:1], %9, %8, %47, v[0:1]\n"
         "v_mad_i64_i32 v[0:1], %9, %7, %48, v[0:1]\n"
         "v_mad_i64_i32 v[0:1], %9, %6, %49, v[0:1]\n"
@@ -504,13 +493,12 @@
         "v_mad_u64_u32 v[0:1], %9, %16, %24, v[0:1]\n"
         "v_mad_u64_u32 v[0:1], %9, %17, %23, v[0:1]\n"
         "v_mad_u64_u32 v[0:1], %9, %18, %22, v[0:1]\n"
-        "v_mad_u64_u32 v[2:3], %9, %31, %45, 0\n"
-        "v_mad_u64_u32 v[2:3], %9, %32, %44, v[2:3]\n"
-        "v_mad_u64_u32 v[2:3], %9, %33, %43, v[2:3]\n"
-        "v_mad_u64_u32 v[2:3], %9, %34, %42, v[2:3]\n"
-        "v_mad_u64_u32 v[2:3], %9, %35, %41, v[2:3]\n"
-        "v_mad_u64_u32 v[2:3], %9, %36, %40, v[2:3]\n"
-        "v_lshl_add_u64 v[0:1], v[2:3], 0, v[0:1]\n"
+        "v_mad_u64_u32 v[0:1], %9, %31, %45, v[0:1]\n"
+        "v_mad_u64_u32 v[0:1], %9, %32, %44, v[0:1]\n"
+        "v_mad_u64_u32 v[0:1], %9, %33, %43, v[0:1]\n"
+        "v_mad_u64_u32 v[0:1], %9, %34, %42, v[0:1]\n"
+        "v_mad_u64_u32 v[0:1], %9, %35, %41, v[0:1]\n"
+        "v_mad_u64_u32 v[0:1], %9, %36, %40, v[0:1]\n"
         "v_mad_i64_i32 v[0:1], %9, %8, %48, v[0:1]\n"
         "v_mad_i64_i32 v[0:1], %9, %7, %49, v[0:1]\n"
         "v_mad_i64_i32 v[0:1], %9, %3, %50, v[0:1]\n"
@@ -521,12 +509,11 @@
         "v_mad_u64_u32 v[0:1], %9, %16, %25, v[0:1]\n"
         "v_mad_u64_u32 v[0:1], %9, %17, %24, v[0:1]\n"
         "v_mad_u64_u32 v[0:1], %9, %18, %23, v[0:1]\n"
-        "v_mad_u64_u32 v[2:3], %9, %32, %45, 0\n"
-        "v_mad_u64_u32 v[2:3], %9, %33, %44, v[2:3]\n"
-        "v_mad_u64_u32 v[2:3], %9, %34, %43, v[2:3]\n"
-        "v_mad_u64_u32 v[2:3], %9, %35, %42, v[2:3]\n"
-        "v_mad_u64_u32 v[2:3], %9, %36, %41, v[2:3]\n"
-        "v_lshl_add_u64 v[0:1], v[2:3], 0, v[0:1]\n"
+        "v_mad_u64_u32 v[0:1], %9, %32, %45, v[0:1]\n"
+        "v_mad_u64_u32 v[0:1], %9, %33, %44, v[0:1]\n"
+        "v_mad_u64_u32 v[0:1], %9, %34, %43, v[0:1]\n"
+        "v_mad_u64_u32 v[0:1], %9, %35, %42, v[0:1]\n"
+        "v_mad_u64_u32 v[0:1], %9, %36, %41, v[0:1]\n"
         "v_mad_i64_i32 v[0:1], %9, %8, %49, v[0:1]\n"
         "v_mad_i64_i32 v[0:1], %9, %4, %50, v[0:1]\n"
         "v_and_b32 %3, 0x1fffffff, v0\n"
@@ -535,41 +522,37 @@
         "v_mad_u64_u32 v[0:1], %9, %16, %26, v[0:1]\n"
         "v_mad_u64_u32 v[0:1], %9, %17, %25, v[0:1]\n"
         "v_mad_u64_u32 v[0:1], %9, %18, %24, v[0:1]\n"
-        "v_mad_u64_u32 v[2:3], %9, %33, %45, 0\n"
-        "v_mad_u64_u32 v[2:3], %9, %34, %44, v[2:3]\n"
-        "v_mad_u64_u32 v[2:3], %9, %35, %43, v[2:3]\n"
-        "v_mad_u64_u32 v[2:3], %9, %36, %42, v[2:3]\n"
-        "v_lshl_add_u64 v[0:1], v[2:3], 0, v[0:1]\n"
+        "v_mad_u64_u32 v[0:1], %9, %33, %45, v[0:1]\n"
+        "v_mad_u64_u32 v[0:1], %9, %34, %44, v[0:1]\n"
+        "v_mad_u64_u32 v[0:1], %9, %35, %43, v[0:1]\n"
+        "v_mad_u64_u32 v[0:1], %9, %36, %42, v[0:1]\n"
         "v_mad_i64_i32 v[0:1], %9, %5, %50, v[0:1]\n"
         "v_and_b32 %4, 0x1fffffff, v0\n"
         "v_ashrrev_i64 v[0:1], 29, v[0:1]\n"
         "v_mad_u64_u32 v[0:1], %9, %16, %27, v[0:1]\n"
         "v_mad_u64_u32 v[0:1], %9, %17, %26, v[0:1]\n"
         "v_mad_u64_u32 v[0:1], %9, %18, %25, v[0:1]\n"
-        "v_mad_u64_u32 v[2:3], %9, %34, %45, 0\n"
-        "v_mad_u64_u32 v[2:3], %9, %35, %44, v[2:3]\n"
-        "v_mad_u64_u32 v[2:3], %9, %36, %43, v[2:3]\n"
-        "v_lshl_add_u64 v[0:1], v[2:3], 0, v[0:1]\n"
+        "v_mad_u64_u32 v[0:1], %9, %34, %45, v[0:1]\n"
+        "v_mad_u64_u32 v[0:1], %9, %35, %44, v[0:1]\n"
+        "v_mad_u64_u32 v[0:1], %9, %36, %43, v[0:1]\n"
         "v_mad_i64_i32 v[0:1], %9, %6, %50, v[0:1]\n"
         "v_and_b32 %5, 0x1fffffff, v0\n"
         "v_ashrrev_i64 v[0:1], 29, v[0:1]\n"
         "v_mad_u64_u32 v[0:1], %9, %17, %27, v[0:1]\n"
         "v_mad_u64_u32 v[0:1], %9, %18, %26, v[0:1]\n"
-        "v_mad_u64_u32 v[2:3], %9, %35, %45, 0\n"
-        "v_mad_u64_u32 v[2:3], %9, %36, %44, v[2:3]\n"
-        "v_lshl_add_u64 v[0:1], v[2:3], 0, v[0:1]\n"
+        "v_mad_u64_u32 v[0:1], %9, %35, %45, v[0:1]\n"
+        "v_mad_u64_u32 v[0:1], %9, %36, %44, v[0:1]\n"
         "v_mad_i64_i32 v[0:1], %9, %7, %50, v[0:1]\n"
         "v_and_b32 %6, 0x1fffffff, v0\n"
         "v_ashrrev_i64 v[0:1], 29, v[0:1]\n"
         "v_mad_u64_u32 v[0:1], %9, %18, %27, v[0:1]\n"
-        "v_mad_u64_u32 v[2:3], %9, %36, %45, 0\n"
-        "v_lshl_add_u64 v[0:1], v[2:3], 0, v[0:1]\n"
+        "v_mad_u64_u32 v[0:1], %9, %36, %45, v[0:1]\n"
         "v_mad_i64_i32 v[0:1], %9, %8, %50, v[0:1]\n"
         "v_and_b32 %7, 0x1fffffff, v0\n"
         "v_alignbit_b32 %8, v1, v0, 29\n"
         : "=&v"(r[0]), "=&v"(r[1]), "=&v"(r[2]), "=&v"(r[3]), "=&v"(r[4]), "=&v"(r[5]), "=&v"(r[6]), "=&v"(r[7]), "=&v"(r[8]), "=&s"(cc)
         : "v"(a[0]), "v"(a[1]), "v"(a[2]), "v"(a[3]), "v"(a[4]), "v"(a[5]), "v"(a[6]), "v"(a[7]), "v"(a[8]), "v"(b[0]), "v"(b[1]), "v"(b[2]), "v"(b[3]), "v"(b[4]), "v"(b[5]), "v"(b[6]), "v"(b[7]), "v"(b[8]), "v"(c[0]), "v"(c[1]), "v"(c[2]), "v"(c[3]), "v"(c[4]), "v"(c[5]), "v"(c[6]), "v"(c[7]), "v"(c[8]), "v"(d[0]), "v"(d[1]), "v"(d[2]), "v"(d[3]), "v"(d[4]), "v"(d[5]), "v"(d[6]), "v"(d[7]), "v"(d[8]), "s"(np[0]), "s"(np[1]), "s"(np[2]), "s"(np[3]), "s"(np[4])
-        : "v0", "v1", "v2", "v3");
+        : "v0", "v1");
 }
 
 __device__ __forceinline__ void fe_muls_asm(const uint32_t (&a)[9], const uint32_t (&b)[9], const uint32_t (&np)[5], uint32_t (&r)[9]) {
diff --git a/halo_amd/csrc/gen_field_asm.py b/halo_amd/csrc/gen_field_asm.py
--- a/halo_amd/csrc/gen_field_asm.py
+++ b/halo_amd/csrc/gen_field_asm.py
@@ -34,10 +34,8 @@
         for x, y in prods:
             ins.append(f"{mad} v[0:1], {{cc}}, {{{x}}}, {{{y}}}, {'0' if first else 'v[0:1]'}")
             first = False
-        if prods2:
-            for t, (x, y) in enumerate(prods2):
-                ins.append(f"v_mad_u64_u32 v[2:3], {{cc}}, {{{x}}}, {{{y}}}, {'0' if t == 0 else 'v[2:3]'}")
-            ins.append("v_lshl_add_u64 v[0:1], v[2:3], 0, v[0:1]")
+        for x, y in prods2:
+            ins.append(f"v_mad_u64_u32 v[0:1], {{cc}}, {{{x}}}, {{{y}}}, v[0:1]")
         for j in RED_J:
             i = k - j
             if 0 <= i < N:
@@ -69,7 +67,7 @@
     outs = ", ".join(f'"=&v"(r[{i}])' for i in range(N)) + ', "=&s"(cc)'
     ins = ", ".join(f'"v"({v}[{i}])' for v in ins_names for i in range(N))
     ins += ", " + ", ".join(f'"s"(np[{t}])' for t in range(len(RED_J)))
-    clob = '"v0", "v1"' + (', "v2", "v3"' if kind == "mul2" else "")
+    clob = '"v0", "v1"'
     asm = "\n".join(f'        "{ln}\\n"' for ln in lines)
     return [f"__device__ __forceinline__ void {name}({params}, const uint32_t (&np)[5], uint32_t (&r)[9]) {{",
             "    uint64_t cc;",
diff --git a/halo_amd/csrc/msm.hip b/halo_amd/csrc/msm.hip
--- a/halo_amd/csrc/msm.hip
+++ b/halo_amd/csrc/msm.hip
@@ -107,7 +107,7 @@
         if (POS != 0 && k != cur) {
             for (uint32_t b = cur + 1; b <= k; b++) bstart[b] = e;
             if (!first_done) {
-                partial_store(first + PARTIAL_U4 * t, xyzz_run_out(acc, sneg));
+                partial_store(first + PARTIAL_U4 * t, acc, sneg);
                 first_done = true;
             } else {
                 xyzz_store(bucket_sums + 8 * (size_t)cur, xyzz_settle(xyzz_run_out(acc, sneg)));
@@ -149,7 +149,7 @@
     step(e++, std::integral_constant<int, 0>{});
     if (e < end) step(e++, std::integral_constant<int, 1>{});
     for (; e < end; e++) step(e, std::integral_constant<int, 2>{});
-    partial_store((first_done ? last : first) + PARTIAL_U4 * t, xyzz_run_out(acc, sneg));
+    partial_store((first_done ? last : first) + PARTIAL_U4 * t, acc, sneg);
     if (end == cnt)
         for (uint32_t b = cur + 1; b <= NB; b++) bstart[b] = cnt;
 }
diff --git a/halo_amd/csrc/msm_tail.hip b/halo_amd/csrc/msm_tail.hip
--- a/halo_amd/csrc/msm_tail.hip
+++ b/halo_amd/csrc/msm_tail.hip
@@ -47,9 +47,9 @@
     }
     XYZZ<F> acc = xyzz_id<F>();
     if (active) {
-        const uint32_t total = t1 - t0, per = (total + LN - 1) / LN;
-        uint32_t t = t0 + 1 + j * per;
-        const uint32_t tb = min(t1, t0 + (j + 1) * per);
+        const uint32_t total = t1 - t0 + 1, per = (total + LN - 1) / LN;
+        uint32_t t = t0 + j * per + (j == 0 ? 1u : 0u);
+        const uint32_t tb = min(t1, t0 + (j + 1) * per - 1);
         constexpr uint32_t G2 = MSM_GROUP * MSM_GROUP;
         auto next_src = [&]() -> const uint4* {
             const uint4* src;
diff --git a/halo_amd/csrc/sort.hip b/halo_amd/csrc/sort.hip
--- a/halo_amd/csrc/sort.hip
+++ b/halo_amd/csrc/sort.hip
@@ -22,6 +22,7 @@
 
 struct RsScalars {
     const uint4* s[8] = {};
+    uint4* folded = nullptr;
     uint32_t n = 0, P = 1, B = 0;
 };
 HALO_DEV const uint4* rs_scalar(const RsScalars& sc, uint32_t g, uint32_t& p, uint32_t& i) {
@@ -203,8 +204,11 @@
     __syncthreads();
     const uint32_t g = blockIdx.x * RS_THREADS + threadIdx.x;
     if (g < sc.P * sc.n) {
-        uint32_t p, i;
-        scalar_signed_digits<S, 0, C>(rs_scalar(sc, g, p, i), c, W, [&](int, uint32_t d) {
+        uint32_t p, i, f8[8];
+        scalar_fold<S>(rs_scalar(sc, g, p, i), f8);
+        sc.folded[2 * (size_t)g] = make_uint4(f8[0], f8[1], f8[2], f8[3]);
+        sc.folded[2 * (size_t)g + 1] = make_uint4(f8[4], f8[5], f8[6], f8[7]);
+        folded_signed_digits<0, C>(f8, c, W, [&](int, uint32_t d) {
             if (d != DIGIT_NONE) atomicAdd(&h[d & 255u], 1u);
         });
     }
@@ -244,10 +248,11 @@
         }
         const uint32_t g = blockIdx.x * RS_THREADS + tid;
         if (g < in.sc.P * in.sc.n) {
-            uint32_t p, i;
-            const uint4* src = rs_scalar(in.sc, g, p, i);
+            const uint32_t p = in.sc.P == 1 ? 0u : g / in.sc.n, i = g - p * in.sc.n;
+            const uint4 lo = in.sc.folded[2 * (size_t)g], hi = in.sc.folded[2 * (size_t)g + 1];
+            const uint32_t f8[8] = {lo.x, lo.y, lo.z, lo.w, hi.x, hi.y, hi.z, hi.w};
             const uint32_t koff = p * in.sc.B;
-            scalar_signed_digits<SF, R, C>(src, in.c, in.W, [&](int w, uint32_t d) {
+            folded_signed_digits<R, C>(f8, in.c, in.W, [&](int w, uint32_t d) {
                 K[w] = koff + (d & 0x7fffffffu);
                 V[w] = ((uint32_t)w * in.sc.n + i) | (d & 0x80000000u);
                 validmask |= (uint32_t)(d != DIGIT_NONE) << w;
@@ -511,6 +516,7 @@
     const size_t nchmax = (ntmax + RS_CH - 1) / RS_CH;
     HALO_CHECK(S.offs.reserve(nchmax * RS_BINS_MAX * 4));
     HALO_CHECK(S.count.reserve(16));
+    if (fused) HALO_CHECK(S.folded.reserve(std::max<size_t>(nsc, 1) * 32));
     const size_t ctr_had = S.ctr.bytes;
     HALO_CHECK(S.ctr.reserve((nchmax + 1) * 4));
     if (S.ctr.bytes != ctr_had) HALO_HIP(hipMemsetAsync(S.ctr.ptr, 0, S.ctr.bytes, s));
@@ -534,6 +540,7 @@
         if (fp) {
             for (int q = 0; q < 8; q++)
                 in.sc.s[q] = (const uint4*)(fused->P == 1 ? (q == 0 ? fused->scalars : nullptr) : fused->srcs[q]);
+            in.sc.folded = S.folded.as<uint4>();
             in.sc.n = (uint32_t)fused->n;
             in.sc.P = (uint32_t)fused->P;
             in.sc.B = B;
diff --git a/halo_amd/csrc/sort.hpp b/halo_amd/csrc/sort.hpp
--- a/halo_amd/csrc/sort.hpp
+++ b/halo_amd/csrc/sort.hpp
@@ -5,6 +5,7 @@
 
 struct SortScratch {
     DevBuf keys[2], vals[2], hist, offs, count, scan_tmp, ctr;
+    DevBuf folded;
 };
 
 int device_exclusive_scan(const uint32_t* in, size_t n, uint32_t* out, DevBuf& tmp, hipStream_t s);
```

Result: faster. 977.4 million, median of 6 (+1.2%).
